# USDA-ARS-GBRU/itsxpress

Measured on AMD Instinct MI355X. Metric: reads/sec trimmed (ITS2, stand-in taxon Tracheophyta for Fungi), higher is better.
Workload: dtype u8+f32

## Files before the change

### itsxpress_amd/csrc/engine.h

```cpp
#pragma once
#include <cstddef>
#include <hip/hip_runtime.h>
#include <stdint.h>
#include <string>
#include <vector>
#include "../../include/itsx_hip.h"
#include "switches.h"

namespace itsx {

constexpr int KP = 18;
constexpr int NCODE = 16;
constexpr int QMAX = 12;
constexpr int MMAX = 46;
constexpr int MSV_REGS = 23;
constexpr int MSV_TW = 24;
constexpr int MAXDOM = 8;
constexpr int BOUND_PAIRS = 23;
constexpr int BOUND_RTAB = BOUND_PAIRS * 12 + 4;
constexpr int BOUND_TAB = (BOUND_PAIRS + 1) * 16 + 2 * BOUND_PAIRS + 2;

struct HostProfile {
  std::string name;
  int M = 0, Q = 0;
  float compo[4];
  float evparam[6];
  std::vector<float> t, mat, tsc, msc;
  float scale_b; int base_b, bias_b, tbm_b, tec_b;
  std::vector<uint8_t> rbv;
  std::vector<float> rfv;
  std::vector<float> tfv;
  float ft10, ft11, fpi0, fpi1;
  float feo[KP][2];
  std::vector<int16_t> rww;
  std::vector<int16_t> tww;
};
std::string parse_hmm_text(const char *text, int64_t len, std::vector<HostProfile> &out);
uint8_t host_tjb_b(int L);

struct alignas(16) DevProfile {
  float tf[QMAX * 8 * 4];
  float tb[QMAX * 6 * 4];
  float rf[NCODE * QMAX * 4];
  float feo[NCODE * 2];
  float ft10, ft11, fpi0, fpi1;
  float ev[6];
  int   M, Q;
  int   pad[4];
  float tfn[(QMAX * 4 + 1) * 8];
};

static_assert(offsetof(DevProfile, tb) == sizeof(float) * QMAX * 8 * 4, "k_float.hip reaches tb as tf + 384 floats");
static_assert(offsetof(DevProfile, tfn) % 16 == 0 && sizeof(DevProfile) % 16 == 0, "tfn is read with 16-byte loads");

constexpr int VIT_TAB = 8 * (MMAX + 1) + NCODE * (MMAX + 1);
struct LenTables {
  float   nullsc;
  float   bias_a;
  float   bias_b;
  float   p1;
  double  lognn3;
  int     tjb;
  int     vmove;
  float   lazy_c;
  int     pad;
};

struct PairRec {
  int32_t  useq;
  int32_t  prof;
  int32_t  xj;
  int32_t  L;
};
struct PairOut {
  float filtersc, fwdsc, bcksc, nullsc, msv_sc;
  int32_t pass_bias, pass_fwd, nregions, ndom, flags;
  int32_t nregions_raw;
};
struct RegionRec {
  int32_t pair;
  int32_t ienv, jenv;
  int32_t multi;
};
struct RegionOut {
  float envsc;
  float domcorrection;
  float n2log[NCODE];
  int32_t ok;
  int32_t own;
  float bN0;
};

#define HIPCHK(expr)                                                                            \
  do {                                                                                          \
    hipError_t e__ = (expr);                                                                    \
    if (e__ != hipSuccess) {                                                                    \
      set_error(std::string(#expr) + ": " + hipGetErrorString(e__));                            \
      return ITSX_E_DEVICE;                                                                     \
    }                                                                                           \
  } while (0)

}
```

### itsxpress_amd/csrc/engine.hip

```cpp
#include <algorithm>
#include <chrono>
#include <cmath>
#include <cstdio>
#include <cstring>
#include <functional>
#include <map>
#include <memory>
#include <numeric>
#include <atomic>
#include <condition_variable>
#include <mutex>
#include <string_view>
#include <thread>
#include <unordered_map>
#include "detmath.h"
#include "engine.h"
#include "k_api.h"
#include "deflate_codes.h"
#include "inflate_codes.h"
#include "fastq_rec.h"
#include "twriter_dev.h"
#include "cluster_multi.h"
#include "fastq_io.h"
#include "iupac.h"
// ... 373 lines not shown
  DBuf<uint32_t> w_slot_of; DBuf<unsigned int> w_ncoll;
  DBuf<uint16_t> w_thr, w_res; DBuf<int32_t> w_tjb, w_cnt, w_total, w_rows, w_rcnt, w_rpref, w_scan2, w_b, w_rrows;
  DBuf<int64_t> w_seg_start, w_idx, w_rseg, w_dz, w_counters, w_useg;
  DBuf<int32_t> w_rrep, w_ruq, w_rurank;
  DBuf<WaveDesc> w_waves, w_rw; DBuf<RegionRec> w_raw; DBuf<float> w_slab, w_eslab;
  DBuf<int32_t> w_mrcnt, w_mroff, w_mrlen, w_mrloff, w_mrrows, w_mrulist, w_mrulist2, w_mru; DBuf<int64_t> w_mrrowoff; DBuf<MrRec> w_mr; DBuf<MrOut> w_mrout; DBuf<int64_t> w_n2off; DBuf<float> w_n2sc, w_mrslab;
  DBuf<uint8_t> w_mrscratch; DBuf<WaveDesc> w_mrwaves;
  DBuf<RegionRec> w_pool, w_pool_sorted; DBuf<int32_t> w_pool_k; DBuf<unsigned long long> w_pool_n, w_pool_key; int64_t pool_cap = 0;
  DBuf<int32_t> w_mrsel; DBuf<int64_t> w_mrselrow; DBuf<MrBig> w_mrbig; DBuf<uint8_t> w_mrarena; DBuf<int32_t> w_mrenv; DBuf<WaveDesc> w_mrbigwaves;
  DBuf<int32_t> w_cl, w_cr;
  DBuf<int8_t> w_side; DBuf<unsigned long long> w_bl, w_br; DBuf<int32_t> w_uind, w_us, w_ue, w_ut, w_rs, w_re, w_rt, w_ri, w_uflag;

  struct ShareBatch { int32_t k0, k1; int64_t node0, nnodes; int32_t nsplit; int64_t gnode0, gnnodes; };
  bool share_on = false; int share_B = 32, share_logB = 5, share_maxd = 0;
  DBuf<unsigned long long> sh_tab, sh_mask_s, sh_mask, sh_counters, msv_xb; DBuf<uint8_t> sh_depth_s, sh_depth;
  DBuf<int32_t> sh_src, sh_parent_s, sh_parent, sh_nn_s, sh_nn, sh_node0_s, sh_node0, sh_order, sh_ulen, sh_uorder, sh_inv, sh_flag, sh_pos, sh_bstart, sh_cursor, sh_segk, sh_scan, sh_cuts;
  std::vector<ShareBatch> sh_batches; std::vector<int32_t> sh_segk_h;
  DBuf<uint4> sh_mgslots; size_t sh_mgslots_half = 0;
  DBuf<uint4> sh_mslots; size_t sh_mslots_half = 0, sh_fslots_half = 0; DBuf<uint32_t> sh_pass, sh_need; DBuf<int32_t> sh_real, sh_segflat, sh_segdepth, sh_wc, sh_woff; DBuf<int64_t> sh_bnd;
  DBuf<uint16_t> sh_res_chk; DBuf<float> sh_fb_chk;
  ShareDev sh_dev{};
  std::string switches_at_search;
  struct TopUp { bool valid = false, list_live = false ; int64_t NP = 0; std::vector<int64_t> seg_start; std::vector<int32_t> total; int32_t u0 = 0, Uc = 0; } topup;
  DBuf<unsigned long long> l_zneed, l_zsplit, l_tcnt; DBuf<int32_t> l_slot, l_pslot; DBuf<uint32_t> l_cut;
  DBuf<int32_t> l_src; DBuf<unsigned long long> l_dmask, l_defn, l_tcnt2;
  int64_t n_topup_deferred = 0, n_topup_ensemble = 0, topup_deferred_live = 0 ;
  std::vector<int64_t> topup_defp;
  std::vector<int32_t> topup_profs, topup_partial;
  std::vector<unsigned long long> h_zneed;
  bool prev_lazy = false; int prev_P = 0; int64_t prev_U = 0, prev_Uc = 0;
  std::vector<int32_t> h_merge_index;
  bool merge_join = false;
  std::vector<int8_t> h_merge_join;
  int64_t pack_exc_hint = 0;
  bool keep_records = false;
  struct Records {
    bool have = false;
    DBuf<uint8_t> seq, qual, titles;
    const uint8_t *seq_p = nullptr;
    DBuf<int64_t> off, toff;
    NameList h_titles;
    void drop() { have = false; seq_p = nullptr; seq.release(); qual.release(); titles.release(); off.release(); toff.release(); h_titles.clear(); }
  } rec;
  bool keep_pair_records = false;
  struct PairRecords {
    bool have = false; int64_t n = 0;
    DBuf<uint8_t> s1, q1, t1, s2, q2, t2;
    DBuf<int64_t> o1, to1, o2, to2;
    DBuf<int32_t> pair_read;
    std::vector<int64_t> pstart;
    void drop()
    {
      have = false; n = 0; pstart.clear(); pair_read.release();
      s1.release(); q1.release(); t1.release(); s2.release(); q2.release(); t2.release(); o1.release(); to1.release(); o2.release(); to2.release();
    }
  } prec;
  DBuf<TrimRec> w_trec2; DBuf<int32_t> w_ttlen;
  DBuf<TrimRec> w_trec; DBuf<int64_t> w_tcnt, w_ttot, w_tblk, w_tfirst, w_tbounds; DBuf<int32_t> w_tstart, w_tstop; DBuf<uint32_t> w_tout;
  DBuf<DeflateBlock> w_dblk; DBuf<uint32_t> w_dtok, w_dtext; DBuf<uint8_t> w_dslots, w_dpacked; DBuf<int32_t> w_dsizes; DBuf<int64_t> w_ddst;
  DBuf<uint8_t> tw_raw; DBuf<int32_t> tw_ls, tw_le; DBuf<int64_t> tw_lblk, tw_qsrc, tw_info;
  DBuf<int8_t> tw_strand; DBuf<uint8_t> tw_comp; bool tw_comp_set = false;
  std::mutex tw_mu; bool tw_failed = false; float tw_ms_deflate = 0;
  DBuf<uint8_t> inf_gz, inf_text; DBuf<int64_t> inf_counts, inf_base, inf_list, inf_where; DBuf<InflateMember> inf_mem; DBuf<int32_t> inf_status;
  int64_t inf_len = -1, n_inf_device = 0, n_inf_declined = 0; bool device_inflate = false; std::mutex inf_mu;
  DBuf<uint8_t> ps_text, ps_seq, ps_qual, ps_titles; DBuf<int64_t> ps_lblk, ps_nl, ps_blk, ps_off, ps_toff, ps_info;
  int64_t ps_n = -1, ps_nb = 0, ps_nt = 0, n_parse_device = 0, n_parse_declined = 0; bool ps_qual_kept = false, device_parse = false; std::mutex ps_mu;
  struct PairSide { DBuf<uint8_t> seq, qual, titles; DBuf<int64_t> off, toff; int64_t nb = 0, nt = 0; } pp[2];
  int64_t pp_n = -1; DBuf<unsigned long long> pp_info;
  bool two_on = false; int share_maxrd = 0; int32_t Ub = 0; size_t sh_gslots_off = 0;
  DBuf<uint8_t> sh_rdepth_s, sh_rdepth; DBuf<unsigned long long> sh_rmask_s, sh_rmask, sh_keys, sh_keys2;
  DBuf<int32_t> sh_rparent_s, sh_rparent, sh_jlev_s, sh_jown_s, sh_endrow_s, sh_rsteps_s, sh_rnn_s, sh_rnode0_s, sh_endrow, sh_jlev, sh_jsrc, sh_jownb;
  DBuf<int32_t> sh_border_s, sh_invb, sh_bsegk, sh_rnn, sh_rnode0, sh_border, sh_bulen, sh_rsrc, sh_bsteps, sh_vals;
  DBuf<uint8_t> sh_sorttmp;
  std::vector<int32_t> sh_bsegk_h;
  BShareDev sh_bdev{};
  DBuf<uint32_t> sh_needb; DBuf<uint16_t> sh_resb; DBuf<int32_t> sh_cntb, sh_totalb, sh_realb, sh_bsegflat, sh_bsegdepth, sh_bwc, sh_bwoff; DBuf<int64_t> sh_bbnd, sh_bseg_start;
  DBuf<PairRec> sh_bpairs; DBuf<WaveDesc> sh_bwaves;
};

#define CTXCHK(c)                                   \
  if (!(c)) return ITSX_E_ARG;
#define SET_ERR(ctx, code, msg) do { (ctx)->set_error(msg); return (code); } while (0)
#undef HIPCHK
#define HIPCHK(expr)                                                                      \
  do {                                                                                    \
    hipError_t e__ = (expr);                                                              \
    if (e__ != hipSuccess) { ctx->set_error(std::string(#expr) + ": " + hipGetErrorString(e__)); return ITSX_E_DEVICE; } \
  } while (0)

template <class T> static hipError_t upload(DBuf<T> &d, const std::vector<T> &h, hipStream_t st, size_t min_elems = 1)
{
  hipError_t e = d.alloc(std::max(h.size(), min_elems));
  if (e != hipSuccess) return e;
  if (h.empty()) return hipSuccess;
  return hipMemcpyAsync(d.p, h.data(), h.size() * sizeof(T), hipMemcpyHostToDevice, st);
}

struct LazyTimers {
  struct Rec { hipEvent_t a, b; float *acc; };
  std::vector<Rec> recs; hipStream_t st;
  explicit LazyTimers(hipStream_t s) : st(s) {}
  size_t begin(float *acc) { Rec r; (void)hipEventCreate(&r.a); (void)hipEventCreate(&r.b); r.acc = acc; (void)hipEventRecord(r.a, st); recs.push_back(r); return recs.size() - 1; }
  void end(size_t i) { (void)hipEventRecord(recs[i].b, st); }
  void collect()
  {
    for (auto &r : recs) { (void)hipEventSynchronize(r.b); float ms = 0; (void)hipEventElapsedTime(&ms, r.a, r.b); *r.acc += ms; (void)hipEventDestroy(r.a); (void)hipEventDestroy(r.b); }
    recs.clear();
  }
  ~LazyTimers() { collect(); }
};

struct StageTimer {
  hipEvent_t a = nullptr, b = nullptr; hipStream_t st;
  explicit StageTimer(hipStream_t s) : st(s) { (void)hipEventCreate(&a); (void)hipEventCreate(&b); (void)hipEventRecord(a, st); }
  float stop() { (void)hipEventRecord(b, st); (void)hipEventSynchronize(b); float ms = 0; (void)hipEventElapsedTime(&ms, a, b); return ms; }
  ~StageTimer() { if (a) (void)hipEventDestroy(a); if (b) (void)hipEventDestroy(b); }
};

using itsx_io::on_threads;

extern "C" {

int itsx_abi_version(void) { return ITSX_ABI_VERSION; }

const char *itsx_last_error(const itsx_ctx *ctx) { return ctx ? ctx->err.c_str() : g_create_error.c_str(); }

struct LoadPriority {
  itsx_ctx *c; bool on;
  explicit LoadPriority(itsx_ctx *ctx) : c(ctx), on(ctx && ctx->st_hi != nullptr) { if (on) std::swap(c->st, c->st_hi); }
  ~LoadPriority() { if (on) { (void)hipStreamSynchronize(c->st); std::swap(c->st, c->st_hi); } }
  LoadPriority(const LoadPriority &) = delete;
  LoadPriority &operator=(const LoadPriority &) = delete;
};

itsx_ctx *itsx_create(int device_id, int flags)
{
  (void)flags;
  int ndev = 0;
  hipError_t e = hipGetDeviceCount(&ndev);
  if (e != hipSuccess || ndev <= 0) { g_create_error = "no HIP device is visible (the engine has no CPU fallback)"; return nullptr; }
  if (device_id < 0 || device_id >= ndev) { g_create_error = "device ordinal out of range"; return nullptr; }
  e = hipSetDevice(device_id);
  if (e != hipSuccess) { g_create_error = std::string("hipSetDevice: ") + hipGetErrorString(e); return nullptr; }
  hipDeviceProp_t prop;
  if (hipGetDeviceProperties(&prop, device_id) != hipSuccess) { g_create_error = "hipGetDeviceProperties failed"; return nullptr; }
  if (std::string(prop.gcnArchName).compare(0, 6, "gfx950") != 0) {
    g_create_error = std::string("device is ") + prop.gcnArchName + "; this engine ships gfx950 code only";
    return nullptr;
  }
  itsx_ctx *ctx = new itsx_ctx();
  ctx->device = device_id;
  ctx->w_slab.pool_device = device_id;
  { std::lock_guard<std::mutex> g(g_pool_mu); g_live_contexts++; }
  if (hipStreamCreate(&ctx->st) != hipSuccess) { g_create_error = "hipStreamCreate failed"; delete ctx; return nullptr; }
  if (!(sw_get("ITSX_LOAD_PRIORITY") && atoi(sw_get("ITSX_LOAD_PRIORITY")) == 0)) {
    int least = 0, greatest = 0;
    if (hipDeviceGetStreamPriorityRange(&least, &greatest) != hipSuccess || greatest == least ||
        hipStreamCreateWithPriority(&ctx->st_hi, hipStreamDefault, greatest) != hipSuccess) { (void)hipGetLastError(); ctx->st_hi = nullptr; }
  }
  std::vector<float> tbl(16000);
  for (int i = 0; i < 16000; i++) tbl[i] = (float)log(1. + exp((double)-i / 1000.f));
  if (upload(ctx->d_flogsum, tbl, ctx->st) != hipSuccess) { g_create_error = "device allocation failed"; delete ctx; return nullptr; }
  std::vector<LogTab> lt(LOGTAB_N);
  build_logtab(lt.data());
  if (upload(ctx->d_logtab, lt, ctx->st) != hipSuccess) { g_create_error = "device allocation failed"; delete ctx; return nullptr; }
  (void)hipStreamSynchronize(ctx->st);
  return ctx;
}

void itsx_destroy(itsx_ctx *ctx)
{
  if (!ctx) return;
  (void)hipSetDevice(ctx->device);
  (void)hipStreamSynchronize(ctx->st);
  if (ctx->st3) { (void)hipStreamSynchronize(ctx->st3); (void)hipStreamDestroy(ctx->st3); (void)hipEventDestroy(ctx->ev_s3a); (void)hipEventDestroy(ctx->ev_s3b); }
  if (ctx->st2) { (void)hipStreamSynchronize(ctx->st2); (void)hipStreamDestroy(ctx->st2); (void)hipEventDestroy(ctx->ev_a); (void)hipEventDestroy(ctx->ev_b);
                  if (ctx->ev_msv0) { (void)hipEventDestroy(ctx->ev_msv0); (void)hipEventDestroy(ctx->ev_msv1); (void)hipEventDestroy(ctx->ev_c); } }
  (void)hipStreamDestroy(ctx->st);
  if (ctx->st_hi) { (void)hipStreamSynchronize(ctx->st_hi); (void)hipStreamDestroy(ctx->st_hi); }
  for (int k = 0; k < itsx_ctx::NSTAGE; k++) { if (ctx->stage_pin[k]) (void)hipHostFree(ctx->stage_pin[k]); if (ctx->stage_ev[k]) (void)hipEventDestroy(ctx->stage_ev[k]); }
  delete ctx;
  grave_flush();
  bool last = false;
  { std::lock_guard<std::mutex> g(g_pool_mu); last = --g_live_contexts <= 0; }
  if (last) pool_flush();
}

int itsx_release_scratch(itsx_ctx *ctx)
{
  CTXCHK(ctx);
  HIPCHK(hipSetDevice(ctx->device));
  HIPCHK(hipStreamSynchronize(ctx->st));
  if (ctx->st2) HIPCHK(hipStreamSynchronize(ctx->st2));
  if (ctx->st3) HIPCHK(hipStreamSynchronize(ctx->st3));
  if (ctx->w_slab.p) { pool_put(ctx->w_slab.p, ctx->w_slab.cap * sizeof(float), ctx->device); ctx->w_slab.p = nullptr; ctx->w_slab.n = ctx->w_slab.cap = 0; }
  return ITSX_OK;
}

static int install_profiles(itsx_ctx *ctx, std::vector<HostProfile> &pv, int *n_profiles)
{
  for (auto &p : pv) {
    if (p.M > MMAX || p.Q > QMAX) SET_ERR(ctx, ITSX_E_UNSUPPORTED, "model '" + p.name + "' has more than 46 nodes; the device kernels hold at most 46");
    if (p.base_b + p.bias_b >= 255) SET_ERR(ctx, ITSX_E_UNSUPPORTED, "model '" + p.name + "': MSV bias too large");
  }
  ctx->thr_memo.clear(); ctx->thr_memo_have.clear(); ctx->thr_memo_F1 = -1.0;
  HIPCHK(hipSetDevice(ctx->device));
  LoadPriority load_priority(ctx);
  ctx->profs = std::move(pv);
  const int P = (int)ctx->profs.size();
  ctx->P = P; ctx->G = (P + 63) / 64;
  const int Ppad = ctx->G * 64;
  std::vector<DevProfile> dp(std::max(P, 1));
  ctx->generic_q.assign(P, 0);
  std::vector<uint32_t> etab((size_t)std::max(P, 1) * 16 * MSV_TW, 0);
  std::vector<int32_t> pb(std::max(Ppad, 64), 0), pt(std::max(Ppad, 64), 0), pm(std::max(Ppad, 64), 0);
  for (size_t i = 0; i < etab.size(); i++) etab[i] = 0xFF01FF01u;
  for (int i = 0; i < P; i++) {
    const HostProfile &h = ctx->profs[i];
    DevProfile &d = dp[i];
    memset(&d, 0, sizeof(d));
    for (int q = 0; q < h.Q; q++) {
      for (int t = 0; t < 7; t++) for (int z = 0; z < 4; z++) d.tf[(q * 8 + t) * 4 + z] = h.tfv[((size_t)q * 7 + t) * 4 + z];
      for (int z = 0; z < 4; z++) d.tf[(q * 8 + 7) * 4 + z] = h.tfv[((size_t)7 * h.Q + q) * 4 + z];
    }
    for (int k = 1; k <= 4 * h.Q; k++)
      for (int t = 0; t < 8; t++) d.tfn[k * 8 + t] = d.tf[(((k - 1) % h.Q) * 8 + t) * 4 + (k - 1) / h.Q];
    for (int q = 0; q < h.Q; q++) {
      const int order[3] = {6, 5, 0};
      for (int k = 0; k < 3; k++) for (int z = 0; z < 4; z++) d.tb[(q * 6 + k) * 4 + z] = d.tf[(q * 8 + order[k]) * 4 + z];
      for (int k = 0; k < 3; k++)
        for (int z = 0; z < 4; z++) {
          float v;
          if (q + 1 < h.Q) v = d.tf[((q + 1) * 8 + 1 + k) * 4 + z];
          else v = (z < 3) ? d.tf[(0 * 8 + 1 + k) * 4 + z + 1] : 0.0f;
          d.tb[(q * 6 + 3 + k) * 4 + z] = v;
        }
    }
    for (int x = 0; x < NCODE; x++)
      for (int q = 0; q < h.Q; q++) for (int z = 0; z < 4; z++) d.rf[(x * QMAX + q) * 4 + z] = h.rfv[((size_t)x * h.Q + q) * 4 + z];
    for (int x = 0; x < NCODE; x++) { d.feo[x * 2] = h.feo[x][0]; d.feo[x * 2 + 1] = h.feo[x][1]; }
    d.ft10 = h.ft10; d.ft11 = h.ft11; d.fpi0 = h.fpi0; d.fpi1 = h.fpi1;
    for (int k = 0; k < 6; k++) d.ev[k] = h.evparam[k];
    d.M = h.M; d.Q = h.Q;
    ctx->generic_q[i] = (h.Q != QMAX);
    for (int x = 0; x < NCODE; x++)
      for (int r = 0; r < MSV_REGS; r++) {
        uint32_t packed = 0;
        for (int half = 0; half < 2; half++) {
          const int k = half * MSV_REGS + r + 1;
          const int cost = (k <= h.M) ? h.rbv[(size_t)x * (h.M + 1) + k] : 255;
          const int16_t e = (int16_t)(h.bias_b - cost);
          packed |= (uint32_t)(uint16_t)e << (16 * half);
        }
        etab[((size_t)i * 16 + x) * MSV_TW + r] = packed;
      }
    pb[i] = h.bias_b; pt[i] = h.tec_b; pm[i] = h.tbm_b;
  }
  {
    std::vector<int16_t> vt((size_t)std::max(P, 1) * VIT_TAB, (int16_t)-32768);
    for (int i = 0; i < P; i++) {
      const HostProfile &h = ctx->profs[i];
      int16_t *t = vt.data() + (size_t)i * VIT_TAB;
      for (int k8 = 0; k8 < 8; k8++) for (int k = 0; k <= h.M; k++) t[k8 * (MMAX + 1) + k] = h.tww[(size_t)k8 * (h.M + 1) + k];
      for (int x = 0; x < NCODE; x++) for (int k = 0; k <= h.M; k++) t[(8 + x) * (MMAX + 1) + k] = h.rww[(size_t)x * (h.M + 1) + k];
    }
    HIPCHK(upload(ctx->d_vtab, vt, ctx->st));
  }
  {
    const int KK = 2 * BOUND_PAIRS;
    std::vector<std::vector<double>> G((size_t)P), SC((size_t)P), AA((size_t)P), RI((size_t)P);
    bool fold = !(sw_get("ITSX_BOUND_FOLD") && atoi(sw_get("ITSX_BOUND_FOLD")) == 0);
    for (int i = 0; i < P && fold; i++) {
      const DevProfile &d = dp[i];
      const int K = 4 * ctx->profs[i].Q;
      auto tn = [&](int k, int t) { return (k >= 1 && k <= K) ? (double)d.tfn[k * 8 + t] : 0.0; };
      std::vector<double> H((size_t)KK + 3, 1.0), &g = G[(size_t)i], &sc = SC[(size_t)i], &aa = AA[(size_t)i], &ri = RI[(size_t)i];
      g.assign((size_t)KK + 2, 1.0); sc.assign((size_t)KK + 3, 1.0); aa.assign((size_t)KK + 2, 0.0); ri.assign((size_t)KK + 2, 1.0);
      for (int k = KK; k >= 1; k--) H[(size_t)k] = 1.0 + tn(k, 7) * H[(size_t)k + 1];
      for (int k = 1; k <= KK; k++) g[(size_t)k] = 1.0 + tn(k, 4) * H[(size_t)k + 1];
      for (int k = 1; k <= KK; k++) {
        const double md = tn(k, 4), dd = tn(k, 7);
        if (md > 0.0) { sc[(size_t)k + 1] = md / g[(size_t)k]; aa[(size_t)k] = sc[(size_t)k] * dd / sc[(size_t)k + 1]; }
        else if (dd > 0.0 && k > 1) fold = false;
        else { sc[(size_t)k + 1] = 1.0; aa[(size_t)k] = 0.0; }
        if (!(sc[(size_t)k + 1] > 1e-6 && sc[(size_t)k + 1] < 1e6 && aa[(size_t)k] < 1e6)) fold = false;
        const double mi = tn(k, 5);
        if (mi > 0.0) ri[(size_t)k] = mi / g[(size_t)k];
        else if (tn(k, 6) > 0.0 || tn(k + 1, 2) > 0.0) fold = false;
        else ri[(size_t)k] = 1.0;
        if (!(ri[(size_t)k] > 1e-6)) fold = false;
      }
    }
    ctx->bound_fold = fold;
    std::vector<float> bt((size_t)std::max(P, 1) * BOUND_TAB, 0.0f);
    for (int i = 0; i < P; i++) {
      const DevProfile &d = dp[i];
      const int K = 4 * ctx->profs[i].Q;
      auto tn = [&](int k, int t) { return (k >= 1 && k <= K) ? d.tfn[k * 8 + t] : 0.0f; };
      auto gk = [&](int k) { return fold && k >= 1 && k <= KK ? G[(size_t)i][(size_t)k] : 1.0; };
      auto sk = [&](int k) { return fold && k >= 1 && k <= KK + 1 ? SC[(size_t)i][(size_t)k] : 1.0; };
      auto rk = [&](int k) { return fold && k >= 1 && k <= KK ? RI[(size_t)i][(size_t)k] : 1.0; };
      for (int j = 0; j <= BOUND_PAIRS; j++) {
        float *o = bt.data() + (size_t)i * BOUND_TAB + (size_t)j * 16;
        if (j < BOUND_PAIRS) {
          const int k1 = 2 * j + 1, k2 = 2 * j + 2;
          o[0] = (float)(tn(k1 + 1, 1) / gk(k1)); o[1] = (float)(tn(k2 + 1, 1) / gk(k2));
          o[2] = (float)(tn(k1 + 1, 2) * rk(k1)); o[3] = (float)(tn(k2 + 1, 2) * rk(k2));
          o[4] = (float)(tn(k1 + 1, 3) * sk(k1)); o[5] = (float)(tn(k2 + 1, 3) * sk(k2));
          o[6] = tn(k1, 6); o[7] = tn(k2, 6);
          o[12] = (float)(tn(k1, 5) / gk(k1)); o[13] = (float)(tn(k2, 5) / gk(k2));
        }
        if (j > 0) {
          const int k1 = 2 * (j - 1) + 1, k2 = 2 * (j - 1) + 2;
          o[8] = tn(k1, 0); o[9] = tn(k2, 0);
          if (fold) { o[10] = k1 > 1 ? (float)AA[(size_t)i][(size_t)k1 - 1] : 0.0f; o[11] = (float)AA[(size_t)i][(size_t)k1]; }
          else { o[10] = tn(k1 - 1, 7); o[11] = tn(k1, 7); }
          o[14] = tn(k1, 4); o[15] = tn(k2, 4);
        }
      }
      float *gq = bt.data() + (size_t)i * BOUND_TAB + (size_t)(BOUND_PAIRS + 1) * 16;
      for (int k0 = 0; k0 < KK; k0++) gq[k0] = (float)gk(k0 + 1);
    }
    HIPCHK(upload(ctx->d_btab, bt, ctx->st));
    std::vector<float> rt((size_t)std::max(P, 1) * BOUND_RTAB, 0.0f);
    for (int i = 0; i < P && fold; i++) {
      const float *b = bt.data() + (size_t)i * BOUND_TAB;
      for (int j = 0; j <= BOUND_PAIRS; j++) {
        float *o = rt.data() + (size_t)i * BOUND_RTAB + (size_t)j * 12;
        if (j < BOUND_PAIRS) {
          for (int q = 0; q < 6; q++) o[q] = b[(size_t)j * 16 + q];
          o[6] = b[(size_t)(j + 1) * 16 + 8]; o[7] = b[(size_t)(j + 1) * 16 + 9];
        }
        if (j >= 1) {
          const int jj = j - 1;
          float *q = j < BOUND_PAIRS ? o + 8 : o;
          q[0] = b[(size_t)jj * 16 + 6]; q[1] = b[(size_t)jj * 16 + 7];
          q[2] = b[(size_t)(jj + 1) * 16 + 11];
          q[3] = (jj + 2 <= BOUND_PAIRS) ? b[(size_t)(jj + 2) * 16 + 10] : 0.0f;
        }
      }
    }
    HIPCHK(upload(ctx->d_rtab, rt, ctx->st));
    std::vector<float> et((size_t)std::max(P, 1) * NCODE * KK, 0.0f);
    for (int i = 0; i < P && fold; i++) {
      const DevProfile &d = dp[i];
      const int Q = ctx->profs[i].Q;
      const float *gq = bt.data() + (size_t)i * BOUND_TAB + (size_t)(BOUND_PAIRS + 1) * 16;
      for (int x = 0; x < NCODE; x++)
        for (int k0 = 0; k0 < KK; k0++) {
          const float e = (k0 < 4 * Q) ? d.rf[(x * QMAX + (k0 % Q)) * 4 + k0 / Q] : 0.0f;
          et[((size_t)i * NCODE + x) * KK + k0] = e * gq[k0];
        }
    }
    HIPCHK(upload(ctx->d_entab, et, ctx->st));
  }
  HIPCHK(upload(ctx->d_prof, dp, ctx->st));
  HIPCHK(upload(ctx->d_etab, etab, ctx->st));
  HIPCHK(upload(ctx->d_pbias, pb, ctx->st));
  HIPCHK(upload(ctx->d_ptec, pt, ctx->st));
  HIPCHK(upload(ctx->d_ptbm, pm, ctx->st));
  HIPCHK(hipStreamSynchronize(ctx->st));
  ctx->stats.n_profiles = P;
  ctx->have_search = ctx->have_final = false;
  if (n_profiles) *n_profiles = P;
  return ITSX_OK;
}

int itsx_load_profiles_mem(itsx_ctx *ctx, const char *text, int64_t len, int *n_profiles)
{
  CTXCHK(ctx && text && len >= 0);
  std::vector<HostProfile> pv;
  const std::string e = parse_hmm_text(text, len, pv);
  if (!e.empty()) SET_ERR(ctx, ITSX_E_FORMAT, e);
  return install_profiles(ctx, pv, n_profiles);
}

static bool inflate_for_loader(itsx_ctx *ctx, const itsx_io::Text &raw, itsx_io::Text &out);
static bool device_inflate_on(const itsx_ctx *ctx);
constexpr int PARSE_FALLBACK = 1;
static bool device_parse_on(const itsx_ctx *ctx);
static int load_parsed_device(itsx_ctx *ctx, const char *const *paths, int32_t n_paths, const char *text, int64_t nbytes, int64_t *n_reads_per_file, bool batch);
static int merge_pairs_load_device(itsx_ctx *ctx, const char *const *r1_paths, const char *const *r2_paths, const char *const *seq_out_paths, int32_t S,
                                   const char *text1, int64_t nb1, const char *text2, int64_t nb2, int maxdiffs, double maxee, int allow_stagger,
                                   int64_t *n_pairs_per_sample, int64_t *n_merged_per_sample, bool batch);
static std::shared_ptr<const itsx_io::Text> slurp(const char *path, bool cacheable, std::string &err, itsx_ctx *ctx = nullptr)
{
  if (ctx && device_inflate_on(ctx)) {
    const itsx_io::InflateFirst first = [ctx](const itsx_io::Text &raw, itsx_io::Text &out) { return inflate_for_loader(ctx, raw, out); };
    return itsx_io::read_text(path, err, cacheable, &first);
  }
  return itsx_io::read_text(path, err, cacheable);
}

int itsx_load_profiles_file(itsx_ctx *ctx, const char *hmm_path, int *n_profiles)
{
  CTXCHK(ctx && hmm_path);
  std::string err;
  const auto tp = slurp(hmm_path, false, err);
  if (!tp) SET_ERR(ctx, ITSX_E_IO, err);
  return itsx_load_profiles_mem(ctx, tp->data(), (int64_t)tp->size(), n_profiles);
}

int itsx_profile_name(const itsx_ctx *ctx, int i, char *buf, int buflen)
{
  CTXCHK(ctx && buf && buflen > 0 && i >= 0 && i < ctx->P);
  snprintf(buf, (size_t)buflen, "%s", ctx->profs[i].name.c_str());
  return ITSX_OK;
}

int itsx_profile_tables(const itsx_ctx *ctx, int i, uint8_t *rbv, float *rfv, float *tfv, int32_t *params6)
{
  CTXCHK(ctx && i >= 0 && i < ctx->P);
  const HostProfile &h = ctx->profs[i];
  if (rbv) memcpy(rbv, h.rbv.data(), h.rbv.size());
  if (rfv) memcpy(rfv, h.rfv.data(), h.rfv.size() * sizeof(float));
  if (tfv) memcpy(tfv, h.tfv.data(), h.tfv.size() * sizeof(float));
  if (params6) { params6[0] = h.M; params6[1] = h.Q; params6[2] = h.base_b; params6[3] = h.bias_b; params6[4] = h.tbm_b; params6[5] = h.tec_b; }
  return ITSX_OK;
}

static int8_t g_code[256];
static bool g_code_init = false;
static void init_codes()
{
  if (g_code_init) return;
  memset(g_code, -1, sizeof(g_code));
  const char *sym = "ACGT-RYMKSWHBVDN";
  for (int i = 0; i < 16; i++) { g_code[(unsigned char)sym[i]] = (int8_t)i; g_code[(unsigned char)(sym[i] | 0x20)] = (int8_t)i; }
  g_code[(unsigned char)'-'] = -1;
  g_code[(unsigned char)'U'] = g_code[(unsigned char)'u'] = 3;
  g_code[(unsigned char)'X'] = g_code[(unsigned char)'x'] = 15;
  g_code_init = true;
}

static int stage_reserve(itsx_ctx *ctx, int64_t bytes)
{
  if ((int64_t)ctx->stage_cap >= bytes) return ITSX_OK;
  for (int k = 0; k < itsx_ctx::NSTAGE; k++) {
    if (ctx->stage_pin[k]) { (void)hipHostFree(ctx->stage_pin[k]); ctx->stage_pin[k] = nullptr; }
    HIPCHK(hipHostMalloc(&ctx->stage_pin[k], (size_t)bytes, hipHostMallocDefault));
    HIPCHK(ctx->stage_dev[k].alloc((size_t)bytes + 16, true));
    if (!ctx->stage_ev[k]) HIPCHK(hipEventCreateWithFlags(&ctx->stage_ev[k], hipEventDisableTiming));
  }
  ctx->stage_cap = (size_t)bytes;
  return ITSX_OK;
}

static int pack_and_upload(itsx_ctx *ctx, const char *view = nullptr, const uint8_t *dev_raw = nullptr)
{
  init_codes();
  ctx->rec.drop(); ctx->prec.drop();
  const auto tp0 = std::chrono::steady_clock::now();
  const int64_t n = ctx->N;
  ctx->dev_bases = dev_raw;
  if (ctx->d_merged_text.p && dev_raw != ctx->d_merged_text.p) ctx->d_merged_text.release();
  ctx->bases_view = dev_raw ? nullptr : (view ? view : ctx->h_bases.data());
  const char *bases = ctx->bases_view;
  ctx->h_len.resize((size_t)n); ctx->h_woff.resize((size_t)n + 1);
  ctx->h_woff[0] = 0;
  int Lmax = 0;
  {
    const int T = n >= (1 << 20) ? std::max(1, std::min(8, itsx_io::io_threads())) : 1;
    std::vector<int64_t> wsum((size_t)T + 1, 0); std::vector<int> lmx((size_t)T, 0), bad((size_t)T, 0);
    on_threads(T, [&](int t) {
      const int64_t lo = n * t / T, hi = n * (t + 1) / T;
      int64_t w = 0; int mx = 0, b = 0;
      for (int64_t r = lo; r < hi; r++) {
        const int64_t L = ctx->h_off[r + 1] - ctx->h_off[r];
        if (L < 0) b |= 1;
        if (L > 65535) b |= 2;
        ctx->h_len[r] = (int32_t)L;
        mx = std::max(mx, (int)std::min<int64_t>(L, 1 << 30));
        w += std::max<int64_t>(1, (L + 15) / 16);
        ctx->h_woff[r + 1] = w;
      }
      wsum[(size_t)t + 1] = w; lmx[(size_t)t] = mx; bad[(size_t)t] = b;
    });
    int b = 0;
    for (int t = 0; t < T; t++) { wsum[(size_t)t + 1] += wsum[(size_t)t]; Lmax = std::max(Lmax, lmx[(size_t)t]); b |= bad[(size_t)t]; }
    if (b & 1) SET_ERR(ctx, ITSX_E_ARG, "read offsets must be non-decreasing");
    if (b & 2) SET_ERR(ctx, ITSX_E_UNSUPPORTED, "reads longer than 65535 bases are not supported");
    if (T > 1)
      on_threads(T, [&](int t) {
        if (t == 0) return;
        const int64_t lo = n * t / T, hi = n * (t + 1) / T, add = wsum[(size_t)t];
        for (int64_t r = lo; r < hi; r++) ctx->h_woff[r + 1] += add;
      });
  }
  ctx->Lmax = Lmax;
  HIPCHK(hipSetDevice(ctx->device));
  hipStream_t st = ctx->st;
  const int64_t nb = n > 0 ? ctx->h_off[n] : 0;
  int64_t CH = 64ll << 20;
  if (const char *e = sw_get("ITSX_PACK_CHUNK")) CH = std::max<int64_t>(70000, atoll(e));
  CH = std::min<int64_t>(CH, std::max<int64_t>(nb, 70000));
  constexpr int K = itsx_ctx::NSTAGE;
  if (!dev_raw) { const int src = stage_reserve(ctx, CH); if (src != ITSX_OK) return src; }
  DBuf<int64_t> &d_off = ctx->w_pk_off; DBuf<int8_t> &d_lut = ctx->w_pk_lut; DBuf<int32_t> &d_excnt = ctx->w_pk_excnt, &d_exstart = ctx->w_pk_exstart, &d_tmp = ctx->w_pk_tmp;
  DBuf<long long> &d_bad = ctx->w_pk_bad;
  HIPCHK(d_off.alloc((size_t)n + 1)); HIPCHK(d_lut.alloc(256)); HIPCHK(d_excnt.alloc((size_t)n + 2)); HIPCHK(d_exstart.alloc((size_t)n + 2));
  HIPCHK(d_tmp.alloc((size_t)scan_tmp_elems(n + 2))); HIPCHK(d_bad.alloc(4));
  HIPCHK(ctx->d_words.alloc((size_t)ctx->h_woff[n] + 1)); HIPCHK(ctx->d_woff.alloc((size_t)n + 1)); HIPCHK(ctx->d_excoff.alloc((size_t)n + 1)); HIPCHK(ctx->d_len.alloc((size_t)n + 1));
  HIPCHK(hipMemcpyAsync(d_off.p, ctx->h_off.data(), ((size_t)n + 1) * 8, hipMemcpyHostToDevice, st));
  HIPCHK(hipMemcpyAsync(ctx->d_woff.p, ctx->h_woff.data(), ((size_t)n + 1) * 8, hipMemcpyHostToDevice, st));
  if (n) HIPCHK(hipMemcpyAsync(ctx->d_len.p, ctx->h_len.data(), (size_t)n * 4, hipMemcpyHostToDevice, st));
  HIPCHK(hipMemcpyAsync(d_lut.p, g_code, 256, hipMemcpyHostToDevice, st));
  HIPCHK(hipMemsetAsync(d_excnt.p, 0, ((size_t)n + 2) * 4, st));
  int64_t ecap = std::max<int64_t>((int64_t)ctx->d_exc.cap, nb / 256 + 4096 + ctx->pack_exc_hint);
  ctx->pack_exc_hint = 0;
  if (const char *e = sw_get("ITSX_PACK_ECAP")) ecap = std::max<int64_t>(1, atoll(e));
  HIPCHK(ctx->d_exc.alloc((size_t)ecap));
  int copy_threads = std::max(1, std::min(8, itsx_io::io_threads()));
  long long hb[4] = {0, 0, 0, 0};
  for (int pass = 0; pass < 2; pass++) {
    const long long init[4] = {0, 0, 0x7f7f7f7f7f7f7f7fll, 0};
    HIPCHK(hipMemcpyAsync(d_bad.p, init, sizeof(init), hipMemcpyHostToDevice, st));
    int64_t r0 = 0; int c = 0;
    if (dev_raw && n > 0) {
      if (pass == 0) launch_pack(dev_raw, 0, d_off.p, ctx->d_woff.p, 0, n, d_lut.p, ctx->d_words.p, d_excnt.p, d_bad.p + 2, st);
      launch_exclusive_scan(d_excnt.p, d_exstart.p, n + 1, d_tmp.p, st);
      launch_pack_exc(dev_raw, 0, d_off.p, 0, n, d_lut.p, d_excnt.p, d_exstart.p, d_bad.p, ecap, ctx->d_excoff.p, ctx->d_exc.p, st);
      r0 = n;
    }
    while (r0 < n) {
      const int64_t b0 = ctx->h_off[r0];
      int64_t r1 = (int64_t)(std::upper_bound(ctx->h_off.begin() + r0, ctx->h_off.begin() + n + 1, b0 + CH) - ctx->h_off.begin()) - 1;
      r1 = std::min<int64_t>(n, std::max<int64_t>(r1, r0 + 1));
      const int64_t bytes = ctx->h_off[r1] - b0;
      const int k = c % K;
      if (c >= K) HIPCHK(hipEventSynchronize(ctx->stage_ev[k]));
      if (bytes > 0) {
        char *dst = (char *)ctx->stage_pin[k];
        const int T = bytes >= (4 << 20) ? copy_threads : 1;
        on_threads(T, [&](int t) { const int64_t lo = bytes * t / T, hi = bytes * (t + 1) / T; memcpy(dst + lo, bases + b0 + lo, (size_t)(hi - lo)); });
        HIPCHK(hipMemcpyAsync(ctx->stage_dev[k].p, dst, (size_t)bytes, hipMemcpyHostToDevice, st));
      }
      if (pass == 0) launch_pack(ctx->stage_dev[k].p, b0, d_off.p, ctx->d_woff.p, r0, r1, d_lut.p, ctx->d_words.p, d_excnt.p, d_bad.p + 2, st);
      launch_exclusive_scan(d_excnt.p + r0, d_exstart.p + r0, r1 - r0 + 1, d_tmp.p, st);
      launch_pack_exc(ctx->stage_dev[k].p, b0, d_off.p, r0, r1, d_lut.p, d_excnt.p, d_exstart.p, d_bad.p, ecap, ctx->d_excoff.p, ctx->d_exc.p, st);
      HIPCHK(hipEventRecord(ctx->stage_ev[k], st));
      r0 = r1; c++;
    }
    if (n == 0) HIPCHK(hipMemsetAsync(ctx->d_excoff.p, 0, 8, st));
    HIPCHK(hipMemcpyAsync(hb, d_bad.p, sizeof(hb), hipMemcpyDeviceToHost, st));
    HIPCHK(hipStreamSynchronize(st));
    HIPCHK(hipGetLastError());
    if (hb[2] >= 0 && hb[2] < n) SET_ERR(ctx, ITSX_E_FORMAT, "read " + std::to_string(hb[2]) + " contains a symbol outside the IUPAC DNA alphabet");
    if (!hb[1]) break;
    if (pass == 1) SET_ERR(ctx, ITSX_E_DEVICE, "exception list overflow after resizing");
    ecap = hb[0] + 1;
    HIPCHK(ctx->d_exc.alloc((size_t)ecap));
  }
  ctx->rd.words = ctx->d_words.p; ctx->rd.woff = ctx->d_woff.p; ctx->rd.len = ctx->d_len.p;
  ctx->rd.excoff = ctx->d_excoff.p; ctx->rd.exc = ctx->d_exc.p; ctx->rd.n = n;
  ctx->have_derep = ctx->have_search = ctx->have_final = false; ctx->drop_cigars();
  ctx->stats.n_reads = n;
  ctx->order_cache_ok = false;
  ctx->S = 1; ctx->sel_sample = -1; ctx->h_sample.clear(); ctx->h_usample.clear();
  ctx->stats.ms_pack = (float)std::chrono::duration<double, std::milli>(std::chrono::steady_clock::now() - tp0).count();
  return ITSX_OK;
}

static int64_t take_offsets(itsx_ctx *ctx, const int64_t *offsets, int64_t n)
{
  const int64_t base0 = offsets[0];
  ctx->h_off.resize((size_t)n + 1);
  int64_t *dst = ctx->h_off.data();
  const int T = n >= (1 << 20) ? std::max(1, std::min(8, itsx_io::io_threads())) : 1;
  on_threads(T, [&](int t) { for (int64_t r = (n + 1) * t / T, hi = (n + 1) * (t + 1) / T; r < hi; r++) dst[r] = offsets[r] - base0; });
  return base0;
}
static int set_reads_impl(itsx_ctx *ctx, const char *bases, const int64_t *offsets, int64_t n, const char *names, const int64_t *name_offsets, bool borrow)
{
  CTXCHK(ctx && offsets && n >= 0 && (bases || offsets[n] == offsets[0]));
  if (n >= (1ll << 31) - 64) SET_ERR(ctx, ITSX_E_UNSUPPORTED, "more than 2^31 reads in one context");
  ctx->N = n;
  const int64_t base0 = take_offsets(ctx, offsets, n);
  const char *view = nullptr;
  if (borrow) { itsx_io::Text().swap(ctx->h_bases); view = bases ? bases + base0 : ""; }
  else if (bases) ctx->h_bases.assign(bases + base0, (size_t)(offsets[n] - base0));
  else ctx->h_bases.clear();
  ctx->h_names.clear();
  if (names && name_offsets) {
    ctx->h_names.assign(names, name_offsets, n);
  }
  return pack_and_upload(ctx, view);
}
int itsx_set_reads(itsx_ctx *ctx, const char *bases, const int64_t *offsets, int64_t n, const char *names, const int64_t *name_offsets)
{ return set_reads_impl(ctx, bases, offsets, n, names, name_offsets, false); }
int itsx_set_reads_view(itsx_ctx *ctx, const char *bases, const int64_t *offsets, int64_t n, const char *names, const int64_t *name_offsets)
{ return set_reads_impl(ctx, bases, offsets, n, names, name_offsets, true); }
int itsx_set_reads_device(itsx_ctx *ctx, const void *d_bases, const int64_t *offsets, int64_t n, const char *names, const int64_t *name_offsets)
{
  CTXCHK(ctx && offsets && n >= 0 && (d_bases || offsets[n] == offsets[0]));
  if (n >= (1ll << 31) - 64) SET_ERR(ctx, ITSX_E_UNSUPPORTED, "more than 2^31 reads in one context");
  ctx->N = n;
  const int64_t base0 = take_offsets(ctx, offsets, n);
  itsx_io::Text().swap(ctx->h_bases);
  ctx->h_names.clear();
  if (names && name_offsets) {
    ctx->h_names.assign(names, name_offsets, n);
  }
  static const uint8_t none = 0;
  return pack_and_upload(ctx, nullptr, d_bases ? (const uint8_t *)d_bases + base0 : &none);
}

struct FastxPart {
  itsx_io::Text seq, qual; std::vector<int64_t> off{0}; NameList ids;
  NameList titles;
  bool lower = false;
  int rc = ITSX_OK; std::string err;
};

static void parse_fastx_range(const char *s, const char *end, bool want_qual, bool upper, FastxPart &out)
{
  auto next_line = [&](const char *&b, const char *&e) -> bool {
    if (s >= end) return false;
    b = s; const char *nl = (const char *)memchr(s, '\n', (size_t)(end - s));
    e = nl ? nl : end; s = nl ? nl + 1 : end;
    if (e > b && e[-1] == '\r') e--;
    return true;
  };
  auto put_seq = [&](const char *b, const char *e) {
    const size_t o = out.seq.size();
    out.seq.append(b, e);
    if (upper) { char *q = out.seq.data(); for (size_t i = o; i < out.seq.size(); i++) { const char u = (char)toupper((unsigned char)q[i]); if (u != q[i]) { q[i] = u; out.lower = true; } } }
  };
  if (end > s && (size_t)(end - s) > ((size_t)1 << 20)) { out.seq.reserve(out.seq.size() + (size_t)(end - s) / 2 + 4096); if (want_qual) out.qual.reserve(out.qual.size() + (size_t)(end - s) / 2 + 4096); out.ids.blob.reserve(out.ids.blob.size() + (size_t)(end - s) / 8); }
  const char *b, *e;
  bool pending = false;
  while (pending || next_line(b, e)) {
    pending = false;
    if (b == e) continue;
    if (*b == '@') {
      const char *ne = b + 1; while (ne < e && *ne != ' ' && *ne != '\t') ne++;
      out.ids.emplace_back(b + 1, ne);
      const char *sb, *se, *pb, *pe, *qb, *qe;
      if (!next_line(sb, se) || !next_line(pb, pe) || !next_line(qb, qe) || pb == pe || *pb != '+' || (qe - qb) != (se - sb)) {
        out.rc = ITSX_E_FORMAT; out.err = "malformed FASTQ record"; return;
      }
      put_seq(sb, se);
// ... 693 lines not shown
  }
  if (n_helpers == 0) return itsx_cluster(ctx, id, strand_both, n_unique);
  if (!(id > 0.0 && id <= 1.0)) SET_ERR(ctx, ITSX_E_ARG, "cluster id must be in (0, 1]");
  if (id == 1.0) return itsx_derep(ctx, strand_both, 32, n_unique);
  if (ctx->S > 1) SET_ERR(ctx, ITSX_E_UNSUPPORTED, "greedy clustering (id < 1) is sequential per sample: run it one sample per call, not on a sample batch");
  ClusterShards shards(ctx->device, ctx->st, hs);
  return cluster_run(ctx, id, strand_both, n_unique, false, &shards);
}
int itsx_cluster_samples(itsx_ctx *ctx, double id, int strand_both, int64_t *n_unique)
{
  CTXCHK(ctx);
  if (!(id > 0.0 && id <= 1.0)) SET_ERR(ctx, ITSX_E_ARG, "cluster id must be in (0, 1]");
  if (id == 1.0) return itsx_derep(ctx, strand_both, 32, n_unique);
  if (ctx->S <= 1) return itsx_cluster(ctx, id, strand_both, n_unique);
  return cluster_run(ctx, id, strand_both, n_unique, true);
}

int itsx_get_cluster(const itsx_ctx *ctx, double *pct_id, int64_t *order, int64_t *n_order)
{
  CTXCHK(ctx && ctx->have_derep && ctx->clustered);
  if (pct_id) for (int64_t r = 0; r < ctx->N; r++) pct_id[r] = ctx->h_pct[r];
  if (order) for (size_t i = 0; i < ctx->h_order.size(); i++) order[i] = ctx->h_order[i];
  if (n_order) *n_order = (int64_t)ctx->h_order.size();
  return ITSX_OK;
}

int itsx_align_clusters(itsx_ctx *ctx, int64_t *n_aligned, float *ms_kernels)
{
  CTXCHK(ctx);
  if (!ctx->have_derep || !ctx->clustered) SET_ERR(ctx, ITSX_E_ARG, "itsx_align_clusters comes after a clustering at id < 1 (itsx_cluster, itsx_cluster_multi, itsx_cluster_samples); exact dereplication has nothing to align");
  HIPCHK(hipSetDevice(ctx->device));
  ctx->drop_cigars();
  const int64_t n = ctx->N;
  hipStream_t st = ctx->st;
  std::vector<int32_t> hq, ht; std::vector<int8_t> hs;
  int Lmax = 1;
  for (int64_t r = 0; r < n; r++) {
    const int32_t rep = ctx->h_rep_of[(size_t)r];
    if (rep < 0 || rep == r) continue;
    hq.push_back((int32_t)r); ht.push_back(rep); hs.push_back(ctx->h_strand[(size_t)r]);
    Lmax = std::max(Lmax, std::max((int)ctx->h_len[(size_t)r], (int)ctx->h_len[(size_t)rep]));
  }
  const size_t M = hq.size();
  float ms = 0.0f;
  std::vector<std::string> text(M);
  if (M > 0) {
    int rows_per_lane = (Lmax + 1 <= 320) ? 5 : (Lmax + 1 <= 512) ? 8 : 10;
    if (const char *e = sw_get("ITSX_CL_ROWS")) rows_per_lane = atoi(e) <= 5 ? 5 : atoi(e) <= 8 ? 8 : 10;
    double budget_mb = 2048.0;
    if (const char *e = sw_get("ITSX_CIGAR_MB")) budget_mb = std::max(0.0, atof(e));
    const size_t budget = (size_t)(budget_mb * 1048576.0);
    DBuf<int32_t> d_q, d_t, d_eq, d_tlen; DBuf<int8_t> d_s; DBuf<int64_t> d_doff, d_soff, d_toff;
    DBuf<uint8_t> d_dir, d_text; DBuf<long long> d_scr, d_res; DBuf<double> d_pid;
    HIPCHK(upload(d_q, hq, st)); HIPCHK(upload(d_t, ht, st)); HIPCHK(upload(d_s, hs, st));
    HIPCHK(d_eq.alloc(M)); HIPCHK(d_res.alloc(M)); HIPCHK(d_pid.alloc(M));
    CigarArgs a{};
    a.rd = ctx->rd; a.q_read = d_q.p; a.t_read = d_t.p; a.strand = d_s.p; a.res = d_res.p; a.pid = d_pid.p;
    std::vector<int32_t> eq(M);
    launch_cg_equal(a, (int32_t)M, d_eq.p, st);
    HIPCHK(hipMemcpyAsync(eq.data(), d_eq.p, M * sizeof(int32_t), hipMemcpyDeviceToHost, st));
    HIPCHK(hipStreamSynchronize(st));
    std::vector<int32_t> pq, pt, pm; std::vector<int8_t> ps; std::vector<int64_t> doff, soff;
    struct Batch { size_t p0, np, dir_bytes, scr_elems; };
    std::vector<Batch> batches;
    for (size_t m = 0; m < M; m++) {
      if (eq[m]) { text[m] = "="; continue; }
      size_t db = 0, sb = 0;
      cg_pair_bytes(ctx->h_len[(size_t)hq[m]], ctx->h_len[(size_t)ht[m]], rows_per_lane, &db, &sb);
      db = (db + 255) & ~(size_t)255;
      if (batches.empty() || (batches.back().np > 0 && batches.back().dir_bytes + batches.back().scr_elems * 8 + db + sb > budget)) batches.push_back(Batch{pq.size(), 0, 0, 0});
      Batch &b = batches.back();
      doff.push_back((int64_t)b.dir_bytes); soff.push_back((int64_t)b.scr_elems);
      b.np++; b.dir_bytes += db; b.scr_elems += sb / 8;
      pq.push_back(hq[m]); pt.push_back(ht[m]); ps.push_back(hs[m]); pm.push_back((int32_t)m);
    }
    const size_t NP = pq.size();
    if (NP > 0) {
      size_t max_dir = 0, max_scr = 0, max_np = 0;
      for (const Batch &b : batches) { max_dir = std::max(max_dir, b.dir_bytes); max_scr = std::max(max_scr, b.scr_elems); max_np = std::max(max_np, b.np); }
      HIPCHK(upload(d_q, pq, st)); HIPCHK(upload(d_t, pt, st)); HIPCHK(upload(d_s, ps, st)); HIPCHK(upload(d_doff, doff, st)); HIPCHK(upload(d_soff, soff, st));
      if (d_dir.alloc(max_dir + 256, true) != hipSuccess || d_scr.alloc(max_scr + 2, true) != hipSuccess) {
        (void)hipGetLastError();
        SET_ERR(ctx, ITSX_E_NOMEM, "itsx_align_clusters: no device memory for " + std::to_string((max_dir + max_scr * 8) >> 20) + " MB of direction bits (lower ITSX_CIGAR_MB; a pair larger than the budget needs its own size)");
      }
      HIPCHK(d_tlen.alloc(max_np)); HIPCHK(d_toff.alloc(max_np + 1));
      a.q_read = d_q.p; a.t_read = d_t.p; a.strand = d_s.p; a.dir_off = d_doff.p; a.scr_off = d_soff.p;
      a.dir = d_dir.p; a.scratch = d_scr.p; a.tlen = d_tlen.p; a.toff = d_toff.p;
      std::vector<int32_t> tlen; std::vector<int64_t> toff; std::vector<char> plane;
      for (const Batch &b : batches) {
        StageTimer t1(st);
        launch_cg_forward(a, (int32_t)b.p0, (int32_t)b.np, rows_per_lane, Lmax, st);
        launch_cg_traceback(a, (int32_t)b.p0, (int32_t)b.np, rows_per_lane, 0, st);
        ms += t1.stop();
        HIPCHK(hipGetLastError());
        tlen.resize(b.np); toff.assign(b.np + 1, 0);
        HIPCHK(hipMemcpy(tlen.data(), d_tlen.p, b.np * sizeof(int32_t), hipMemcpyDeviceToHost));
        for (size_t k = 0; k < b.np; k++) {
          if (tlen[k] <= 0) SET_ERR(ctx, ITSX_E_DEVICE, "itsx_align_clusters: the direction bits of read " + std::to_string(pq[b.p0 + k]) + " do not lead back to the first cell");
          toff[k + 1] = toff[k] + tlen[k];
        }
        HIPCHK(d_text.alloc((size_t)toff[b.np] + 1));
        a.text = reinterpret_cast<char *>(d_text.p);
        HIPCHK(hipMemcpyAsync(d_toff.p, toff.data(), (b.np + 1) * sizeof(int64_t), hipMemcpyHostToDevice, st));
        StageTimer t2(st);
        launch_cg_traceback(a, (int32_t)b.p0, (int32_t)b.np, rows_per_lane, 1, st);
        ms += t2.stop();
        HIPCHK(hipGetLastError());
        plane.resize((size_t)toff[b.np]);
        HIPCHK(hipMemcpy(plane.data(), d_text.p, plane.size(), hipMemcpyDeviceToHost));
        for (size_t k = 0; k < b.np; k++) text[(size_t)pm[b.p0 + k]].assign(plane.data() + toff[k], (size_t)tlen[k]);
      }
      std::vector<double> pid(NP);
      HIPCHK(hipMemcpy(pid.data(), d_pid.p, NP * sizeof(double), hipMemcpyDeviceToHost));
      for (size_t k = 0; k < NP; k++)
        if (memcmp(&pid[k], &ctx->h_pct[(size_t)pq[k]], sizeof(double)) != 0)
          SET_ERR(ctx, ITSX_E_DEVICE, "itsx_align_clusters: read " + std::to_string(pq[k]) + " aligns at identity " + std::to_string(pid[k]) + ", the clustering accepted it at " + std::to_string(ctx->h_pct[(size_t)pq[k]]));
    }
  }
  ctx->h_cg_off.assign((size_t)n + 1, 0);
  { size_t m = 0, tot = 0; for (int64_t r = 0; r < n; r++) { ctx->h_cg_off[(size_t)r] = (int64_t)tot; if (m < M && hq[m] == r) tot += text[m++].size(); } ctx->h_cg_off[(size_t)n] = (int64_t)tot; ctx->h_cg_text.reserve(tot); }
  for (size_t m = 0; m < M; m++) ctx->h_cg_text += text[m];
  ctx->have_cigar = true;
  if (n_aligned) *n_aligned = (int64_t)M;
  if (ms_kernels) *ms_kernels = ms;
  return ITSX_OK;
}
int itsx_get_cluster_cigars(const itsx_ctx *ctx, int64_t *offs, char *text)
{
  CTXCHK(ctx && offs);
  if (!ctx->cigars_live()) SET_ERR(ctx, ITSX_E_ARG, "itsx_get_cluster_cigars: no alignments for the current clustering (itsx_align_clusters comes after itsx_cluster* at id < 1)");
  memcpy(offs, ctx->h_cg_off.data(), ((size_t)ctx->N + 1) * sizeof(int64_t));
  if (text && !ctx->h_cg_text.empty()) memcpy(text, ctx->h_cg_text.data(), ctx->h_cg_text.size());
  return ITSX_OK;
}

int itsx_get_derep(const itsx_ctx *ctx, int64_t *rep_of, int8_t *strand, int64_t *uniq_of)
{
  CTXCHK(ctx && ctx->have_derep);
  for (int64_t r = 0; r < ctx->N; r++) {
    if (rep_of) rep_of[r] = ctx->h_rep_of[r];
    if (strand) strand[r] = ctx->h_strand[r];
    if (uniq_of) uniq_of[r] = ctx->h_uniq_of[r];
  }
  return ITSX_OK;
}
int itsx_get_uniques(const itsx_ctx *ctx, int64_t *seed_read, int64_t *abundance)
{
  CTXCHK(ctx && ctx->have_derep);
  for (int32_t u = 0; u < ctx->U; u++) { if (seed_read) seed_read[u] = ctx->h_seed_read[u]; if (abundance) abundance[u] = ctx->h_abund[u]; }
  return ITSX_OK;
}


int itsx_unique_keys(itsx_ctx *ctx, uint64_t seed, uint64_t *fwd, uint64_t *rc)
{
  CTXCHK(ctx && ctx->have_derep && fwd && rc);
  if (ctx->S > 1) SET_ERR(ctx, ITSX_E_UNSUPPORTED, "cross-rank dereplication of a sample batch is not supported: shard whole samples across ranks");
  HIPCHK(hipSetDevice(ctx->device));
  const int64_t n = ctx->N;
  if (n == 0 || ctx->U == 0) return ITSX_OK;
  HIPCHK(ctx->w_hf.alloc((size_t)n + 1)); HIPCHK(ctx->w_hr.alloc((size_t)n + 1));
  launch_hash_reads(ctx->rd, seed, 1, ctx->w_hf.p, ctx->w_hr.p, ctx->st);
  std::vector<uint64_t> hf((size_t)n), hr((size_t)n);
  HIPCHK(hipMemcpyAsync(hf.data(), ctx->w_hf.p, (size_t)n * 8, hipMemcpyDeviceToHost, ctx->st));
  HIPCHK(hipMemcpyAsync(hr.data(), ctx->w_hr.p, (size_t)n * 8, hipMemcpyDeviceToHost, ctx->st));
  HIPCHK(hipStreamSynchronize(ctx->st));
  for (int32_t u = 0; u < ctx->U; u++) {
    const size_t r = (size_t)ctx->h_seed_read[u];
    const uint64_t lm = (uint64_t)ctx->h_len[r] * 0x9E3779B97F4A7C15ULL;
    fwd[u] = hf[r] ^ lm; rc[u] = hr[r] ^ lm;
  }
  return ITSX_OK;
}

static int set_walked_uniques(itsx_ctx *ctx, const std::vector<int32_t> *keep)
{
  const std::vector<int32_t> &lst = keep ? *keep : ctx->h_sorted_uniq;
  ctx->U_active = (int32_t)lst.size();
  ctx->h_sorted_active = lst;
  if (!lst.empty()) {
    HIPCHK(hipMemcpyAsync(ctx->d_sorted_uniq.p, lst.data(), lst.size() * 4, hipMemcpyHostToDevice, ctx->st));
    launch_fill_ulen(ctx->U_active, ctx->d_sorted_uniq.p, ctx->d_seed_read.p, ctx->rd.len, ctx->d_ulen.p, ctx->st);
    HIPCHK(hipStreamSynchronize(ctx->st));
  }
  return ITSX_OK;
}

int itsx_set_active_uniques(itsx_ctx *ctx, const uint8_t *active)
{
  CTXCHK(ctx && ctx->have_derep && (active || ctx->U == 0));
  HIPCHK(hipSetDevice(ctx->device));
  std::vector<int32_t> keep; keep.reserve((size_t)ctx->U);
  for (int32_t s = 0; s < ctx->U; s++) { const int32_t u = ctx->h_sorted_uniq[(size_t)s]; if (active[u]) keep.push_back(u); }
  { const int rc = set_walked_uniques(ctx, &keep); if (rc != ITSX_OK) return rc; }
  ctx->active_narrowed = true;
  ctx->have_search = ctx->have_final = false;
  return ITSX_OK;
}

static float msv_score_from_byte(int xj, int tjb)
{
  float sc = ((float)(xj - tjb) - 190.0f);
  sc /= (float)(3.0 / 0.69314718055994529);
  sc -= 3.0f;
  return sc;
}

static int search_chunk(itsx_ctx *ctx, int ci, int32_t u0, int32_t U, int Lcap, double T, double F1, double F3);
static int append_traces(itsx_ctx *ctx);

static int build_share(itsx_ctx *ctx)
{
  hipStream_t st = ctx->st;
  itsx_stats &S = ctx->stats;
  ctx->share_on = false; ctx->sh_batches.clear(); ctx->sh_segk_h.clear();
  S.share_B = 0; S.share_batches = 0; S.share_nodes = S.share_chains = 0; S.ms_share_build = 0; S.share_frac = 0;
  ctx->two_on = false; ctx->Ub = 0; ctx->share_maxrd = 0; ctx->sh_bsegk_h.clear();
  S.two_sided = 0; S.n_joined = 0; S.bwd_chains = 0; S.gamma_nodes = 0; S.bwd_rows = 0; S.join_maxdiff = 0; S.ms_bwd_bound = 0; S.n_bwd_launches = 0; S.two_fwd_rows = S.two_bwd_rows = S.two_rows_full = 0;
  const int32_t U = ctx->U_active, Uc = (int32_t)std::min<int64_t>(ctx->s_Uc, 0x7fffffff), P = ctx->P;
  if (const char *e = sw_get("ITSX_SHARE")) if (atoi(e) == 0) return ITSX_OK;
  if (sw_get("ITSX_LAZY_EXACT_BOUND")) return ITSX_OK;
  if (U < 2 || U >= (1 << 26) || P <= 0) return ITSX_OK;
  int B = 32;
  if (const char *e = sw_get("ITSX_SHARE_B")) B = atoi(e);
  int logB = 0; while ((1 << logB) < B) logB++;
  if (B < 16 || B > 1024 || (1 << logB) != B) SET_ERR(ctx, ITSX_E_ARG, "ITSX_SHARE_B must be a power of two between 16 and 1024");
  StageTimer tm(st);
  TrieArgs a{};
  a.rd = ctx->rd; a.sorted_uniq = ctx->d_sorted_uniq.p; a.seed_read = ctx->d_seed_read.p; a.U = U; a.Uc = std::max(1, Uc); a.B = B;
  HIPCHK(ctx->sh_counters.alloc(16));
  HIPCHK(hipMemsetAsync(ctx->sh_counters.p, 0, 16 * sizeof(unsigned long long), st));
  a.counters = ctx->sh_counters.p;
  launch_trie_keycount(a, st);
  if (ctx->lazy && ctx->bound_fold) { TrieArgs r0 = a; r0.rev = 1; launch_trie_keycount(r0, st); }
  unsigned long long hc0[8] = {0, 0, 0, 0, 0, 0, 0, 0};
  HIPCHK(hipMemcpyAsync(hc0, ctx->sh_counters.p, sizeof(hc0), hipMemcpyDeviceToHost, st));
  HIPCHK(hipStreamSynchronize(st));
  const unsigned long long nkeys = std::max(hc0[4], hc0[6]);
  if (nkeys == 0) return ITSX_OK;
  uint64_t slots = 1024; while (slots < 2 * nkeys) slots <<= 1;
  HIPCHK(ctx->sh_tab.alloc((size_t)slots, true));
  HIPCHK(hipMemsetAsync(ctx->sh_tab.p, 0xFF, (size_t)slots * sizeof(unsigned long long), st));
  HIPCHK(ctx->sh_depth_s.alloc((size_t)U + 1)); HIPCHK(ctx->sh_parent_s.alloc((size_t)U + 1)); HIPCHK(ctx->sh_mask_s.alloc((size_t)U + 1));
  HIPCHK(ctx->sh_nn_s.alloc((size_t)U + 2)); HIPCHK(ctx->sh_node0_s.alloc((size_t)U + 2)); HIPCHK(ctx->sh_scan.alloc((size_t)scan_tmp_elems((int64_t)U + 2)));
  HIPCHK(hipMemsetAsync(ctx->sh_mask_s.p, 0, ((size_t)U + 1) * sizeof(unsigned long long), st));
  a.tab = ctx->sh_tab.p; a.tmask = slots - 1; a.depth = ctx->sh_depth_s.p; a.parent = ctx->sh_parent_s.p; a.mask = ctx->sh_mask_s.p; a.nn = ctx->sh_nn_s.p;
  launch_trie_insert(a, st); launch_trie_resolve(a, st); launch_trie_link(a, st); launch_trie_count(a, st);
  launch_exclusive_scan(ctx->sh_nn_s.p, ctx->sh_node0_s.p, (int64_t)U + 1, ctx->sh_scan.p, st);
  bool two = ctx->lazy && ctx->bound_fold && !(sw_get("ITSX_SHARE_TWO") && atoi(sw_get("ITSX_SHARE_TWO")) == 0);
  TrieArgs ar = a;
  JoinArgs ja{};
  if (two) {
    HIPCHK(ctx->sh_rdepth_s.alloc((size_t)U + 1)); HIPCHK(ctx->sh_rparent_s.alloc((size_t)U + 1)); HIPCHK(ctx->sh_rmask_s.alloc((size_t)U + 1));
    HIPCHK(ctx->sh_jlev_s.alloc((size_t)U + 1)); HIPCHK(ctx->sh_jown_s.alloc((size_t)U + 1)); HIPCHK(ctx->sh_endrow_s.alloc((size_t)U + 1));
    HIPCHK(ctx->sh_rsteps_s.alloc((size_t)U + 1)); HIPCHK(ctx->sh_rnn_s.alloc((size_t)U + 2)); HIPCHK(ctx->sh_rnode0_s.alloc((size_t)U + 2));
    HIPCHK(hipMemsetAsync(ctx->sh_tab.p, 0xFF, (size_t)slots * sizeof(unsigned long long), st));
    HIPCHK(hipMemsetAsync(ctx->sh_rmask_s.p, 0, ((size_t)U + 1) * sizeof(unsigned long long), st));
    ar.rev = 1; ar.depth = ctx->sh_rdepth_s.p; ar.parent = ctx->sh_rparent_s.p; ar.mask = ctx->sh_rmask_s.p; ar.nn = ctx->sh_rnn_s.p;
    launch_trie_insert(ar, st); launch_trie_resolve(ar, st); launch_trie_link(ar, st);
    ja.t = ar; ja.fdepth = ctx->sh_depth_s.p; ja.fmask = ctx->sh_mask_s.p; ja.rmask = ctx->sh_rmask_s.p; ja.jlev = ctx->sh_jlev_s.p; ja.jown = ctx->sh_jown_s.p;
    ja.endrow = ctx->sh_endrow_s.p; ja.rsteps = ctx->sh_rsteps_s.p; ja.counters = ctx->sh_counters.p;
    launch_join_resolve(ja, st);
    for (int r = 63; r >= 1; r--) launch_join_up(ja, r, st);
    launch_join_ends(ja, st);
    launch_popc64(ctx->sh_rmask_s.p, ctx->sh_rnn_s.p, (int64_t)U + 1, U, st);
    launch_exclusive_scan(ctx->sh_rnn_s.p, ctx->sh_rnode0_s.p, (int64_t)U + 1, ctx->sh_scan.p, st);
  }
  const int32_t ncap = 65536 + U / std::max(1, Uc) + 8;
  HIPCHK(ctx->sh_cuts.alloc((size_t)ncap * 3));
  launch_share_cuts(ctx->d_ulen.p, ctx->sh_node0_s.p, two ? ctx->sh_rnode0_s.p : nullptr, U, a.Uc, ncap, ctx->sh_cuts.p, ctx->sh_counters.p + 5, st);
  int32_t NN = 0, NG = 0;
  unsigned long long hc[16];
  HIPCHK(hipMemcpyAsync(hc, ctx->sh_counters.p, sizeof(hc), hipMemcpyDeviceToHost, st));
  HIPCHK(hipMemcpyAsync(&NN, ctx->sh_node0_s.p + U, sizeof(NN), hipMemcpyDeviceToHost, st));
  if (two) HIPCHK(hipMemcpyAsync(&NG, ctx->sh_rnode0_s.p + U, sizeof(NG), hipMemcpyDeviceToHost, st));
  HIPCHK(hipStreamSynchronize(st));
  const int maxd = (int)hc[0];
  const double frac = hc[2] ? (double)hc[1] / (double)hc[2] : 0.0;
  S.share_frac = (float)frac;
  double min_frac = 0.10;
  if (const char *e = sw_get("ITSX_SHARE_MIN")) min_frac = atof(e);
  const int64_t ncuts = (int64_t)hc[5];
  if (frac < min_frac || maxd <= 0 || NN <= 0 || ncuts > ncap) { S.ms_share_build = tm.stop(); return ITSX_OK; }
  if (two && (hc[10] == 0 || NG <= 0)) two = false;
  const int maxrd = two ? (int)hc[13] : 0;
  std::vector<int32_t> cuts((size_t)ncuts * 3);
  HIPCHK(hipMemcpyAsync(cuts.data(), ctx->sh_cuts.p, cuts.size() * 4, hipMemcpyDeviceToHost, st));
  HIPCHK(hipStreamSynchronize(st));
  struct Cut { int32_t s, n, g; };
  std::vector<Cut> cv((size_t)ncuts);
  for (int64_t i = 0; i < ncuts; i++) cv[(size_t)i] = {cuts[(size_t)3 * i], cuts[(size_t)3 * i + 1], two ? cuts[(size_t)3 * i + 2] : 0};
  std::sort(cv.begin(), cv.end(), [](const Cut &x, const Cut &y) { return x.s < y.s; });
  cv.push_back({U, NN, two ? NG : 0});
  const bool fwd_too = ctx->lazy;
  double gb = fwd_too ? (two ? 76.0 : 48.0) : 8.0;
  {
    size_t fr = 0, tot = 0;
    const double held = (double)ctx->w_slab.cap * sizeof(float) + (double)ctx->sh_mslots.cap * sizeof(uint4);
    if (hipMemGetInfo(&fr, &tot) == hipSuccess) gb = std::min(gb, std::max(0.25, ((double)fr + held) / (double)(1ull << 30) / (fwd_too ? 3.0 : 8.0)));
  }
  if (const char *e = sw_get("ITSX_SHARE_GB")) gb = std::max(0.0001, atof(e));
  const bool two_fwd = sw_get("ITSX_SHARE_FWD_STREAMS") ? atoi(sw_get("ITSX_SHARE_FWD_STREAMS")) >= 2 : (U < 2000000 && !sw_get("ITSX_SHARE_GB"));
  const double state_b = fwd_too ? (two_fwd ? 2.0 : 1.0) * (double)FWD_STATE_Q * sizeof(float4) : 2.0 * (double)MSV_STATE_Q * sizeof(uint4);
  if (!sw_get("ITSX_SHARE_GB")) gb = std::min(gb, std::max(1.0, (double)((int64_t)NN + NG) * state_b * (double)P / (double)(1ull << 30) / 3.8));
  if (gb > 1.0) gb = floor(gb * 2.0) / 2.0;
  const int64_t nodes_max = std::max<int64_t>(1, (int64_t)(gb * (double)(1ull << 30) / (state_b * (double)P)));
  std::vector<int32_t> bstart; std::vector<itsx_ctx::ShareBatch> &bt = ctx->sh_batches;
  {
    size_t i = 0;
    while (i + 1 < cv.size()) {
      size_t j = i + 1;
      while (j + 1 < cv.size() && cv[j].s % a.Uc != 0 && ((int64_t)cv[j + 1].n - cv[i].n) + ((int64_t)cv[j + 1].g - cv[i].g) <= nodes_max) j++;
      itsx_ctx::ShareBatch b{};
      b.k0 = cv[i].s; b.k1 = cv[j].s; b.node0 = cv[i].n; b.nnodes = (int64_t)cv[j].n - cv[i].n; b.gnode0 = cv[i].g; b.gnnodes = (int64_t)cv[j].g - cv[i].g;
      b.nsplit = (int32_t)std::min<int64_t>(P, (b.nnodes + b.gnnodes + nodes_max - 1) / nodes_max); if (b.nsplit < 1) b.nsplit = 1;
      bstart.push_back(b.k0); bt.push_back(b);
      i = j;
    }
    bstart.push_back(U);
  }
  const int nb = (int)bt.size();
  if (nb >= (1 << 24)) { bt.clear(); S.ms_share_build = tm.stop(); return ITSX_OK; }
  for (auto &b : bt) if ((double)(b.nnodes + b.gnnodes) * state_b * (double)((P + b.nsplit - 1) / b.nsplit) > 1.5 * gb * (double)(1ull << 30)) { bt.clear(); S.ms_share_build = tm.stop(); return ITSX_OK; }
  HIPCHK(upload(ctx->sh_bstart, bstart, st)); HIPCHK(ctx->sh_segk.alloc((size_t)nb * SHARE_SEGS));
  HIPCHK(ctx->sh_uorder.alloc((size_t)U + 1)); HIPCHK(ctx->sh_inv.alloc((size_t)U + 1));
  HIPCHK(ctx->sh_keys.alloc((size_t)U + 1)); HIPCHK(ctx->sh_keys2.alloc((size_t)U + 1)); HIPCHK(ctx->sh_vals.alloc((size_t)U + 1));
  const size_t sort_bytes = order_sort_bytes(U);
  HIPCHK(ctx->sh_sorttmp.alloc(sort_bytes));
  launch_order_keys(ctx->sh_depth_s.p, two ? ctx->sh_endrow_s.p : ctx->d_ulen.p, nullptr, U, ctx->sh_bstart.p, nb, ctx->sh_keys.p, ctx->sh_vals.p, st);
  if (order_sort(ctx->sh_sorttmp.p, sort_bytes, ctx->sh_keys.p, ctx->sh_keys2.p, ctx->sh_vals.p, ctx->sh_uorder.p, U, st) != 0) SET_ERR(ctx, ITSX_E_DEVICE, "prefix sharing: the order's radix sort failed");
  HIPCHK(hipMemsetAsync(ctx->sh_counters.p + 15, 0, sizeof(unsigned long long), st));
  launch_order_segk(ctx->sh_keys2.p, U, nb, ctx->sh_segk.p, ctx->sh_inv.p, ctx->sh_uorder.p, U, ctx->sh_counters.p + 15, st);
  ctx->sh_segk_h.assign((size_t)nb * SHARE_SEGS, 0);
  HIPCHK(hipMemcpyAsync(ctx->sh_segk_h.data(), ctx->sh_segk.p, (size_t)nb * SHARE_SEGS * 4, hipMemcpyDeviceToHost, st));
  HIPCHK(ctx->sh_depth.alloc((size_t)U + 1)); HIPCHK(ctx->sh_parent.alloc((size_t)U + 1)); HIPCHK(ctx->sh_mask.alloc((size_t)U + 1));
  HIPCHK(ctx->sh_nn.alloc((size_t)U + 2)); HIPCHK(ctx->sh_node0.alloc((size_t)U + 2)); HIPCHK(ctx->sh_order.alloc((size_t)U + 1)); HIPCHK(ctx->sh_ulen.alloc((size_t)U + 1));
  HIPCHK(ctx->sh_endrow.alloc((size_t)U + 1)); HIPCHK(ctx->sh_jlev.alloc((size_t)U + 1)); HIPCHK(ctx->sh_jsrc.alloc((size_t)U + 1)); HIPCHK(ctx->sh_jownb.alloc((size_t)U + 1));
  ShareDev &o = ctx->sh_dev;
  HIPCHK(ctx->sh_src.alloc((size_t)U + 1));
  o.src = ctx->sh_src.p;
  o.depth = ctx->sh_depth.p; o.parent = ctx->sh_parent.p; o.mask = ctx->sh_mask.p; o.nn = ctx->sh_nn.p; o.node0 = ctx->sh_node0.p; o.order = ctx->sh_order.p; o.ulen = ctx->sh_ulen.p;
  o.endrow = ctx->sh_endrow.p; o.jlev = ctx->sh_jlev.p; o.jsrc = ctx->sh_jsrc.p;
  launch_share_permute(a, ctx->d_ulen.p, ctx->sh_uorder.p, ctx->sh_inv.p, two ? ctx->sh_endrow_s.p : nullptr, two ? ctx->sh_jlev_s.p : nullptr, o, st);
  launch_exclusive_scan(ctx->sh_nn.p, ctx->sh_node0.p, (int64_t)U + 1, ctx->sh_scan.p, st);
  launch_share_src(o, U, a.Uc, st);
  int32_t Ub = 0;
  if (two) {
    HIPCHK(ctx->sh_border_s.alloc((size_t)U + 1)); HIPCHK(ctx->sh_invb.alloc((size_t)U + 1)); HIPCHK(ctx->sh_bsegk.alloc((size_t)nb * SHARE_SEGS));
    launch_order_keys(ctx->sh_rdepth_s.p, ctx->sh_rsteps_s.p, ctx->sh_rsteps_s.p, U, ctx->sh_bstart.p, nb, ctx->sh_keys.p, ctx->sh_vals.p, st);
    if (order_sort(ctx->sh_sorttmp.p, sort_bytes, ctx->sh_keys.p, ctx->sh_keys2.p, ctx->sh_vals.p, ctx->sh_border_s.p, U, st) != 0) SET_ERR(ctx, ITSX_E_DEVICE, "two-sided sharing: the order's radix sort failed");
    HIPCHK(hipMemsetAsync(ctx->sh_counters.p + 15, 0, sizeof(unsigned long long), st));
    launch_order_segk(ctx->sh_keys2.p, U, nb, ctx->sh_bsegk.p, ctx->sh_invb.p, ctx->sh_border_s.p, U, ctx->sh_counters.p + 15, st);
    unsigned long long nv = 0;
    ctx->sh_bsegk_h.assign((size_t)nb * SHARE_SEGS, 0);
    HIPCHK(hipMemcpyAsync(ctx->sh_bsegk_h.data(), ctx->sh_bsegk.p, (size_t)nb * SHARE_SEGS * 4, hipMemcpyDeviceToHost, st));
    HIPCHK(hipMemcpyAsync(&nv, ctx->sh_counters.p + 15, sizeof(nv), hipMemcpyDeviceToHost, st));
    HIPCHK(hipStreamSynchronize(st));
    Ub = (int32_t)nv;
    HIPCHK(ctx->sh_rdepth.alloc((size_t)Ub + 1)); HIPCHK(ctx->sh_rparent.alloc((size_t)Ub + 1)); HIPCHK(ctx->sh_rmask.alloc((size_t)Ub + 1));
    HIPCHK(ctx->sh_rnn.alloc((size_t)Ub + 2)); HIPCHK(ctx->sh_rnode0.alloc((size_t)Ub + 2)); HIPCHK(ctx->sh_border.alloc((size_t)Ub + 1)); HIPCHK(ctx->sh_bulen.alloc((size_t)Ub + 1));
    HIPCHK(ctx->sh_rsrc.alloc((size_t)Ub + 1)); HIPCHK(ctx->sh_bsteps.alloc((size_t)Ub + 1));
    BShareDev &ob = ctx->sh_bdev;
    ob.depth = ctx->sh_rdepth.p; ob.parent = ctx->sh_rparent.p; ob.mask = ctx->sh_rmask.p; ob.nn = ctx->sh_rnn.p; ob.node0 = ctx->sh_rnode0.p; ob.order = ctx->sh_border.p;
    ob.ulen = ctx->sh_bulen.p; ob.src = ctx->sh_rsrc.p; ob.steps = ctx->sh_bsteps.p;
    launch_bshare_permute(ar, Ub, ctx->d_ulen.p, ctx->sh_border_s.p, ctx->sh_invb.p, ctx->sh_rmask_s.p, ctx->sh_rsteps_s.p, ob, st);
    launch_exclusive_scan(ctx->sh_rnn.p, ctx->sh_rnode0.p, (int64_t)Ub + 1, ctx->sh_scan.p, st);
    launch_bshare_src(ob, Ub, st);
    launch_join_src(U, B, ctx->sh_uorder.p, ctx->sh_jown_s.p, ctx->sh_invb.p, ob, o, ctx->sh_jownb.p, st);
    HIPCHK(ctx->sh_chain.alloc((size_t)U + 1)); HIPCHK(ctx->sh_bchain.alloc((size_t)Ub + 1));
    launch_chain_recs(U, ctx->rd, o.order, ctx->d_seed_read.p, o.src, o.node0, o.mask, o.endrow, o.jlev, o.jsrc, ctx->sh_chain.p, st);
    launch_chain_recs(Ub, ctx->rd, ob.order, ctx->d_seed_read.p, ob.src, ob.node0, ob.mask, ob.steps, nullptr, nullptr, ctx->sh_bchain.p, st);
  }
  HIPCHK(hipStreamSynchronize(st));
  int64_t need_slots = 0, need_gslots = 0;
  for (auto &b : bt) {
    const int64_t pr = (int64_t)((P + b.nsplit - 1) / b.nsplit);
    need_slots = std::max<int64_t>(need_slots, b.nnodes * pr); need_gslots = std::max<int64_t>(need_gslots, b.gnnodes * pr);
  }
  ctx->sh_mslots_half = (size_t)need_slots * MSV_STATE_Q;
  const size_t half = ((size_t)need_slots + (size_t)(two ? need_gslots : 0)) * FWD_STATE_Q;
  ctx->sh_gslots_off = (size_t)need_slots * FWD_STATE_Q;
  ctx->sh_fslots_half = (fwd_too && two_fwd && nb > 1) ? half : 0;
  ctx->sh_mgslots_half = (size_t)need_gslots * MSV_STATE_Q;
  if (ctx->sh_mslots.alloc(2 * (size_t)need_slots * MSV_STATE_Q + 1) != hipSuccess || (two && ctx->sh_mgslots.alloc(2 * (size_t)need_gslots * MSV_STATE_Q + 1) != hipSuccess) ||
      (fwd_too && ctx->w_slab.alloc(((4 * (half * (ctx->sh_fslots_half ? 2 : 1) + 1) + ((size_t)64 << 20) - 1) >> 26) << 26, true) != hipSuccess)) {
    (void)hipGetLastError();
    ctx->sh_mslots.release(); bt.clear();
    S.ms_share_build = tm.stop();
    return ITSX_OK;
  }
  ctx->share_on = true; ctx->share_B = B; ctx->share_logB = logB; ctx->share_maxd = maxd;
  ctx->two_on = two; ctx->Ub = Ub; ctx->share_maxrd = maxrd;
  S.share_B = B; S.share_batches = nb; S.share_nodes = NN; S.share_chains = (int64_t)hc[3];
  S.msv_rows_full = (int64_t)hc[2] * P; S.msv_rows = (int64_t)(hc[2] - hc[1]) * P;
  if (two && !(sw_get("ITSX_MSV_TWO") && atoi(sw_get("ITSX_MSV_TWO")) == 0)) S.msv_rows = (int64_t)(hc[11] + hc[12]) * P;
  if (two) { S.two_sided = 1; S.n_joined = (int64_t)hc[10]; S.bwd_chains = (int64_t)hc[14]; S.gamma_nodes = NG; S.two_fwd_rows = (int64_t)hc[11]; S.two_bwd_rows = (int64_t)hc[12]; S.two_rows_full = (int64_t)hc[2]; }
  S.ms_share_build = tm.stop();
  return ITSX_OK;
}

static int run_chunks(itsx_ctx *ctx, double T, double F1, double F3)
{
  const int64_t U = ctx->U_active, Uc = std::max<int64_t>(1, ctx->s_Uc);
  int ci = 0;
  if (ctx->st2) HIPCHK(hipStreamSynchronize(ctx->st2));
  ctx->msv_pre_u0 = -1;
  msv_diag_begin();
  const bool count_xb = sw_get("ITSX_PASSA_DBG") && (atoi(sw_get("ITSX_PASSA_DBG")) & 64);
  if (count_xb) { HIPCHK(ctx->msv_xb.alloc(8)); HIPCHK(hipMemsetAsync(ctx->msv_xb.p, 0, 8 * sizeof(unsigned long long), ctx->st)); HIPCHK(hipStreamSynchronize(ctx->st)); }
  else ctx->msv_xb.release();
  for (int64_t u0 = 0; u0 < U; u0 += Uc, ci++) {
    ctx->next_u0 = (u0 + Uc < U) ? u0 + Uc : -1;
    ctx->next_U = (int32_t)std::min<int64_t>(Uc, U - (u0 + Uc));
    const int rc = search_chunk(ctx, ci, (int32_t)u0, (int32_t)std::min<int64_t>(Uc, U - u0), ctx->s_Lcap, T, F1, F3);
    if (rc != ITSX_OK) return rc;
  }
  if (count_xb) {
    unsigned long long n[5] = {0, 0, 0, 0, 0};
    HIPCHK(hipDeviceSynchronize());
    HIPCHK(hipMemcpy(n, ctx->msv_xb.p, sizeof(n), hipMemcpyDeviceToHost));
    fprintf(stderr, "[itsx] msv floored wave-rows %llu, with the xB branch %llu (%.4f)\n", n[0], n[1], n[0] ? (double)n[1] / (double)n[0] : 0.0);
    int nsplit = 0;
    for (const auto &b : ctx->sh_batches) nsplit = std::max(nsplit, (int)b.nsplit);
    fprintf(stderr, "[itsx] msv shared waves: whole read %llu, window %llu, 16 words at a time %llu; profile ranges of a batch: at most %d\n", n[2], n[3], n[4], nsplit);
  }
  ctx->n_chunks = ci;
  return ITSX_OK;
}

static int compact_setup(itsx_ctx *ctx)
{
  hipStream_t st = ctx->st;
  const int P = ctx->P;
  ctx->compact_zmax = 1e9; ctx->compact_dome_min = 1e-2;
  if (const char *e = sw_get("ITSX_COMPACT_ZMAX")) ctx->compact_zmax = std::max(1.0, atof(e));
  if (const char *e = sw_get("ITSX_COMPACT_DOME_MIN")) ctx->compact_dome_min = std::max(1e-300, atof(e));
  ctx->compact_lnp = log(ctx->compact_dome_min / ctx->compact_zmax) - 1e-6;
  std::vector<int8_t> cls((size_t)P, 0); std::vector<std::string> seen;
  for (int p = 0; p < P; p++) {
    const std::string pre = ctx->profs[p].name.substr(0, 2);
    size_t k = 0; while (k < seen.size() && seen[k] != pre) k++;
    if (k == seen.size()) seen.push_back(pre);
    if (k > 126) SET_ERR(ctx, ITSX_E_UNSUPPORTED, "ITSX_COMPACT_ROWS: more than 127 distinct 2-character profile name prefixes");
    cls[p] = (int8_t)k;
  }
  ctx->compact_ncls = (int)seen.size();
  HIPCHK(upload(ctx->w_cls, cls, st));
  HIPCHK(ctx->w_bestc.alloc((size_t)ctx->U * ctx->compact_ncls + 1));
  HIPCHK(hipMemsetAsync(ctx->w_bestc.p, 0, ((size_t)ctx->U * ctx->compact_ncls + 1) * sizeof(unsigned long long), st));
  return ITSX_OK;
}

static int compact_segment(itsx_ctx *ctx, const itsx_domain *d_rows, int64_t NR, size_t di)
{
  hipStream_t st = ctx->st;
  launch_compact_best(d_rows, NR, ctx->w_cls.p, ctx->compact_ncls, ctx->compact_lnp, ctx->w_bestc.p, st);
  HIPCHK(ctx->w_keep.alloc((size_t)NR + 1)); HIPCHK(ctx->w_keeppos.alloc((size_t)NR + 1)); HIPCHK(ctx->w_keeptmp.alloc((size_t)scan_tmp_elems(NR + 1)));
  launch_compact_mark(d_rows, NR, ctx->w_cls.p, ctx->compact_ncls, ctx->compact_lnp, ctx->w_bestc.p, ctx->w_keep.p, st);
  launch_exclusive_scan(ctx->w_keep.p, ctx->w_keeppos.p, NR + 1, ctx->w_keeptmp.p, st);
  int32_t kept = 0;
  HIPCHK(hipMemcpyAsync(&kept, ctx->w_keeppos.p + NR, sizeof(kept), hipMemcpyDeviceToHost, st));
  HIPCHK(hipStreamSynchronize(st));
  DBuf<itsx_domain> &small = *ctx->dom_bufs[di];
  HIPCHK(small.alloc((size_t)std::max<int32_t>(kept, 1), true));
  launch_compact_scatter(d_rows, NR, ctx->w_keep.p, ctx->w_keeppos.p, small.p, st);
  ctx->rows_before_compaction += NR;
  ctx->dom_n[di] = kept;
  return ITSX_OK;
}

static int search_rows_mode(const itsx_ctx *ctx)
{
  int mode = ctx->rows_mode;
  if (mode < 0) {
    mode = ITSX_ROWS_FULL;
    if (sw_get("ITSX_COMPACT_ROWS") && atoi(sw_get("ITSX_COMPACT_ROWS")) != 0) mode = ITSX_ROWS_COMPACT;
    if (const char *e = sw_get("ITSX_ROWS")) mode = !strcmp(e, "lazy") ? ITSX_ROWS_LAZY : !strcmp(e, "compact") ? ITSX_ROWS_COMPACT : ITSX_ROWS_FULL;
  }
  if (mode == ITSX_ROWS_LAZY && sw_get("ITSX_KEEP_TRACE")) mode = ITSX_ROWS_COMPACT;
  return mode;
}

static int filter_tables(itsx_ctx *ctx, double F1, int64_t *cells_active_out)
{
  hipStream_t st = ctx->st;
  const int P = ctx->P, Ppad = ctx->G * 64;
  const int Lcap = ctx->Lmax + 1;
  std::vector<LenTables> lt((size_t)Lcap);
  std::vector<int32_t> tjb((size_t)Lcap, 0);
  std::vector<char> present((size_t)Lcap, 0);
  int64_t cells_active = 0;
  {
    const int32_t Ua = ctx->U, Uact = ctx->U_active;
    const int Th = Ua >= (1 << 19) ? std::max(1, std::min(8, itsx_io::io_threads())) : 1;
    std::vector<std::vector<char>> pres((size_t)Th); std::vector<int64_t> csum((size_t)Th, 0);
    on_threads(Th, [&](int t) {
      std::vector<char> &pr = pres[(size_t)t]; pr.assign((size_t)Lcap, 0);
      int64_t c = 0;
      for (int64_t u = (int64_t)Ua * t / Th, hi = (int64_t)Ua * (t + 1) / Th; u < hi; u++) {
        const int32_t L = ctx->h_len[ctx->h_seed_read[(size_t)u]];
        pr[(size_t)L] = 1;
        if (Uact == Ua) c += L;
      }
      csum[(size_t)t] = c;
    });
    for (int t = 0; t < Th; t++) { cells_active += csum[(size_t)t]; for (int L = 0; L < Lcap; L++) present[(size_t)L] |= pres[(size_t)t][(size_t)L]; }
    if (Uact != Ua) for (int32_t u : ctx->h_sorted_active) cells_active += ctx->h_len[ctx->h_seed_read[(size_t)u]];
  }
  for (int L = 0; L < Lcap; L++) {
    LenTables &t = lt[L]; memset(&t, 0, sizeof(t));
    if (L == 0) continue;
    const float p1 = (float)L / (float)(L + 1);
    t.p1 = p1;
    t.nullsc = (float)((double)(float)L * log((double)p1) + log(1. - (double)p1));
    t.bias_a = (float)L * logf(p1);
    t.bias_b = logf((float)(1. - (double)p1));
    t.lognn3 = log((double)((float)L / (float)(L + 3)));
    t.tjb = host_tjb_b(L);
    tjb[L] = t.tjb;
    {
      const double n = (double)L;
      const double c = 1.0 + (2.0 * log(2.0 * (n + 3.0) / (3.0 * (n + 2.0))) + n * log((n + 3.0) / (n + 2.0))) / 0.69314718055994529;
      const double margin = std::max(0.02, 6.0 * (n + (double)MMAX) * 5.9604644775390625e-8 / 0.69314718055994529);
      t.lazy_c = nextafterf((float)(c + margin), 1e30f);
    }
    { const float w = roundf((float)(500.0 / 0.69314718055994529) * logf((2.0f + 1.0f) / ((float)L + 2.0f + 1.0f)));
      t.vmove = (w >= 32767.0f) ? 32767 : (w <= -32768.0f) ? -32768 : (int)w; }
  }
  if (ctx->thr_memo_F1 != F1 || ctx->thr_memo_Ppad != Ppad) { ctx->thr_memo.clear(); ctx->thr_memo_have.clear(); ctx->thr_memo_F1 = F1; ctx->thr_memo_Ppad = Ppad; }
  if (ctx->thr_memo_have.size() < (size_t)Lcap) { ctx->thr_memo_have.resize((size_t)Lcap, 0); ctx->thr_memo.resize((size_t)Lcap * Ppad, 257); }
  std::vector<uint16_t> thr((size_t)Lcap * Ppad, 257);
  for (int L = 1; L < Lcap; L++) {
    if (!present[L]) continue;
    if (ctx->thr_memo_have[(size_t)L]) { memcpy(&thr[(size_t)L * Ppad], &ctx->thr_memo[(size_t)L * Ppad], (size_t)Ppad * sizeof(uint16_t)); continue; }
    ctx->thr_memo_have[(size_t)L] = 2;
    for (int p = 0; p < P; p++) {
      const HostProfile &h = ctx->profs[p];
      auto passes = [&](int xj) {
        const float usc = msv_score_from_byte(xj, lt[L].tjb);
        const double Pv = gumbel_surv((double)(usc - lt[L].nullsc) / 0.69314718055994529, (double)h.evparam[0], (double)h.evparam[1]);
        return !(Pv > F1);
      };
      int lo = 0, hi = 255;
      if (!passes(254)) { thr[(size_t)L * Ppad + p] = 256; continue; }
      while (lo < hi) { const int mid = (lo + hi) / 2; if (passes(mid)) hi = mid; else lo = mid + 1; }
      thr[(size_t)L * Ppad + p] = (uint16_t)lo;
    }
  }
  for (int L = 1; L < Lcap; L++)
    if (ctx->thr_memo_have[(size_t)L] == 2) { memcpy(&ctx->thr_memo[(size_t)L * Ppad], &thr[(size_t)L * Ppad], (size_t)Ppad * sizeof(uint16_t)); ctx->thr_memo_have[(size_t)L] = 1; }
  DBuf<uint16_t> &d_thr = ctx->w_thr; DBuf<int32_t> &d_tjb = ctx->w_tjb;
  HIPCHK(upload(ctx->d_lt, lt, st)); HIPCHK(upload(d_thr, thr, st)); HIPCHK(upload(d_tjb, tjb, st));

  HIPCHK(hipStreamSynchronize(st));
  if (cells_active_out) *cells_active_out = cells_active;
  return ITSX_OK;
}

static int search_active(itsx_ctx *ctx, double T, double F1, double F2, double F3)
{
  CTXCHK(ctx);
  if (!ctx->have_derep) SET_ERR(ctx, ITSX_E_ARG, "itsx_search called before itsx_derep / itsx_cluster");
  if (ctx->P <= 0) SET_ERR(ctx, ITSX_E_ARG, "no profiles loaded");
  ctx->F2 = F2; ctx->have_vit = F2 < F1;
  ctx->switches_at_search = sw_report();
  HIPCHK(hipSetDevice(ctx->device));
  hipStream_t st = ctx->st;
  const int P = ctx->P, G = ctx->G, Ppad = G * 64, U = ctx->U_active;
  ctx->T = T;
  ctx->h_dom.clear(); ctx->drop_alignments(); ctx->h_trace.clear(); ctx->trace_sorted = false;
  ctx->domz.assign((size_t)P * ctx->S, 0);
  itsx_stats &S = ctx->stats;
  S.n_pairs = (int64_t)U * P; S.n_past_msv = S.n_past_bias = S.n_past_fwd = S.n_regions = S.n_multidomain = S.n_domains = S.n_domain_overflow = 0;
  S.ms_msv = S.ms_filters = S.ms_domains = S.ms_msv_kernel = S.ms_fwd_kernel = S.ms_bwd_kernel = S.ms_env_kernel = S.ms_bias_kernel = S.ms_decode_kernel = 0; S.n_batches = 0; S.ms_ensemble = 0; S.n_mr_clustered = S.n_mr_distinct = S.n_mr_failed = S.n_mr_envelopes = 0; S.n_slab_shrinks = 0; S.n_mr_overflow = 0; S.ms_vit_kernel = 0; for (int k = 0; k < 8; k++) S.n_mr_fail_kind[k] = 0; S.n_rows_resident = 0; S.msv_cells = 0; S.msv_launches = 0; S.fwd_rows = 0; S.env_rows = 0; S.n_env_unique = 0;
  ctx->npairs_padded = 0; ctx->dom_n.clear(); ctx->trace_u0 = 0; ctx->n_chunks = 0;
  ctx->have_search = true; ctx->have_final = false; ctx->domz_on_device = false; ctx->topup.valid = false; ctx->topup.list_live = false; ctx->injected = false;
  const int mode = search_rows_mode(ctx);
  ctx->compact_rows = mode != ITSX_ROWS_FULL;
  ctx->lazy = mode == ITSX_ROWS_LAZY;
  ctx->lazy_pending = 0; ctx->domz_exchanged = false; ctx->sF1 = F1; ctx->sF3 = F3;
  ctx->domz_ub.assign((size_t)P * ctx->S, 0);
  if (ctx->compact_rows)
    for (auto &b : ctx->dom_bufs) if (b && b->cap * sizeof(itsx_domain) > ((size_t)256 << 20)) b->release();
  S.lazy = ctx->lazy; S.n_lazy_evaluated = S.n_lazy_round1 = S.n_lazy_pending = S.n_lazy_reruns = 0; S.n_lazy_completed = S.n_lazy_completed_profiles = S.n_lazy_pending_profiles = 0; S.ms_lazy_complete = 0; S.lazy_bound_maxdiff = 0; S.ms_bound_kernel = S.ms_lazy_select = 0; S.bound_rows = 0; S.n_bound_launches = 0; S.n_lazy_topup = 0; S.ms_lazy_topup = 0; S.ms_lazy_topup_stages = 0; ctx->n_topup_deferred = ctx->n_topup_ensemble = 0;
  if (ctx->compact_rows && U > 0) { const int rc = compact_setup(ctx); if (rc != ITSX_OK) return rc; }
  if (U == 0) return ITSX_OK;

  const int Lcap = ctx->Lmax + 1;
  int64_t cells_active = 0;
  { const int rc = filter_tables(ctx, F1, &cells_active); if (rc != ITSX_OK) return rc; }
  HIPCHK(ctx->d_domz32.alloc((size_t)P * ctx->S));
  HIPCHK(hipMemsetAsync(ctx->d_domz32.p, 0, (size_t)P * ctx->S * 4, st));
  {
    const int64_t cells = cells_active;
    int64_t msum = 0; for (auto &h : ctx->profs) msum += h.M;
    S.msv_cells = cells * msum;
    S.msv_rows = S.msv_rows_full = cells * P; S.bound_rows_full = 0; S.n_share_helpers = 0; S.share_mismatch = 0;
  }
  if (ctx->pair_budget <= 0) {
    size_t fr = 0, tot = 0;
    double gb = 32.0;
    if (hipMemGetInfo(&fr, &tot) == hipSuccess) gb = std::max(1.0, (double)fr / (double)(1ull << 30) / 4.0);
    ctx->pair_budget = (int64_t)(gb * (double)(1ull << 30) / 400.0);
  }
  int64_t lazy_budget = ctx->pair_budget * 5;
  if (ctx->lazy) {
    size_t fr = 0, tot = 0;
// ... 4582 lines not shown
```

### itsxpress_amd/csrc/k_api.h

```cpp
#pragma once
#include "engine.h"

#include "detmath.h"
namespace itsx {

struct ReadsDev {
  const uint32_t *words;
  const int64_t  *woff;
  const int32_t  *len;
  const int64_t  *excoff;
  const uint32_t *exc;
  int64_t         n;
};

void launch_hash_reads(const ReadsDev &rd, uint64_t seed, int strand_both, uint64_t *hf, uint64_t *hr, hipStream_t st, const int32_t *sample = nullptr);
void launch_table_insert(int64_t n, const int32_t *len, int minlen, const uint64_t *hf, const uint64_t *hr,
                         unsigned long long *keys, int32_t *vals, uint64_t mask, uint32_t *slot_of, hipStream_t st);
void launch_table_resolve(const ReadsDev &rd, const uint64_t *hf, const int32_t *vals, const uint32_t *slot_of,
                          int32_t *rep_of, int8_t *strand, int32_t *is_seed, unsigned int *n_collisions, hipStream_t st,
                          const int32_t *sample = nullptr);
void launch_uniques(int64_t n, const int32_t *rep_of, const int32_t *seed_rank, int32_t *uniq_of, int32_t *seed_read,
                    int32_t *abundance, hipStream_t st);
void launch_len_hist(int32_t U, const int32_t *seed_read, const int32_t *len, int32_t *hist, int32_t lcap, hipStream_t st, int32_t nb = 0 );
void launch_len_scatter(int32_t U, const int32_t *seed_read, const int32_t *len, int32_t *cursor, int32_t lcap,
// ... 53 lines not shown
  int32_t *newq, *rm;
  int32_t *xlist, *xn, *hard; unsigned long long *xkey; double *xpid;
  int32_t *work, *xwork, *work_n;
  int32_t *spairs;
  int32_t *awork;
  const uint32_t *dmask;
  const uint64_t *rhash;
  unsigned long long *ctab_key; int32_t *ctab_val; int32_t *canon;
  int32_t *replay;
  int32_t *skipm;
  int32_t *wout;
  int32_t *dbg;
  unsigned long long *scratch; int32_t scratch_pitch;
  double thr;
  unsigned long long *n_align;
  int32_t *need; int32_t need_pitch;
  unsigned long long *n_skipped;
  unsigned long long *pre_stats;
  int32_t pre_k;
  int32_t use_score;
};
constexpr int CL_QS_MAX = 8192;
constexpr int CL_HEAVY = 128;
void launch_cl_segs(const ClusterArgs &a, hipStream_t st);
void launch_cl_kmers(const ClusterArgs &a, hipStream_t st);
void launch_cl_qindex(const ClusterArgs &a, int32_t *scan_tmp, hipStream_t st);
void launch_cl_stream(const ClusterArgs &a, int c0, int c1, int mode, hipStream_t st);
void launch_cl_topk(const ClusterArgs &a, int final, hipStream_t st);
void launch_cl_init(const ClusterArgs &a, hipStream_t st);
void launch_cl_walk(const ClusterArgs &a, int rows_per_lane, hipStream_t st);
void launch_cl_outcome(const ClusterArgs &a, hipStream_t st);
void launch_cl_wsum(const ClusterArgs &a, hipStream_t st);
void launch_cl_columns(const ClusterArgs &a, int clear, hipStream_t st);
void launch_cl_validate(const ClusterArgs &a, int rows_per_lane, hipStream_t st);
void launch_cl_finalize(int32_t nk, const int32_t *order, const int32_t *res_col, const int8_t *res_strand, const double *res_id,
                        const int32_t *cent_read, int32_t *rep_of, int8_t *strand, double *pct, int32_t *is_seed, hipStream_t st);

struct CigarArgs {
  ReadsDev rd;
  const int32_t *q_read, *t_read;
  const int8_t *strand;
  const int64_t *dir_off;
  const int64_t *scr_off;
  uint8_t *dir; long long *scratch;
  long long *res; double *pid;
  int32_t *tlen;
  const int64_t *toff; char *text;
};
void launch_cg_equal(const CigarArgs &a, int32_t n, int32_t *eq, hipStream_t st);
void launch_cg_forward(const CigarArgs &a, int32_t p0, int32_t np, int rows_per_lane, int lmax, hipStream_t st);
void launch_cg_traceback(const CigarArgs &a, int32_t p0, int32_t np, int rows_per_lane, int fill, hipStream_t st);
void cg_pair_bytes(int Lq, int Lt, int rows_per_lane, size_t *dir_bytes, size_t *scr_bytes);

void launch_orient(const ReadsDev &rd, const uint32_t *dbbits , const uint32_t *dmask , int8_t *strand, int32_t *cfwd, int32_t *crev, hipStream_t st);
void launch_dust(const ReadsDev &rd, uint32_t *dmask, hipStream_t st);
int64_t orient_long_table_words(int64_t n_long);
void launch_orient_long(const ReadsDev &rd, const int32_t *list, int64_t n_long, const uint32_t *dbbits, const uint32_t *dmask, uint32_t *tabs,
                        int8_t *strand, int32_t *cfwd, int32_t *crev, hipStream_t st);
struct OrientApplyArgs {
  ReadsDev rd;
  const int8_t *strand;
  const int32_t *sample;
  int64_t *blk;
  int64_t *total;
  int32_t *src;
  int64_t *woff, *excoff;
  int32_t *len, *osample;
  int64_t *sample_count;
  uint32_t *words, *exc;
};
int64_t orient_apply_blocks(int64_t n);
int orient_apply_tile();
void launch_orient_apply_plan(const OrientApplyArgs &a, hipStream_t st);
void launch_orient_apply_scatter(const OrientApplyArgs &a, int64_t m, hipStream_t st);
void launch_op_iota(int32_t *v, int32_t n, hipStream_t st);
void launch_op_verdict(const uint16_t *res_f, const uint16_t *res_r, int32_t cU, int32_t P, const int32_t *sorted, int32_t *ucf, int32_t *ucr,
                       int8_t *ustrand, hipStream_t st);
void launch_op_compose(int64_t n, const int32_t *uniq_of, const int8_t *rstrand, const int32_t *ucf, const int32_t *ucr, const int8_t *ustrand,
                       int8_t *strand, int32_t *cf, int32_t *cr, int8_t *keep, hipStream_t st);

struct MergeArgs {
  const uint8_t *fseq, *fqual, *rseq, *rqual;
  const int64_t *foff, *roff;
  int64_t n;
  int32_t max_total;
  int32_t maxdiffs, allow_stagger; double maxee;
  const double *q2p, *match, *mism;
  const uint8_t *qsame, *qdiff;
  uint8_t *out_seq, *out_qual;
  int32_t *out_len, *reason, *shift; double *score;
  int32_t join; int8_t *joined;
};
void launch_merge(const MergeArgs &a, hipStream_t st);
struct MergeCompactArgs {
  const int32_t *reason, *out_len;
  const int64_t *foff, *roff;
  int64_t n;
  int32_t n_samples;
  const int64_t *pair_start;
  int64_t *blk_cnt, *blk_len;
  int32_t *pair_index;
  int64_t *srcoff, *dstoff;
  int32_t *sample;
  int64_t *sample_count;
  int32_t join;
};
int64_t merge_compact_blocks(int64_t n);
void launch_merge_compact(const MergeCompactArgs &a, int64_t *total, hipStream_t st);

struct alignas(16) TrimRec {
  int64_t out;
  int64_t src;
  int64_t toff;
  int32_t tl, slen;
};
static_assert(sizeof(TrimRec) == 32, "k_trim_copy reads a record as two 16-byte loads");
struct TrimPlanArgs {
  const int32_t *start, *stop; int32_t stride;
  const int64_t *off, *toff;
  int64_t n; int32_t ccs;
  int64_t *blk;
  TrimRec *rec; int64_t *cnt, *tot;
};
int64_t trim_plan_blocks(int64_t n);
void launch_trim_plan(const TrimPlanArgs &a, const int64_t *first, int32_t S, int64_t *bounds, hipStream_t st);
struct TrimCopyArgs {
  const TrimRec *rec; int64_t n;
  const uint8_t *seq, *qual, *titles;
  int64_t total, ntiles; int32_t ccs;
  uint32_t *out;
  const int64_t *qsrc = nullptr;
  const uint8_t *comp = nullptr;
};
int64_t trim_copy_bytes(int64_t total);
void launch_trim_copy(TrimCopyArgs a, hipStream_t st);
struct TrimPairPlanArgs {
  const int32_t *start, *stop, *tlen; int32_t stride;
  const int32_t *pair_read; int64_t n_reads;
  const int64_t *off1, *toff1, *off2, *toff2;
  int64_t n; int32_t ccs;
  int64_t *blk;
  TrimRec *rec1, *rec2; int64_t *cnt;
};
void launch_trim_pair_plan(const TrimPairPlanArgs &a, const int64_t *first, int32_t S, int64_t *bounds, hipStream_t st);
constexpr int TRIM_UNIT_INFO = 8;
struct TrimUnitArgs {
  const uint8_t *text; int64_t nbytes;
  int64_t count;
  int32_t *ls, *le;
  const int32_t *start, *stop;
  const int8_t *strand;
  int32_t mode, ccs;
  int64_t *lblk;
  int64_t *blk;
  TrimRec *rec; int64_t *qsrc;
  int64_t *info;
};
int64_t trim_index_blocks(int64_t nbytes);
void launch_trim_unit(const TrimUnitArgs &a, hipStream_t st);
void launch_trim_orient(const uint8_t *seq, const uint8_t *qual, const int64_t *off, const int32_t *from, const int8_t *strand, const uint8_t *comp,
                        const int64_t *noff, int64_t m, uint8_t *nseq, uint8_t *nqual, hipStream_t st);

constexpr int DEFLATE_BLOCK_BYTES = 65535;
constexpr int DEFLATE_SLOT_BYTES = 65600;
constexpr int DEFLATE_TOKEN_SLOT = 65536;
struct DeflateBlock { int64_t src; int32_t len, pad; };
struct DeflateArgs {
  const uint8_t *text;
  const DeflateBlock *blk; int32_t nblk;
  uint32_t *tokens;
  uint8_t *slots;
  int32_t *sizes;
};
void launch_deflate(const DeflateArgs &a, int grid, hipStream_t st);
void launch_deflate_pack(const uint8_t *slots, const int32_t *sizes, const int64_t *dst, int32_t nblk, uint8_t *out, hipStream_t st);

constexpr int INFLATE_FIND_TILE = 4096;
struct InflateMember { int64_t c, c_end, o; uint32_t isize; int32_t id; };
struct InflateArgs {
  const uint8_t *gz;
  const InflateMember *mem; int32_t nmem;
  uint8_t *text;
  int32_t *status;
  int64_t *where;
};
void launch_inflate_find(const uint8_t *gz, int64_t n, int64_t *counts, const int64_t *base, int64_t *list, hipStream_t st);
void launch_inflate_scan(const int64_t *counts, int64_t ntiles, int64_t *base, int64_t *total, hipStream_t st);
void launch_inflate(const InflateArgs &a, int grid, hipStream_t st);

constexpr int FASTQ_INFO = 8;
struct FastqArgs {
  const uint8_t *text; int64_t nbytes;
  int64_t *lblk;
  int64_t *nl; int64_t nlines, nnl;
  int64_t n;
  int64_t *blk;
  int64_t *off, *toff;
  int64_t *info;
};
int64_t fastq_index_blocks(int64_t nbytes);
int64_t fastq_plan_blocks(int64_t n);
void launch_fastq_count(const FastqArgs &a, hipStream_t st);
void launch_fastq_index(const FastqArgs &a, hipStream_t st);
void launch_fastq_plan(const FastqArgs &a, hipStream_t st);
void launch_fastq_gather(const uint8_t *text, const int64_t *nl, const int64_t *doff, int64_t n, int which, uint8_t *dst, int64_t gbase, int64_t total, hipStream_t st);
struct FastqPairArgs { uint8_t *seq[2]; const uint8_t *qual[2]; int64_t total[2]; const int64_t *off[2]; int64_t n; unsigned long long *info; };
void launch_fastq_pairs(const FastqPairArgs &a, hipStream_t st);

int64_t scan_tmp_elems(int64_t n);
void    launch_exclusive_scan(const int32_t *in, int32_t *out, int64_t n, int32_t *tmp, hipStream_t st);
void    launch_pack(const uint8_t *raw, int64_t raw_base, const int64_t *off, const int64_t *woff, int64_t r0, int64_t r1, const int8_t *lut,
                    uint32_t *words, int32_t *excnt, long long *first_bad, hipStream_t st);
void    launch_pack_exc(const uint8_t *raw, int64_t raw_base, const int64_t *off, int64_t r0, int64_t r1, const int8_t *lut, const int32_t *excnt,
                        const int32_t *exstart, long long *ebase, int64_t ecap, int64_t *excoff, uint32_t *exc, hipStream_t st);
void    launch_calib(int pattern, float *slab, int64_t nwaves, int64_t R, float *out, hipStream_t st);
void    launch_issue(int op, int waves_per_simd, int iters, int blocks, unsigned long long *ticks, float *sink, hipStream_t st);
void    launch_detmath(const double *x, int64_t n, double *ol, double *oe, hipStream_t st);
void    launch_logf_fast(const float *x, int64_t n, const LogTab *tab, float *out, hipStream_t st);

struct TrieArgs {
  ReadsDev rd;
  const int32_t *sorted_uniq, *seed_read;
  int32_t U, Uc, B;
  int32_t rev;
  unsigned long long *tab; uint64_t tmask;
  uint8_t *depth;
  int32_t *parent;
  unsigned long long *mask;
  int32_t *nn;
  unsigned long long *counters;
};
void launch_trie_keycount(const TrieArgs &a, hipStream_t st);
void launch_trie_insert(const TrieArgs &a, hipStream_t st);
void launch_trie_resolve(const TrieArgs &a, hipStream_t st);
void launch_trie_link(const TrieArgs &a, hipStream_t st);
void launch_trie_count(const TrieArgs &a, hipStream_t st);
void launch_share_cuts(const int32_t *ulen, const int32_t *node0_s, const int32_t *rnode0_s , int32_t U, int32_t Uc, int32_t cap,
                       int32_t *cuts , unsigned long long *n, hipStream_t st);
struct PairRec;
void launch_diff_u16(const uint16_t *x, const uint16_t *y, int64_t n, unsigned long long *c, hipStream_t st);
void launch_diff_scores(const float *x, const float *y, const PairRec *pairs, int64_t n, const int32_t *jlev , unsigned long long *c , hipStream_t st);
void launch_popc64(const unsigned long long *m, int32_t *out, int64_t n, int64_t nvalid, hipStream_t st);
constexpr int SHARE_SEGS = 66;
struct ShareDev {
  uint8_t *depth; int32_t *parent ; unsigned long long *mask; int32_t *nn, *node0; int32_t *order , *ulen;
  int32_t *src;
  int32_t *endrow, *jlev, *jsrc;
};
void launch_share_src(const ShareDev &o, int32_t U, int32_t Uc, hipStream_t st);
struct JoinArgs {
  TrieArgs t;
  const uint8_t *fdepth; const unsigned long long *fmask;
  unsigned long long *rmask;
  int32_t *jlev, *jown;
  int32_t *endrow;
  int32_t *rsteps;
  unsigned long long *counters;
};
void launch_join_resolve(const JoinArgs &a, hipStream_t st);
void launch_join_up(const JoinArgs &a, int r, hipStream_t st);
void launch_join_ends(const JoinArgs &a, hipStream_t st);
void launch_order_keys(const uint8_t *depth, const int32_t *minor, const int32_t *runs , int32_t U, const int32_t *bstart, int nb, unsigned long long *keys, int32_t *vals, hipStream_t st);
size_t order_sort_bytes(int64_t n);
int  order_sort(void *tmp, size_t bytes, const unsigned long long *kin, unsigned long long *kout, const int32_t *vin, int32_t *vout, int64_t n, hipStream_t st);
void launch_order_segk(const unsigned long long *sorted_keys, int32_t n, int nb, int32_t *segk , int32_t *inv , const int32_t *vals, int32_t U, unsigned long long *nvalid, hipStream_t st);
void launch_share_permute(const TrieArgs &a, const int32_t *ulen_s, const int32_t *uorder, const int32_t *inv, const int32_t *endrow_s, const int32_t *jlev_s,
                          const ShareDev &o, hipStream_t st);
struct BShareDev {
  uint8_t *depth; int32_t *parent ; unsigned long long *mask; int32_t *nn, *node0; int32_t *order , *ulen;
  int32_t *src;
  int32_t *steps;
};
void launch_bshare_permute(const TrieArgs &a, int32_t Ub, const int32_t *ulen_s, const int32_t *border_s, const int32_t *invb, const unsigned long long *rmask_s,
                           const int32_t *rsteps_s, const BShareDev &o, hipStream_t st);
void launch_bshare_src(const BShareDev &o, int32_t Ub, hipStream_t st);
void launch_join_src(int32_t U, int32_t B, const int32_t *uorder, const int32_t *jown_s, const int32_t *invb, const BShareDev &ob, const ShareDev &o, int32_t *jownb, hipStream_t st);
void launch_join_need(const int32_t *jlev, const int32_t *jownb, int32_t U, int32_t W, int32_t cb0, const uint32_t *pass, uint32_t *need_b, hipStream_t st);
void launch_need_up_b(int r, const uint8_t *rdepth, const int32_t *rparent, int32_t cb0, int32_t Ub, int32_t W, uint32_t *need_b, hipStream_t st);
void launch_need_res(const uint32_t *need_b, int32_t Ub, int32_t P, int32_t W, uint16_t *res, hipStream_t st);
struct ShareLaunch {
  const int32_t *src; const unsigned long long *mask; const int32_t *node0;
  void *slots;
  int64_t node_base; int32_t p0, Pb;
  int32_t depth, logB;
  float rescale;
  const int32_t *endrow, *jlev, *jsrc;
  const void *gslots; int64_t gnode_base;
  const struct ChainRec *chain;
  const float *entab;
  uint32_t *b10; uint8_t *done; unsigned long long *gtop; const int8_t *cls; int32_t ncls;
  int32_t dbg;
};
struct alignas(16) ChainRec {
  int64_t woff, excoff;
  int32_t nexc, L, src, node0;
  unsigned long long mask;
  int32_t endrow;
  int32_t jlev, jsrc, pad;
};
static_assert(sizeof(ChainRec) == 64, "k_fwd_bound / k_bwd_bound read a chain's record as four 16-byte loads");
void launch_chain_recs(int32_t n, const ReadsDev &rd, const int32_t *order , const int32_t *seed_read, const int32_t *src, const int32_t *node0,
                       const unsigned long long *mask, const int32_t *endrow, const int32_t *jlev, const int32_t *jsrc, ChainRec *out, hipStream_t st);
constexpr int MSV_STATE_Q = 8;
constexpr int FWD_STATE_Q = 36;
void launch_need_bits(const uint16_t *res, int32_t U, int32_t P, int32_t W, uint32_t *pass, uint32_t *need, hipStream_t st);
void launch_need_up(int d, const uint8_t *depth, const int32_t *parent, int32_t U, int32_t W, uint32_t *need, hipStream_t st);
void launch_need_mark(uint16_t *res, int32_t U, int32_t P, int32_t W, const uint32_t *pass, const uint32_t *need, unsigned long long *n_helpers, hipStream_t st);
void launch_share_bounds(const PairRec *pairs, const int64_t *seg_start, const int32_t *total, const int32_t *segk, int32_t nseg, int32_t P, int64_t *bnd, hipStream_t st);
void launch_share_wcount(const int64_t *bnd, int32_t nseg, int32_t P, int32_t *wc, hipStream_t st);
struct WaveDesc;
void launch_share_waves(int32_t nw, int32_t nseg, int32_t P, const int32_t *woff, const int64_t *bnd, const int32_t *seg_depth, int32_t B, const PairRec *pairs,
                        const int32_t *endrow , int backward, WaveDesc *w,
                        unsigned long long *lane_rows , hipStream_t st);
void launch_share_wavelist(int32_t nw, int32_t nseg, int32_t P, const int32_t *woff, const int64_t *bnd, WaveDesc *w, hipStream_t st);
void launch_share_rows(int32_t U, int32_t W, const uint32_t *need, const int32_t *ulen, const int32_t *endrow , const int32_t *segk, int32_t nseg,
                       const int32_t *seg_depth, int32_t B, int backward, unsigned long long *lane_rows, hipStream_t st);

struct MsvArgs {
  ReadsDev rd;
  const int32_t *sorted_uniq;
  const int32_t *seed_read;
  int32_t U;
  int32_t G;
  int32_t P;
  int32_t PB;
  const uint32_t *etab;
  const int32_t *pbias, *ptec, *ptbm;
  const uint16_t *thr;
  const int32_t *tjb;
  int32_t Lcap;
  uint16_t *res;
  const int32_t *plist;
  int32_t nlist;
  int32_t k0, k1;
  int32_t pfirst, plast;
  int32_t wtl;
  int32_t wwin;
  unsigned long long *xb_cnt;
  int32_t share;
  ShareLaunch sl;
};
void launch_msv(const MsvArgs &a, hipStream_t st, int lds_pad = 0);
void msv_diag_begin();

constexpr int CHUNK = 2048;
void launch_pair_count(const uint16_t *res, int32_t P, int32_t U, int32_t nchunks, int32_t *cnt , hipStream_t st);
void launch_chunk_scan(int32_t *cnt, int32_t P, int32_t nchunks, int32_t *total , int32_t *real , hipStream_t st);
void launch_pair_fill(const uint16_t *res, int32_t P, int32_t U, int32_t nchunks, const int32_t *cnt,
                      const int64_t *seg_start , const int32_t *total , const int32_t *ulen ,
                      PairRec *pairs, hipStream_t st);
void launch_fill_ulen(int32_t U, const int32_t *sorted_uniq, const int32_t *seed_read, const int32_t *len, int32_t *ulen, hipStream_t st);

struct WaveDesc {
  int32_t prof;
  int32_t count;
  int64_t first;
  int64_t slab;
  int32_t rows;
  int32_t pad;
};
struct VitOut { float vitsc; int32_t ran, pass; };
struct RegionPool { RegionRec *rec; int32_t *k; unsigned long long *n; int64_t cap; };
__device__ __forceinline__ void pool_put(const RegionPool &p, const RegionRec &r, int k)
{
  const unsigned long long i = atomicAdd(p.n, 1ULL);
  if ((int64_t)i < p.cap) { p.rec[i] = r; p.k[i] = k; }
}
struct RegionPoolView { const RegionRec *rec; const unsigned long long *key; int64_t n; };
__device__ __forceinline__ RegionRec raw_region(const RegionRec *raw, const RegionPoolView &pv, int64_t pi, int k)
{
  if (k < MAXDOM) return raw[pi * MAXDOM + k];
  const unsigned long long want = ((unsigned long long)pi << 24) | (unsigned long long)k;
  int64_t lo = 0, hi = pv.n;
  while (lo < hi) { const int64_t mid = (lo + hi) >> 1; if (pv.key[mid] < want) lo = mid + 1; else hi = mid; }
  return pv.rec[lo];
}
struct FloatArgs {
  ReadsDev rd;
  const int32_t *sorted_uniq, *seed_read;
  const DevProfile *prof;
  const LenTables *lt;
  const float *flogsum;
  const LogTab *logtab;
  const PairRec *pairs;
  PairOut *pout;
  const WaveDesc *waves;
  float *slab;
  int64_t slab_plane;
  RegionRec *regions;
  RegionPool pool;
  const VitOut *vit;
  double F1, F3;
};
struct VitArgs {
  ReadsDev rd;
  const int32_t *sorted_uniq, *seed_read;
  const DevProfile *prof;
  const LenTables *lt;
  const PairRec *pairs;
  const PairOut *pout;
  const WaveDesc *waves;
  const int16_t *vtab;
  VitOut *vit;
  int32_t eloop;
  double F2;
};
void launch_vit(const VitArgs &a, int nwaves, int wave0, hipStream_t st);
void launch_bias(const FloatArgs &a, int64_t npairs, hipStream_t st, int lds_pad = 0);
void launch_filters_fwd(const FloatArgs &a, int nwaves, int wave0, int generic_q, hipStream_t st);
void launch_fwd_bound(const FloatArgs &a, float *fb, int nwaves, int wave0, int generic_q, hipStream_t st);
void launch_fwd_bound_seq(const FloatArgs &a, const float *btab, bool fold, float *fb, int nwaves, int wave0, hipStream_t st);
void launch_fwd_bound_share(const FloatArgs &a, const float *btab, bool fold, float *fb, int nwaves, int wave0, const ShareLaunch &sl, hipStream_t st);
void launch_bwd_bound_share(const FloatArgs &a, const float *btab, const float *rtab, int nwaves, int wave0, const ShareLaunch &sl, hipStream_t st);
void launch_bwd_decode(const FloatArgs &a, int nwaves, int wave0, int generic_q, hipStream_t st);
void launch_decode(const FloatArgs &a, int nwaves, int wave0, hipStream_t st);

struct EnvArgs {
  ReadsDev rd;
  const int32_t *sorted_uniq, *seed_read;
  const DevProfile *prof;
  const LenTables *lt;
  const PairRec *pairs;
  const RegionRec *regions;
  RegionOut *rout;
  const WaveDesc *waves;
  float *slab;
};
void launch_envelopes(const EnvArgs &a, int nwaves, int wave0, int generic_q, hipStream_t st);
void launch_align(const EnvArgs &a, itsx_alignment *out, int nwaves, int wave0, int generic_q, hipStream_t st);

constexpr int MRV = 52;
constexpr int MRENV = 4;
#ifndef ITSX_MR_LANES
#define ITSX_MR_LANES 64
#endif
constexpr int MR_LANES = ITSX_MR_LANES;
constexpr int MR_LANES_LONG = 4;
constexpr double MR_LONG_FRAC = 0.02;
constexpr int MR_MAXD = 8;
constexpr int MR_TCAP = 512;
constexpr int MR_SCAP = 200 * MR_MAXD;
constexpr int MR_NSIG = 32;
static_assert(MR_NSIG * 50 >= 200 * MR_MAXD, "MR_NSIG must hold every cluster that can reach 25 % of 200 paths");
constexpr int MR_HASH = 1024;
constexpr int MR_EPC = 256;
constexpr int MR_SCRATCH = 19456;
struct MrRec { int32_t pair, ireg, jreg, slot; };
struct MrOut { int32_t status, nenv; int32_t ei[MRENV], ej[MRENV]; int64_t big; };
struct MrBig { int64_t off, envoff; int32_t capD, capT; uint32_t hmask; int32_t pad; };
struct MrArgs {
  ReadsDev rd;
  const int32_t *sorted_uniq, *seed_read;
  const DevProfile *prof;
  const PairRec *pairs;
  const MrRec *mr;
  const int32_t *ulist;
  int64_t u0;
  const WaveDesc *waves;
  int32_t lds_bytes = 0;
  float4 *slab;
  const int64_t *rowoff;
  int64_t rowoff0;
  const int64_t *n2off;
  float *n2sc;
  MrOut *out;
  uint8_t *scratch;
  const int32_t *sel; const int64_t *sel_rowoff; const MrBig *big; uint8_t *arena;
  int32_t *envpool;
  unsigned long long *dbg;
};
void launch_mr_count(const PairOut *pout, const RegionRec *raw, RegionPoolView pv, int64_t npairs, int32_t *cnt, hipStream_t st);
void launch_mr_fill(const PairOut *pout, const RegionRec *raw, RegionPoolView pv, int64_t npairs, const int32_t *off, MrRec *mr, hipStream_t st);
void launch_mr_ulist(int64_t nmr, const MrRec *mr, const int32_t *rep, const int32_t *is_uniq, const int32_t *urank, int32_t *ulist, int32_t *ulen,
                     int32_t *mr_u, hipStream_t st);
void launch_mr_reorder(int64_t nu, int64_t nmr, const int32_t *newpos, const int32_t *ulist_in, int32_t *ulist_out, int32_t *mr_u, hipStream_t st);
void launch_mr_ensemble(const MrArgs &a, int nwaves, int wave0, hipStream_t st, int64_t one_first = 0, int64_t one_count = 0);
void launch_mr_ensemble_big(const MrArgs &a, int nwaves, hipStream_t st);
void launch_mr_overflowed(const MrOut *out, int64_t nu, int32_t *list, unsigned long long *n, hipStream_t st);
struct RegionListArgs {
  PairOut *pout; const RegionRec *raw; RegionPoolView pv; int64_t npairs;
  const int32_t *mr_off; const int32_t *mr_u; const MrOut *mrout; const int32_t *envpool;
};
void launch_region_list_count(const RegionListArgs &a, int32_t *cnt, unsigned long long *counters, hipStream_t st);
void launch_region_list_fill(const RegionListArgs &a, const int64_t *pair_region0, RegionRec *out, hipStream_t st);

struct ScoreArgs {
  ReadsDev rd;
  const int32_t *sorted_uniq, *seed_read;
  const DevProfile *prof;
  const LenTables *lt;
  const float *flogsum;
  const PairRec *pairs;
  const PairOut *pout;
  const RegionRec *regions;
  const RegionOut *rout;
  const int64_t *pair_region0;
  const int32_t *upos;
  itsx_domain *dom;
  int64_t npairs;
  double T;
  const MrRec *mr; const int32_t *mr_u; const MrOut *mrout; const int64_t *n2off; const float *n2sc; const int32_t *mr_off;
  int32_t *domz;
  const int32_t *usample;
  int32_t P;
};
void launch_score(const ScoreArgs &a, hipStream_t st);
void launch_region_count_fill(const PairOut *pout, const RegionRec *raw, int64_t npairs, const int32_t *pref,
                              const int64_t *seg_pair_start, const int64_t *seg_region_start, const int32_t *seg_of_pair_base,
                              RegionRec *out, hipStream_t st);

__host__ __device__ __forceinline__ unsigned long long rank_key(const itsx_domain &d)
{
  long long tenths = (long long)__builtin_rint((double)d.bitscore * 10.0) + (1ll << 23);
  if (tenths < 0) tenths = 0;
  if (tenths > (1ll << 24) - 1) tenths = (1ll << 24) - 1;
  const unsigned long long di = (unsigned long long)(d.dom_idx < 0 ? 0 : (d.dom_idx > 0xFFFFF ? 0xFFFFF : d.dom_idx));
  return ((unsigned long long)tenths << 40) | ((unsigned long long)(0xFFFFF - (d.prof & 0xFFFFF)) << 20) | (0xFFFFFull - di);
}

constexpr int LAZY_TENTHS_BIAS = 1 << 23;
struct LazyArgs {
  const PairRec *pairs; int64_t NP;
  const float *fb;
  const LenTables *lt;
  const int8_t *cls; int32_t ncls;
  const int32_t *sorted_uniq;
  uint32_t *b10;
  unsigned long long *gtop;
  int64_t ngroups;
  const unsigned long long *bestc;
  int64_t nbest;
  uint32_t *thr; int64_t nthr;
  uint8_t *done;
  unsigned long long *smask;
  int32_t *scnt;
};
void launch_lazy_bound(const LazyArgs &a, hipStream_t st);
void launch_pad_b10(int32_t P, const int64_t *seg_start , const int32_t *total , uint32_t *b10, hipStream_t st);
void launch_lazy_mark(const LazyArgs &a, int round, hipStream_t st);
void launch_lazy_scatter(const PairRec *pairs, int64_t NP, const unsigned long long *smask, const int32_t *spos, const int64_t *seg_old, const int64_t *seg_new,
                         PairRec *out, hipStream_t st, int32_t *src = nullptr );
void launch_finalize_lazy(itsx_domain *dom, int64_t n, const int64_t *zlb, const int64_t *zub, double domE, const int32_t *usample, int P, hipStream_t st);
void launch_lazy_sure(const itsx_domain *dom, int64_t n, const int8_t *cls, int ncls, unsigned long long *sure, int32_t *has, hipStream_t st);
void launch_lazy_pending(const itsx_domain *dom, int64_t n, const int8_t *cls, int ncls, const unsigned long long *sure, const int32_t *has,
                         unsigned long long *count, int32_t *prof_flag, uint8_t *uniq_flag, unsigned long long *zneed , const unsigned long long *zsplit , double domE, hipStream_t st);
void launch_topup_count(const uint8_t *done, const int64_t *seg_start, const int32_t *total, const int32_t *prof_of_slot, int nslots, unsigned long long *cnt, hipStream_t st);
void launch_topup_keys(const PairRec *pairs, int64_t NP, const uint8_t *done, const uint32_t *b10, const int32_t *slot_of_prof, unsigned long long *smask, int32_t *scnt, const int32_t *spos ,
                       unsigned long long *keys, int32_t *vals, hipStream_t st);
void launch_topup_mark(const PairRec *pairs, int64_t NP, uint8_t *done, const uint32_t *b10, const int32_t *slot_of_prof, const uint32_t *cutoff, unsigned long long *smask, int32_t *scnt, hipStream_t st);
void launch_topup_defer(PairOut *pout, const int32_t *mrcnt, const int32_t *src, int64_t npairs, uint8_t *done, unsigned long long *dmask, unsigned long long *n, hipStream_t st);
void launch_topup_count_mask(const unsigned long long *dmask, const int64_t *seg_start, const int32_t *total, const int32_t *prof_of_slot, int nslots, unsigned long long *cnt, hipStream_t st);
void launch_topup_deferred_select(const unsigned long long *dmask, int64_t NP, unsigned long long *smask, int32_t *scnt, uint8_t *done, hipStream_t st);

}
```

### itsxpress_amd/csrc/k_lazy.hip

```cpp
#include "engine.h"
#include "k_api.h"
#include "detmath.h"
#include "k_vec.h"

namespace itsx {

constexpr int BP = BOUND_PAIRS;
typedef const f4 __attribute__((address_space(4))) *cf4q;
struct BT { f2 mm, im, dm, mi, ii, bm, md; float dd1, dd2; };
DEV BT ldbt(const float *tab, int j)
{
  const f4 a = *(cf4q)(uintptr_t)(tab + j * 16), b = *(cf4q)(uintptr_t)(tab + j * 16 + 4), c = *(cf4q)(uintptr_t)(tab + j * 16 + 8),
           d = *(cf4q)(uintptr_t)(tab + j * 16 + 12);
  BT t;
  t.mm = (f2){a.x, a.y}; t.im = (f2){a.z, a.w}; t.dm = (f2){b.x, b.y}; t.ii = (f2){b.z, b.w};
  t.bm = (f2){c.x, c.y}; t.dd1 = c.z; t.dd2 = c.w; t.mi = (f2){d.x, d.y}; t.md = (f2){d.z, d.w};
  return t;
}
DEV f2 pfma(f2 a, f2 b, f2 c) { return __builtin_elementwise_fma(a, b, c); }
DEV uint32_t lazy_tenths(float f, const LenTables &lt)
{
  if (f != f || f == __builtin_inff()) return (1u << 24) - 1;
  if (f == -__builtin_inff()) return 1u;
  const double bits = ((double)f - (double)lt.nullsc) / 0.69314718055994529 + (double)lt.lazy_c;
  double t = __builtin_floor(bits * 10.0 + 0.5) + (double)LAZY_TENTHS_BIAS;
  if (t < 1.0) t = 1.0;
  if (t > (double)((1 << 24) - 1)) t = (double)((1 << 24) - 1);
  return (uint32_t)t;
}
DEV void lazy_bound_put(const ShareLaunch &sl, const LenTables *lt, int64_t pi, const PairRec &pr, float f)
{
  if (pr.xj < 0) { sl.b10[pi] = 0u; sl.done[pi] = 1; return; }
  const uint32_t b = lazy_tenths(f, lt[pr.L]);
  sl.b10[pi] = b;
  atomicMax(&sl.gtop[(size_t)pr.useq * sl.ncls + sl.cls[pr.prof]], ((unsigned long long)b << 32) | (unsigned long long)(0xFFFFFFFFu - (uint32_t)pi));
}
DEV int wave_max(int v)
{
#pragma unroll
  for (int o = 32; o >= 1; o >>= 1) { const int t = __shfl_xor(v, o, 64); v = t > v ? t : v; }
  return uni(v);
}

#ifndef ITSX_FWD_WPB
#define ITSX_FWD_WPB 1
#endif
constexpr int FWD_WPB = ITSX_FWD_WPB;
template <bool SHARE, bool FOLD>
__global__ void __launch_bounds__(64 * FWD_WPB, 2) k_fwd_bound(FloatArgs a, int wave0, int nwaves, const float *__restrict__ btab, float *__restrict__ fb, ShareLaunch sl)
{
  const int wv = threadIdx.x >> 6, widx = blockIdx.x * FWD_WPB + wv;
  WaveDesc wd = a.waves[wave0 + min(widx, nwaves - 1)];
  if (widx >= nwaves) { wd.count = 0; wd.rows = 1; }
  const int lane = threadIdx.x & 63;
  const int prof = uni(wd.prof);
  const DevProfile *pp = a.prof + prof;
  __shared__ __attribute__((aligned(16))) float en_all[FWD_WPB][NCODE * 2 * BP];
  float *en = en_all[wv];
  const float *tab = btab + (size_t)prof * BOUND_TAB;
  const bool active = lane < wd.count;
  const int64_t pi = wd.first + (active ? lane : 0);
  const PairRec pr = a.pairs[pi];
  const int L = pr.L;
  const bool recs = SHARE && sl.chain != nullptr;
  ChainRec cr{};
  if (recs) { const f4 *q = (const f4 *)(sl.chain + pr.useq); const f4 q0 = q[0], q1 = q[1], q2 = q[2], q3 = q[3]; f4 *o = (f4 *)&cr; o[0] = q0; o[1] = q1; o[2] = q2; o[3] = q3; }
  if (FOLD && recs && sl.entab) {
    const f4 *e4 = (const f4 *)(sl.entab + (size_t)prof * (NCODE * 2 * BP));
    for (int i = lane; i < NCODE * 2 * BP / 4; i += 64) ((f4 *)en)[i] = e4[i];
    __builtin_amdgcn_fence(__ATOMIC_RELEASE, "wavefront"); __builtin_amdgcn_wave_barrier(); __builtin_amdgcn_fence(__ATOMIC_ACQUIRE, "wavefront");
  } else {
    const int Q = uni(pp->Q);
    const float *g = tab + (BP + 1) * 16;
    for (int i = lane; i < NCODE * 2 * BP; i += 64) {
      const int x = i / (2 * BP), k0 = i % (2 * BP);
      const float e = (k0 < 4 * Q) ? pp->rf[(x * QMAX + (k0 % Q)) * 4 + k0 / Q] : 0.0f;
      en[i] = FOLD ? e * g[k0] : e;
    }
    __syncthreads();
  }
  Seq sq;
  if (recs) { sq.w = a.rd.words + cr.woff; sq.exc = a.rd.exc + cr.excoff; sq.nexc = cr.nexc; sq.L = cr.L; }
  else sq = open_seq(a.rd, a.seed_read[a.sorted_uniq[pr.useq]]);
  int Lw = wd.rows - 1;
  f2 M[BP], I[BP], D[BP];
#pragma unroll
  for (int j = 0; j < BP; j++) { M[j] = (f2){0.f, 0.f}; I[j] = (f2){0.f, 0.f}; D[j] = (f2){0.f, 0.f}; }
  const float pmove = (2.0f + 1.0f) / ((float)L + 2.0f + 1.0f);
  const float ploop = 1.0f - pmove;
  float xE = 0.f, xN = 1.f, xJ = 0.f, xB = pmove, xC = 0.f;
  double totscale = 0.0;
  const int row0 = SHARE ? (sl.depth << sl.logB) : 0;
  unsigned long long smask = 0ull; int64_t snode = 0;
  int endrow = L, jlev = -1; int64_t jnode = 0;
  if constexpr (SHARE) {
    const int k = pr.useq;
    if (active) {
      if (recs) {
        smask = cr.mask; snode = (int64_t)cr.node0 - sl.node_base;
        endrow = cr.endrow; jlev = pr.xj >= 0 ? cr.jlev : -1; jnode = (int64_t)cr.jsrc - sl.gnode_base;
      } else {
        smask = sl.mask[k]; snode = (int64_t)sl.node0[k] - sl.node_base;
        if (sl.endrow) { endrow = sl.endrow[k]; jlev = pr.xj >= 0 ? sl.jlev[k] : -1; jnode = (int64_t)sl.jsrc[k] - sl.gnode_base; }
      }
    }
    Lw = wave_max(active ? endrow : 0);
    if (sl.dbg & 1) Lw = row0;
    if (sl.dbg & 4) jlev = -1;
    if (sl.depth > 0 && !(sl.dbg & 2)) {
      const int64_t node = (int64_t)(recs ? cr.src : sl.src[k]) - sl.node_base;
      const f4 *src = (const f4 *)sl.slots + (node * sl.Pb + (prof - sl.p0)) * FWD_STATE_Q;
#pragma unroll
      for (int j = 0; j < BP; j++) { const f4 v = src[j]; M[j] = (f2){v.x, v.y}; I[j] = (f2){v.z, v.w}; }
#pragma unroll
      for (int j = 0; j < BP / 2; j++) { const f4 v = src[BP + j]; D[2 * j] = (f2){v.x, v.y}; D[2 * j + 1] = (f2){v.z, v.w}; }
      const f4 u = src[BP + BP / 2], t = src[BP + BP / 2 + 1];
      D[BP - 1] = (f2){u.x, u.y}; xN = u.z; xJ = u.w; xC = t.x; xB = t.y;
      totscale = __builtin_bit_cast(double, (f2){t.z, t.w});
    }
  }
  SeqStream ss; ss.open(sq, row0, +1);
  int xnext = ss.get(row0);
  for (int i = row0 + 1; ; i++) {
    if constexpr (SHARE) {
      if (((i - 1) & ((1 << sl.logB) - 1)) == 0) {
        const int d = (i - 1) >> sl.logB;
        if (d < 64 && ((smask >> d) & 1ull) && i - 1 > row0) {
          const int64_t node = snode + __popcll(smask & ((1ull << d) - 1ull));
          f4 *dst = (f4 *)sl.slots + (node * sl.Pb + (prof - sl.p0)) * FWD_STATE_Q;
#pragma unroll
          for (int j = 0; j < BP; j++) dst[j] = (f4){M[j].x, M[j].y, I[j].x, I[j].y};
#pragma unroll
          for (int j = 0; j < BP / 2; j++) dst[BP + j] = (f4){D[2 * j].x, D[2 * j].y, D[2 * j + 1].x, D[2 * j + 1].y};
          const f2 ts = __builtin_bit_cast(f2, totscale);
          dst[BP + BP / 2] = (f4){D[BP - 1].x, D[BP - 1].y, xN, xJ};
          dst[BP + BP / 2 + 1] = (f4){xC, xB, ts.x, ts.y};
        }
        if (d == jlev) {
          const f4 *g = (const f4 *)sl.gslots + (jnode * sl.Pb + (prof - sl.p0)) * FWD_STATE_Q;
          f2 sa = (f2){0.f, 0.f}, sb = (f2){0.f, 0.f};
#pragma unroll
          for (int j = 0; j < BP; j++) { const f4 v = g[j]; sa = pfma(M[j], (f2){v.x, v.y}, sa); sb = pfma(I[j], (f2){v.z, v.w}, sb); }
#pragma unroll
          for (int j = 0; j < BP / 2; j++) { const f4 v = g[BP + j]; sa = pfma(D[2 * j], (f2){v.x, v.y}, sa); sb = pfma(D[2 * j + 1], (f2){v.z, v.w}, sb); }
          const f4 u = g[BP + BP / 2], t = g[BP + BP / 2 + 1];
          sa = pfma(D[BP - 1], (f2){u.x, u.y}, sa);
          sb = pfma((f2){xN, xJ}, (f2){u.z, u.w}, sb);
          sa = pfma((f2){xC, xB}, (f2){t.x, t.y}, sa);
          const float dot = (sa.x + sa.y) + (sb.x + sb.y);
          const double gscale = __builtin_bit_cast(double, (f2){t.z, t.w});
          const bool jbad = (dot != dot) || (dot <= 0.0f) || (dot == __builtin_inff());
          const float sc = jbad ? __builtin_nanf("") : (float)(totscale + gscale + det_log((double)dot));
          fb[pi] = sc;
          if (sl.b10) lazy_bound_put(sl, a.lt, pi, pr, sc);
        }
      }
    }
    if (i > Lw) break;
    if (i <= endrow) {
      const int x = xnext;
      if (i < L) xnext = ss.get(i);
      const float *ex = en + x * (2 * BP);
      const float *tb = tab + opaque_zero();
      const f2 xBv = (f2){xB, xB};
      f2 acc = (f2){0.f, 0.f};
      float sprev = 0.0f;
      BT cur = ldbt(tb, 0);
      f2 ecur = *(const f2 *)(ex);
      __builtin_amdgcn_s_waitcnt(0xC07F);
      f2 Scur = pfma(M[0], cur.mm, pfma(I[0], cur.im, D[0] * cur.dm));
      if constexpr (FOLD) I[0] = pfma(I[0], cur.ii, M[0]); else I[0] = pfma(M[0], cur.mi, I[0] * cur.ii);
      float dprev = 0.0f, mdprev = 0.0f;
      f2 Sprev = (f2){0.f, 0.f};
      f2 dlast = (f2){0.f, 0.f};
      cur = ldbt(tb, 1);
#define SB __builtin_amdgcn_sched_barrier(0)
#pragma unroll
      for (int j = 0; j < BP; j++) {
        __builtin_amdgcn_s_waitcnt(0xC07F);
        const bool more = j + 1 < BP;
        BT nxt = cur; f2 enxt = ecur;
        if (more) { nxt = ldbt(tb, j + 2); enxt = *(const f2 *)(ex + 2 * (j + 1)); }
        SB;
        const f2 sh = (f2){Sprev.y, Scur.x}; SB;
        f2 t = (f2){0.f, 0.f}, u = t, Sn = Scur;
        if (more) { t = D[j + 1] * cur.dm; SB; }
        f2 dn;
        asm("v_fma_f32 %0, %1, %2, %3" : "=v"(dn.x) : "v"(dprev), "s"(cur.dd1), "v"(mdprev)); SB;
        const f2 w = pfma(xBv, cur.bm, sh); SB;
        if (more) { t = pfma(I[j + 1], cur.im, t); SB; if constexpr (!FOLD) { u = I[j + 1] * cur.ii; SB; } }
        const f2 mn = w * ecur; SB;
        if (more) { Sn = pfma(M[j + 1], cur.mm, t); SB; }
        if constexpr (FOLD) {
          acc = acc + mn; SB;
          if (more) { I[j + 1] = pfma(I[j + 1], cur.ii, M[j + 1]); SB; }
          asm("v_fma_f32 %0, %1, %2, %3" : "=v"(dn.y) : "v"(dn.x), "s"(cur.dd2), "v"(mn.x)); SB;
          mdprev = mn.y;
        } else {
          const f2 md = mn * cur.md; SB;
          acc = acc + mn; SB;
          if (more) { I[j + 1] = pfma(M[j + 1], cur.mi, u); SB; }
          acc = acc + dlast; SB;
          asm("v_fma_f32 %0, %1, %2, %3" : "=v"(dn.y) : "v"(dn.x), "s"(cur.dd2), "v"(md.x)); SB;
          mdprev = md.y; dlast = dn;
        }
        M[j] = mn; D[j] = dn;
        dprev = dn.y;
        Sprev = Scur; Scur = Sn; cur = nxt; ecur = enxt;
      }
#undef SB
      if constexpr (!FOLD) acc = acc + dlast;
      xE = acc.x + acc.y;
      xN = xN * ploop;
      xC = __builtin_fmaf(xC, ploop, xE * 0.5f);
      xJ = __builtin_fmaf(xJ, ploop, xE * 0.5f);
      xB = (xJ + xN) * pmove;
      if (xE > sl.rescale) {
        const float r = 1.0f / xE;
        xN *= r; xC *= r; xJ *= r; xB *= r;
        const f2 rv = (f2){r, r};
#pragma unroll
        for (int j = 0; j < BP; j++) { M[j] = M[j] * rv; I[j] = I[j] * rv; D[j] = D[j] * rv; }
        totscale += det_log((double)xE);
        xE = 1.0f;
      }
    }
  }
  const bool bad = (xC != xC) || (xC == 0.0f) || (xC == __builtin_inff());
  if (active && jlev < 0) {
    const float sc = bad ? __builtin_nanf("") : (float)(totscale + det_log((double)(xC * pmove)));
    fb[pi] = sc;
    if (sl.b10) lazy_bound_put(sl, a.lt, pi, pr, sc);
  }
}

struct RT { f2 mm, im, dm, bm, ii, aa; };
DEV RT ldrt(const float *tab, int j)
{
  const f4 a = *(cf4q)(uintptr_t)(tab + j * 12), b = *(cf4q)(uintptr_t)(tab + j * 12 + 4), c = *(cf4q)(uintptr_t)(tab + j * 12 + 8);
  RT t;
  t.mm = (f2){a.x, a.y}; t.im = (f2){a.z, a.w}; t.dm = (f2){b.x, b.y}; t.bm = (f2){b.z, b.w}; t.ii = (f2){c.x, c.y}; t.aa = (f2){c.z, c.w};
  return t;
}
__global__ void __launch_bounds__(64 * FWD_WPB, 2) k_bwd_bound(FloatArgs a, int wave0, int nwaves, const float *__restrict__ btab, const float *__restrict__ rtab, ShareLaunch sl)
{
  const int wv = threadIdx.x >> 6, widx = blockIdx.x * FWD_WPB + wv;
  WaveDesc wd = a.waves[wave0 + min(widx, nwaves - 1)];
  if (widx >= nwaves) { wd.count = 0; wd.rows = 1; }
  const int lane = threadIdx.x & 63;
  const int prof = uni(wd.prof);
  const DevProfile *pp = a.prof + prof;
  __shared__ __attribute__((aligned(16))) float en_all[FWD_WPB][NCODE * 2 * BP];
  float *en = en_all[wv];
  const float *tab = rtab + (size_t)prof * BOUND_RTAB;
  (void)pp; (void)btab;
  const bool active = lane < wd.count;
  const int64_t pi = wd.first + (active ? lane : 0);
  const PairRec pr = a.pairs[pi];
  const int L = pr.L;
  ChainRec cr;
  { const f4 *q = (const f4 *)(sl.chain + pr.useq); const f4 q0 = q[0], q1 = q[1], q2 = q[2], q3 = q[3]; f4 *o = (f4 *)&cr; o[0] = q0; o[1] = q1; o[2] = q2; o[3] = q3; }
  {
    const f4 *e4 = (const f4 *)(sl.entab + (size_t)prof * (NCODE * 2 * BP));
    for (int i = lane; i < NCODE * 2 * BP / 4; i += 64) ((f4 *)en)[i] = e4[i];
    __builtin_amdgcn_fence(__ATOMIC_RELEASE, "wavefront"); __builtin_amdgcn_wave_barrier(); __builtin_amdgcn_fence(__ATOMIC_ACQUIRE, "wavefront");
  }
  Seq sq; sq.w = a.rd.words + cr.woff; sq.exc = a.rd.exc + cr.excoff; sq.nexc = cr.nexc; sq.L = cr.L;
  const int nsteps = (sl.dbg & 32) ? 0 : wave_max(active ? cr.endrow : 0);
  f2 M[BP], I[BP], D[BP];
#pragma unroll
  for (int j = 0; j < BP; j++) { M[j] = (f2){0.f, 0.f}; I[j] = (f2){0.f, 0.f}; D[j] = (f2){0.f, 0.f}; }
  const float pmove = (2.0f + 1.0f) / ((float)L + 2.0f + 1.0f);
  const float ploop = 1.0f - pmove;
  float xN = 0.f, xJ = 0.f, xB = 0.f, xC = pmove;
  double totscale = 0.0;
  const int kb = pr.useq;
  const int rd = sl.depth;
  unsigned long long smask = 0ull; int64_t snode = 0; int mysteps = 0;
  (void)kb;
  if (active) { smask = cr.mask; snode = (int64_t)cr.node0 - sl.node_base; mysteps = cr.endrow; }
  if (rd > 0 && !(sl.dbg & 16)) {
    const int64_t node = (int64_t)cr.src - sl.node_base;
    const f4 *src = (const f4 *)sl.slots + (node * sl.Pb + (prof - sl.p0)) * FWD_STATE_Q;
#pragma unroll
    for (int j = 0; j < BP; j++) { const f4 v = src[j]; M[j] = (f2){v.x, v.y}; I[j] = (f2){v.z, v.w}; }
#pragma unroll
    for (int j = 0; j < BP / 2; j++) { const f4 v = src[BP + j]; D[2 * j] = (f2){v.x, v.y}; D[2 * j + 1] = (f2){v.z, v.w}; }
    const f4 u = src[BP + BP / 2], t = src[BP + BP / 2 + 1];
    D[BP - 1] = (f2){u.x, u.y}; xN = u.z; xJ = u.w; xC = t.x; xB = t.y;
    totscale = __builtin_bit_cast(double, (f2){t.z, t.w});
  }
  const int A = (L + (1 << sl.logB) - 1) >> sl.logB;
  const int top = (A - rd) << sl.logB;
  const int first = top < L ? top : L;
  SeqStream ss; ss.open(sq, first > 0 ? first - 1 : 0, -1);
  int xnext = first > 0 ? ss.get(first - 1) : 0;
  for (int step = 0; ; step++) {
    if ((step & ((1 << sl.logB) - 1)) == 0 && step > 0) {
      const int rdl = rd + (step >> sl.logB);
      if (active && rdl < 64 && ((smask >> rdl) & 1ull) && !(sl.dbg & 8)) {
        const int64_t node = snode + __popcll(smask & ((1ull << rdl) - 1ull));
        f4 *dst = (f4 *)sl.slots + (node * sl.Pb + (prof - sl.p0)) * FWD_STATE_Q;
#pragma unroll
        for (int j = 0; j < BP; j++) dst[j] = (f4){M[j].x, M[j].y, I[j].x, I[j].y};
#pragma unroll
        for (int j = 0; j < BP / 2; j++) dst[BP + j] = (f4){D[2 * j].x, D[2 * j].y, D[2 * j + 1].x, D[2 * j + 1].y};
        const f2 ts = __builtin_bit_cast(f2, totscale);
        dst[BP + BP / 2] = (f4){D[BP - 1].x, D[BP - 1].y, xN, xJ};
        dst[BP + BP / 2 + 1] = (f4){xC, xB, ts.x, ts.y};
      }
    }
    if (step >= nsteps) break;
    const int row = top - step;
    if (row <= L && step < mysteps) {
      const int x = xnext;
      if (row > 1) xnext = ss.get(row - 2);
      const float *ex = en + x * (2 * BP);
      const float *tb = tab + opaque_zero();
      const float gb0 = xB * pmove;
      const float nJ = xJ + gb0, nN = xN + gb0;
      const float aE = 0.5f * (nJ + xC);
      const f2 aEv = (f2){aE, aE};
      float aDn = 0.0f, wn = 0.0f;
      f2 accB = (f2){0.f, 0.f};
#define SB __builtin_amdgcn_sched_barrier(0)
      const f4 tl = *(cf4q)(uintptr_t)(tb + BP * 12);
      RT cur = ldrt(tb, BP - 1);
      f2 ecur = *(const f2 *)(ex + 2 * (BP - 1));
      __builtin_amdgcn_s_waitcnt(0xC07F);
      float aD2 = __builtin_fmaf(tl.w, aDn, D[BP - 1].y);
      f2 pre = M[BP - 1] + aEv;
      float aD1 = __builtin_fmaf(tl.z, aD2, D[BP - 1].x);
      f2 iig = (f2){tl.x, tl.y} * I[BP - 1];
      f2 aM = pre + (f2){aD2, aDn};
      aDn = aD1;
#pragma unroll
      for (int j = BP - 1; j >= 0; j--) {
        __builtin_amdgcn_s_waitcnt(0xC07F);
        const RT t = cur;
        const f2 e = ecur;
        const bool more = j > 0;
        if (more) { cur = ldrt(tb, j - 1); ecur = *(const f2 *)(ex + 2 * (j - 1)); }
        SB;
        const f2 w = aM * e; SB;
        float aD2n = 0.f, aD1n = 0.f; f2 pren = (f2){0.f, 0.f}, iign = pren, aMn = pren;
        if (more) { aD2n = __builtin_fmaf(t.aa.y, aDn, D[j - 1].y); SB; }
        accB = pfma(t.bm, w, accB); SB;
        if (more) { pren = M[j - 1] + aEv; SB; }
        const f2 wsh = (f2){w.y, wn}; SB;
        if (more) { aD1n = __builtin_fmaf(t.aa.x, aD2n, D[j - 1].x); SB; }
        const f2 gi = I[j];
        M[j] = pfma(t.mm, wsh, gi); SB;
        if (more) { iign = t.ii * I[j - 1]; SB; }
        I[j] = pfma(t.im, wsh, iig); SB;
        if (more) { aMn = pren + (f2){aD2n, aDn}; SB; }
        D[j] = t.dm * wsh; SB;
        wn = w.x; aDn = aD1n; aM = aMn; iig = iign;
      }
#undef SB
      xB = accB.x + accB.y;
      xN = ploop * nN; xJ = ploop * nJ; xC = ploop * xC;
    }
    if ((step & 15) == 15) {
      f2 sm = (f2){0.f, 0.f};
#pragma unroll
      for (int j = 0; j < BP; j++) sm = sm + ((M[j] + I[j]) + D[j]);
      const float tot = (sm.x + sm.y) + ((xN + xJ) + (xC + xB));
      if (tot > 1e6f || (tot < 1e-6f && tot > 0.0f)) {
        const float r = 1.0f / tot;
        const f2 rv = (f2){r, r};
#pragma unroll
        for (int j = 0; j < BP; j++) { M[j] = M[j] * rv; I[j] = I[j] * rv; D[j] = D[j] * rv; }
        xN *= r; xJ *= r; xC *= r; xB *= r;
        totscale += det_log((double)tot);
      }
    }
  }
}
void launch_bwd_bound_share(const FloatArgs &a, const float *btab, const float *rtab, int nwaves, int wave0, const ShareLaunch &sl, hipStream_t st)
{
  if (nwaves <= 0) return;
  const dim3 g((nwaves + FWD_WPB - 1) / FWD_WPB), b(64 * FWD_WPB);
  hipLaunchKernelGGL(k_bwd_bound, g, b, 0, st, a, wave0, nwaves, btab, rtab, sl);
}

static float bound_rescale()
{
  static const float v = [] { const char *e = sw_get("ITSX_BOUND_RESCALE_EXP"); const double x = e ? atof(e) : 20.0; return (float)pow(10.0, x < 4.0 ? 4.0 : x > 28.0 ? 28.0 : x); }();
  return v;
}
void launch_fwd_bound_seq(const FloatArgs &a, const float *btab, bool fold, float *fb, int nwaves, int wave0, hipStream_t st)
{
  if (nwaves <= 0) return;
  ShareLaunch none{}; none.rescale = bound_rescale();
  const dim3 g((nwaves + FWD_WPB - 1) / FWD_WPB), b(64 * FWD_WPB);
  if (fold) hipLaunchKernelGGL((k_fwd_bound<false, true>), g, b, 0, st, a, wave0, nwaves, btab, fb, none);
  else hipLaunchKernelGGL((k_fwd_bound<false, false>), g, b, 0, st, a, wave0, nwaves, btab, fb, none);
}
void launch_fwd_bound_share(const FloatArgs &a, const float *btab, bool fold, float *fb, int nwaves, int wave0, const ShareLaunch &sl0, hipStream_t st)
{
  if (nwaves <= 0) return;
  ShareLaunch sl = sl0; sl.rescale = bound_rescale();
  const dim3 g((nwaves + FWD_WPB - 1) / FWD_WPB), b(64 * FWD_WPB);
  if (fold) hipLaunchKernelGGL((k_fwd_bound<true, true>), g, b, 0, st, a, wave0, nwaves, btab, fb, sl);
  else hipLaunchKernelGGL((k_fwd_bound<true, false>), g, b, 0, st, a, wave0, nwaves, btab, fb, sl);
}

__global__ void __launch_bounds__(256) k_lazy_bound(LazyArgs a)
{
  const int64_t i = (int64_t)blockIdx.x * blockDim.x + threadIdx.x;
  if (i >= a.NP) return;
  const PairRec pr = a.pairs[i];
  if (pr.prof < 0) { a.b10[i] = 0u; return; }
  if (pr.xj < 0) { a.b10[i] = 0u; a.done[i] = 1; return; }
  const uint32_t b = lazy_tenths(a.fb[i], a.lt[pr.L]);
  a.b10[i] = b;
  const size_t g = (size_t)pr.useq * a.ncls + a.cls[pr.prof];
  atomicMax(&a.gtop[g], ((unsigned long long)b << 32) | (unsigned long long)(0xFFFFFFFFu - (uint32_t)i));
}

__device__ __forceinline__ void select_store(int64_t i, int64_t nch, int f, unsigned long long *__restrict__ smask, int32_t *__restrict__ scnt)
{
  const unsigned long long m = __ballot(f);
  if ((threadIdx.x & 63) == 0) {
    const int64_t c = i >> 6;
    if (c < nch) smask[c] = m;
    scnt[c] = (int32_t)__popcll(m);
  }
}

__global__ void __launch_bounds__(256) k_lazy_first(LazyArgs a)
{
  const int64_t g = (int64_t)blockIdx.x * blockDim.x + threadIdx.x;
  if (g >= a.ngroups) return;
  const unsigned long long top = a.gtop[g];
  const int64_t i = (int64_t)(0xFFFFFFFFu - (uint32_t)(top & 0xFFFFFFFFull));
  if (i >= a.NP) return;
  const PairRec pr = a.pairs[i];
  if (pr.prof < 0 || a.done[i] || (int64_t)pr.useq * a.ncls + a.cls[pr.prof] != g) return;
  a.done[i] = 1;
  atomicOr(&a.smask[i >> 6], 1ull << (i & 63));
}
__global__ void __launch_bounds__(256) k_select_count(const unsigned long long *__restrict__ smask, int64_t nch, int32_t *__restrict__ scnt)
{
  const int64_t c = (int64_t)blockIdx.x * blockDim.x + threadIdx.x;
  if (c <= nch) scnt[c] = c < nch ? (int32_t)__popcll(smask[c]) : 0;
}
__global__ void __launch_bounds__(256) k_lazy_thr(LazyArgs a)
{
  const int64_t g = (int64_t)blockIdx.x * blockDim.x + threadIdx.x;
  if (g >= a.nthr) return;
  const int64_t su = a.sorted_uniq[g / a.ncls], idx = su * a.ncls + g % a.ncls;
  const unsigned long long bc = (su >= 0 && idx < a.nbest) ? a.bestc[idx] : 0ull;
  a.thr[g] = (uint32_t)(bc >> 40);
}
constexpr int MARK_K = 4;
static inline unsigned select_grid(int64_t NP) { const int64_t nw = (((NP + 63) >> 6) + 1 + MARK_K - 1) / MARK_K; return (unsigned)((nw + 3) / 4); }
__global__ void __launch_bounds__(256) k_lazy_mark(LazyArgs a)
{
  const int lane = threadIdx.x & 63;
  const int64_t nch = (a.NP + 63) >> 6;
  const int64_t c0 = ((int64_t)blockIdx.x * 4 + (threadIdx.x >> 6)) * MARK_K;
  if (c0 > nch) return;
  PairRec pr[MARK_K]; uint8_t dn[MARK_K]; uint32_t b[MARK_K], t[MARK_K]; int cl[MARK_K]; bool live[MARK_K];
#pragma unroll
  for (int k = 0; k < MARK_K; k++) {
    const int64_t i = (c0 + k) * 64 + lane;
    pr[k].useq = 0; pr[k].prof = -1; pr[k].xj = -1; pr[k].L = 0; dn[k] = 1; b[k] = 0;
    if (i < a.NP) { pr[k] = a.pairs[i]; dn[k] = a.done[i]; b[k] = a.b10[i]; }
  }
#pragma unroll
  for (int k = 0; k < MARK_K; k++) {
    live[k] = pr[k].prof >= 0 && !dn[k];
    cl[k] = 0;
    if (live[k]) cl[k] = a.cls[pr[k].prof];
  }
#pragma unroll
  for (int k = 0; k < MARK_K; k++) { t[k] = 0u; if (live[k]) t[k] = a.thr[(size_t)pr[k].useq * a.ncls + cl[k]]; }
#pragma unroll
  for (int k = 0; k < MARK_K; k++) {
    const int64_t c = c0 + k;
    if (c > nch) break;
    const int f = live[k] && b[k] >= t[k];
    if (f) a.done[c * 64 + lane] = 1;
    select_store(c * 64 + lane, nch, f, a.smask, a.scnt);
  }
}

constexpr int SCATTER_CHUNKS = 16;
__global__ void __launch_bounds__(256) k_lazy_scatter(const PairRec *__restrict__ pairs, int64_t NP, const unsigned long long *__restrict__ smask,
                                                      const int32_t *__restrict__ spos, const int64_t *__restrict__ seg_old,
                                                      const int64_t *__restrict__ seg_new, PairRec *__restrict__ out, int32_t *__restrict__ src)
{
  const int lane = threadIdx.x & 63;
  const int64_t nch = (NP + 63) >> 6;
  const int64_t c0 = ((int64_t)blockIdx.x * 4 + (threadIdx.x >> 6)) * SCATTER_CHUNKS;
  for (int k = 0; k < SCATTER_CHUNKS; k++) {
    const int64_t c = c0 + k;
    if (c >= nch) return;
    const unsigned long long m = smask[c];
    if (!((m >> lane) & 1ull)) continue;
    const int64_t i = c * 64 + lane;
    const PairRec pr = pairs[i];
    const int32_t rank = spos[c] + (int32_t)__popcll(m & ((1ull << lane) - 1ull)) - spos[seg_old[pr.prof] >> 6];
    out[seg_new[pr.prof] + (int64_t)rank] = pr;
    if (src) src[seg_new[pr.prof] + (int64_t)rank] = (int32_t)i;
  }
}

__global__ void __launch_bounds__(256) k_finalize_lazy(itsx_domain *__restrict__ dom, int64_t n, const int64_t *__restrict__ zlb,
                                                       const int64_t *__restrict__ zub, double domE, const int32_t *__restrict__ usample, int P)
{
  const int64_t i = (int64_t)blockIdx.x * blockDim.x + threadIdx.x;
  if (i >= n) return;
  const itsx_domain d = dom[i];
  if (d.dom_idx < 0) return;
  int rep = 0;
  if (d.seq_reported) {
    const size_t z = (size_t)(usample ? usample[d.rep] * P : 0) + d.prof;
    const double p = det_exp(d.lnP);
    const double lo = (double)(zlb[z] > 1 ? zlb[z] : 1), hi = (double)(zub[z] > 1 ? zub[z] : 1);
    rep = (p * hi <= domE) ? 1 : (p * lo <= domE) ? 2 : 0;
  }
  dom[i].dom_reported = rep;
}

__global__ void __launch_bounds__(256) k_lazy_sure(const itsx_domain *__restrict__ dom, int64_t n, const int8_t *__restrict__ cls, int ncls,
                                                   unsigned long long *__restrict__ sure, int32_t *__restrict__ has)
{
  const int64_t i = (int64_t)blockIdx.x * blockDim.x + threadIdx.x;
  if (i >= n) return;
  const itsx_domain d = dom[i];
  if (d.dom_idx < 0 || d.dom_reported != 1) return;
  has[d.rep] = 1;
  atomicMax(&sure[(size_t)d.rep * ncls + cls[d.prof]], rank_key(d));
}
__global__ void __launch_bounds__(256) k_lazy_pending(const itsx_domain *__restrict__ dom, int64_t n, const int8_t *__restrict__ cls, int ncls,
                                                      const unsigned long long *__restrict__ sure, const int32_t *__restrict__ has,
                                                      unsigned long long *__restrict__ count, int32_t *__restrict__ prof_flag,
                                                      uint8_t *__restrict__ uniq_flag, unsigned long long *__restrict__ zneed, const unsigned long long *__restrict__ zsplit,
                                                      double domE)
{
  const int64_t i = (int64_t)blockIdx.x * blockDim.x + threadIdx.x;
  int c = 0;
  if (i < n) {
    const itsx_domain d = dom[i];
    if (d.dom_idx >= 0 && d.dom_reported == 2) c = !has[d.rep] || rank_key(d) > sure[(size_t)d.rep * ncls + cls[d.prof]];
    if (c) {
      prof_flag[d.prof] = 1; uniq_flag[d.rep] = 1;
      if (zneed) {
        const double z = domE / det_exp(d.lnP);
        if (z < 9.0e18) {
          const unsigned long long zf = (unsigned long long)z;
          if (zf + 2ull <= zsplit[d.prof]) atomicMax(&zneed[2 * d.prof], zf + 2ull);
          else atomicMin(&zneed[2 * d.prof + 1], zf > 2ull ? zf - 2ull : 0ull);
        } else atomicMin(&zneed[2 * d.prof + 1], (unsigned long long)9.0e18);
      }
    }
  }
  const unsigned long long m = __ballot(c);
  if (m && (threadIdx.x & 63) == (unsigned)__builtin_ctzll(m)) atomicAdd(count, (unsigned long long)__builtin_popcountll(m));
}

__global__ void __launch_bounds__(64) k_pad_b10(const int64_t *__restrict__ seg_start, const int32_t *__restrict__ total, uint32_t *__restrict__ b10)
{
  const int64_t e = seg_start[blockIdx.x] + total[blockIdx.x] + threadIdx.x;
  if (e < seg_start[blockIdx.x + 1]) b10[e] = 0u;
}
void launch_pad_b10(int32_t P, const int64_t *seg_start, const int32_t *total, uint32_t *b10, hipStream_t st)
{
  if (P > 0) hipLaunchKernelGGL(k_pad_b10, dim3((unsigned)P), dim3(64), 0, st, seg_start, total, b10);
}
void launch_lazy_bound(const LazyArgs &a, hipStream_t st)
{
  if (a.NP > 0) hipLaunchKernelGGL(k_lazy_bound, dim3((unsigned)((a.NP + 255) / 256)), dim3(256), 0, st, a);
}
void launch_lazy_mark(const LazyArgs &a, int round, hipStream_t st)
{
  const int64_t nch = (a.NP + 63) >> 6;
  if (round == 0) {
    (void)hipMemsetAsync(a.smask, 0, (size_t)nch * sizeof(unsigned long long), st);
    if (a.ngroups > 0) hipLaunchKernelGGL(k_lazy_first, dim3((unsigned)((a.ngroups + 255) / 256)), dim3(256), 0, st, a);
    hipLaunchKernelGGL(k_select_count, dim3((unsigned)((nch + 1 + 255) / 256)), dim3(256), 0, st, a.smask, nch, a.scnt);
  } else {
    if (a.nthr > 0) hipLaunchKernelGGL(k_lazy_thr, dim3((unsigned)((a.nthr + 255) / 256)), dim3(256), 0, st, a);
    hipLaunchKernelGGL(k_lazy_mark, dim3(select_grid(a.NP)), dim3(256), 0, st, a);
  }
}
void launch_lazy_scatter(const PairRec *pairs, int64_t NP, const unsigned long long *smask, const int32_t *spos, const int64_t *seg_old, const int64_t *seg_new,
                         PairRec *out, hipStream_t st, int32_t *src)
{
  const int64_t nch = (NP + 63) >> 6, per_block = 4 * SCATTER_CHUNKS;
  if (NP > 0) hipLaunchKernelGGL(k_lazy_scatter, dim3((unsigned)((nch + per_block - 1) / per_block)), dim3(256), 0, st, pairs, NP, smask, spos, seg_old, seg_new, out, src);
}
void launch_finalize_lazy(itsx_domain *dom, int64_t n, const int64_t *zlb, const int64_t *zub, double domE, const int32_t *usample, int P, hipStream_t st)
{
  if (n > 0) hipLaunchKernelGGL(k_finalize_lazy, dim3((unsigned)((n + 255) / 256)), dim3(256), 0, st, dom, n, zlb, zub, domE, usample, P);
}
void launch_lazy_sure(const itsx_domain *dom, int64_t n, const int8_t *cls, int ncls, unsigned long long *sure, int32_t *has, hipStream_t st)
{
  if (n > 0) hipLaunchKernelGGL(k_lazy_sure, dim3((unsigned)((n + 255) / 256)), dim3(256), 0, st, dom, n, cls, ncls, sure, has);
}
void launch_lazy_pending(const itsx_domain *dom, int64_t n, const int8_t *cls, int ncls, const unsigned long long *sure, const int32_t *has,
                         unsigned long long *count, int32_t *prof_flag, uint8_t *uniq_flag, unsigned long long *zneed, const unsigned long long *zsplit, double domE, hipStream_t st)
{
  if (n > 0) hipLaunchKernelGGL(k_lazy_pending, dim3((unsigned)((n + 255) / 256)), dim3(256), 0, st, dom, n, cls, ncls, sure, has, count, prof_flag, uniq_flag, zneed, zsplit, domE);
}
__global__ void __launch_bounds__(256) k_topup_count(const uint8_t *__restrict__ done, const int64_t *__restrict__ seg_start, const int32_t *__restrict__ total,
                                                     const int32_t *__restrict__ prof_of_slot, unsigned long long *__restrict__ cnt)
{
  const int sl = blockIdx.y, p = prof_of_slot[sl];
  const int64_t base = seg_start[p], n = total[p];
  unsigned long long c = 0;
  for (int64_t i = (int64_t)blockIdx.x * 256 + threadIdx.x; i < n; i += (int64_t)gridDim.x * 256) c += done[base + i] != 0;
  for (int o = 32; o >= 1; o >>= 1) c += __shfl_xor(c, o, 64);
  if ((threadIdx.x & 63) == 0 && c) atomicAdd(&cnt[sl], c);
}
void launch_topup_count(const uint8_t *done, const int64_t *seg_start, const int32_t *total, const int32_t *prof_of_slot, int nslots, unsigned long long *cnt, hipStream_t st)
{
  if (nslots > 0) hipLaunchKernelGGL(k_topup_count, dim3(512, (unsigned)nslots), dim3(256), 0, st, done, seg_start, total, prof_of_slot, cnt);
}

__global__ void __launch_bounds__(256) k_topup_keys(const PairRec *__restrict__ pairs, int64_t NP, const uint8_t *__restrict__ done, const uint32_t *__restrict__ b10,
                                                    const int32_t *__restrict__ slot_of_prof, unsigned long long *__restrict__ smask, int32_t *__restrict__ scnt,
                                                    const int32_t *__restrict__ spos, unsigned long long *__restrict__ keys, int32_t *__restrict__ vals)
{
  const int lane = threadIdx.x & 63;
  const int64_t nch = (NP + 63) >> 6;
  const int64_t c0 = ((int64_t)blockIdx.x * 4 + (threadIdx.x >> 6)) * MARK_K;
  if (c0 > nch) return;
  if (!spos) {
    PairRec pr[MARK_K]; uint8_t dn[MARK_K];
#pragma unroll
    for (int k = 0; k < MARK_K; k++) {
      const int64_t i = (c0 + k) * 64 + lane;
      pr[k].useq = 0; pr[k].prof = -1; pr[k].xj = -1; pr[k].L = 0; dn[k] = 1;
      if (i < NP) { pr[k] = pairs[i]; dn[k] = done[i]; }
    }
    int sl[MARK_K];
#pragma unroll
    for (int k = 0; k < MARK_K; k++) { sl[k] = -1; if (pr[k].prof >= 0 && pr[k].xj >= 0 && !dn[k]) sl[k] = slot_of_prof[pr[k].prof]; }
#pragma unroll
    for (int k = 0; k < MARK_K; k++) {
      if (c0 + k > nch) break;
      select_store((c0 + k) * 64 + lane, nch, sl[k] >= 0, smask, scnt);
    }
    return;
  }
  unsigned long long m[MARK_K];
#pragma unroll
  for (int k = 0; k < MARK_K; k++) m[k] = c0 + k < nch ? smask[c0 + k] : 0ull;
#pragma unroll
  for (int k = 0; k < MARK_K; k++) {
    if (!((m[k] >> lane) & 1ull)) continue;
    const int64_t i = (c0 + k) * 64 + lane;
    const int32_t at = spos[c0 + k] + (int32_t)__popcll(m[k] & ((1ull << lane) - 1ull));
    const int sl = slot_of_prof[pairs[i].prof];
    keys[at] = ((unsigned long long)sl << 32) | (unsigned long long)(0xFFFFFFFFu - b10[i]); vals[at] = (int32_t)i;
  }
}
__global__ void __launch_bounds__(256) k_topup_mark(const PairRec *__restrict__ pairs, int64_t NP, uint8_t *__restrict__ done, const uint32_t *__restrict__ b10,
                                                    const int32_t *__restrict__ slot_of_prof, const uint32_t *__restrict__ cutoff,
                                                    unsigned long long *__restrict__ smask, int32_t *__restrict__ scnt)
{
  const int lane = threadIdx.x & 63;
  const int64_t nch = (NP + 63) >> 6;
  const int64_t c0 = ((int64_t)blockIdx.x * 4 + (threadIdx.x >> 6)) * MARK_K;
  if (c0 > nch) return;
  PairRec pr[MARK_K]; uint8_t dn[MARK_K]; uint32_t b[MARK_K];
#pragma unroll
  for (int k = 0; k < MARK_K; k++) {
    const int64_t i = (c0 + k) * 64 + lane;
    pr[k].useq = 0; pr[k].prof = -1; pr[k].xj = -1; pr[k].L = 0; dn[k] = 1; b[k] = 0;
    if (i < NP) { pr[k] = pairs[i]; dn[k] = done[i]; b[k] = b10[i]; }
  }
  int sl[MARK_K];
#pragma unroll
  for (int k = 0; k < MARK_K; k++) { sl[k] = -1; if (pr[k].prof >= 0 && pr[k].xj >= 0 && !dn[k]) sl[k] = slot_of_prof[pr[k].prof]; }
  uint32_t hi[MARK_K], lo[MARK_K];
#pragma unroll
  for (int k = 0; k < MARK_K; k++) { hi[k] = 0; lo[k] = 0; if (sl[k] >= 0) { hi[k] = cutoff[2 * sl[k]]; lo[k] = cutoff[2 * sl[k] + 1]; } }
#pragma unroll
  for (int k = 0; k < MARK_K; k++) {
    if (c0 + k > nch) break;
    const int f = (hi[k] > 0 && b[k] >= hi[k]) || (lo[k] > 0 && b[k] <= lo[k]);
    if (f) done[(c0 + k) * 64 + lane] = 1;
    select_store((c0 + k) * 64 + lane, nch, f, smask, scnt);
  }
}
void launch_topup_keys(const PairRec *pairs, int64_t NP, const uint8_t *done, const uint32_t *b10, const int32_t *slot_of_prof, unsigned long long *smask, int32_t *scnt,
                       const int32_t *spos, unsigned long long *keys, int32_t *vals, hipStream_t st)
{
// ... 54 lines not shown
```

### itsxpress_amd/csrc/switches.cpp

```cpp
#include "switches.h"
#include <cstdlib>
#include <cstring>

namespace itsx {

static const Switch g_sw[] = {
  {"ITSX_NO_ENSEMBLE", SW_HOOK, "multidomain regions keep their region as one envelope instead of hmmsearch's stochastic-traceback clustering (changes envelopes)"},
  {"ITSX_LAZY_ZUB_SCALE", SW_HOOK, "multiplies the lazy stage's upper bound on domZ: more undecided rows for the completion tests"},
  {"ITSX_LAZY_FORCE_PENDING", SW_HOOK, "treats rows as undecided so that the completion path runs"},
  {"ITSX_LAZY_NO_RERUN", SW_HOOK, "skips the full re-search safety net (leaves undecided rows undecided)"},
  {"ITSX_LAZY_NO_COMPLETE", SW_HOOK, "skips itsx_lazy_complete inside itsx_search_finalize (leaves undecided rows undecided)"},
  {"ITSX_COMPACT_ZMAX", SW_HOOK, "largest domZ the compact / lazy modes call a row 'certain' for (default 1e9); a value below the data's domZ can drop a winner"},
  {"ITSX_COMPACT_DOME_MIN", SW_HOOK, "smallest --domE the compact / lazy modes call a row 'certain' for (default 1e-2)"},
  {"ITSX_PASSA_DBG", SW_HOOK, "pass A diagnostic bits (no rows / no restore / no join): timings only, scores are garbage; 64: the shared MSV kernel counts its floored wave-rows, those with the xB branch and its waves by word layout (results unchanged; one stderr line per search)"},
  {"ITSX_MSV_PB", SW_HOOK, "profiles one block of the MSV filter takes its sequences through (1 .. 32; default: by the job's size, 1 for a small job): same cells"},
  {"ITSX_TWRITER_HOST_SLICE", SW_HOOK, "=1: a streamed writer with a device (itsx_twriter_set_device) slices every unit on the host, as it does a unit its line index does not fit (same file bytes)"},
  {"ITSX_TOPUP_FORCE_SECOND", SW_HOOK, "=1: the top-up round's second sub-round (the deferred pairs through the ensemble stage) runs as if the count-only sub-round had left rows undecided (same rows)"},
  {"ITSX_ROWS", SW_MODE, "rows mode when the caller did not call itsx_set_rows_mode: full | compact | lazy (coordinates identical in all three)"},
  {"ITSX_COMPACT_ROWS", SW_MODE, "=1: rows mode compact (older spelling of ITSX_ROWS=compact)"},
  {"ITSX_QMASK", SW_MODE, "=none: vsearch's --qmask none for cluster_size / orient seeds (default dust, as vsearch)"},
  {"ITSX_KEEP_TRACE", SW_MODE, "keeps per-pair filter traces for itsx_get_pairtraces (forces the compact path of a lazy search)"},
  {"ITSX_GZIP_LEVEL", SW_MODE, "deflate level of the trimmed-FASTQ writers (default 6; output bytes differ, records do not)"},
  {"ITSX_DEVICE_DEFLATE", SW_MODE, "=1: the batch writers deflate gzip output on the device, and so do the outputs a StreamEngine plans (output bytes differ, records do not)"},
  {"ITSX_SHARE_SAMPLES", SW_MODE, "=1: every context shares the HMM stages across the samples of a batch, as after itsx_set_sample_sharing(ctx, 1) (full rows mode, S > 1; same rows, counters, coordinates and files)"},
  {"ITSX_SHARE_SAMPLES_LAZY", SW_MODE, "=1: every context shares the HMM stages across the samples of a batch in the compact and lazy rows modes, as after itsx_set_sample_sharing_lazy(ctx, 1) (S > 1; same coordinates and files, valid domZ bounds)"},
  {"ITSX_TEST_HOOKS", SW_DIAG, "=1: honour the HOOK switches above"},
  {"ITSX_SHARE_CHECK", SW_DIAG, "runs the unshared kernels beside the shared ones and counts differences (itsx_stats.share_mismatch, join_maxdiff)"},
  {"ITSX_LAZY_CHECK_BOUND", SW_DIAG, "compares pass A's scores with HMMER's own Forward arithmetic (itsx_stats.lazy_bound_maxdiff)"},
  {"ITSX_LAZY_HIST", SW_DIAG, "prints the histogram of round-2 candidates per group"},
  {"ITSX_PASSA_DUMP", SW_DIAG, "prints every pass-A launch's waves and wave-rows (scripts/passa_launches.py)"},
  {"ITSX_TRACE_ALLOC", SW_DIAG, "prints every hipMalloc / free with its time"},
  {"ITSX_CL_DEBUG", SW_DIAG, "clustering: prints per-window counters"},
  {"ITSX_MR_DEBUG", SW_DIAG, "ensemble stage: prints per-batch counters"},
  {"ITSX_SHARE", SW_TUNING, "=0: no prefix sharing (round 4's schedule)"},
  {"ITSX_SHARE_TWO", SW_TUNING, "=0: one-sided (prefix-only) sharing for pass A"},
  {"ITSX_MSV_TWO", SW_TUNING, "=0: the MSV filter keeps the one-sided (prefix-only) schedule when pass A shares two-sidedly"},
  {"ITSX_SHARE_B", SW_TUNING, "rows per block of the prefix / suffix trees (default 32)"},
  {"ITSX_SHARE_GB", SW_TUNING, "budget of the saved row states, GB"},
  {"ITSX_SHARE_MIN", SW_TUNING, "smallest shared-row fraction for which the shared schedule is used (default 0.10)"},
  {"ITSX_SHARE_FWD_STREAMS", SW_TUNING, "1 | 2 streams for pass A's batches"},
  {"ITSX_SHARE_MSV_STREAMS", SW_TUNING, "1 | 2 streams for the MSV filter's batches"},
  {"ITSX_NO_CHAINREC", SW_TUNING, "pass A reads a chain's data through the round-5 arrays instead of its 64-byte record (A/B)"},
  {"ITSX_BOUND_FOLD", SW_TUNING, "=0: pass A's plain recurrences instead of the folded ones (also switches two-sided sharing off)"},
  {"ITSX_BOUND_RESCALE_EXP", SW_TUNING, "power of ten at which pass A rescales a row (default 20)"},
  {"ITSX_LAZY_TOPUP", SW_TUNING, "=0: undecided rows go straight to the full count of their profiles (no top-up round); =2: the round also looks for unreported pairs among a profile's weakest (rows settled from above)"},
  {"ITSX_LAZY_EXACT_BOUND", SW_TUNING, "pass A through the HMMER-order Forward kernel (A/B)"},
  {"ITSX_CHUNK_UNIQUES", SW_TUNING, "representatives per search chunk"},
  {"ITSX_MSV_OVERLAP", SW_TUNING, "=0: the next chunk's MSV filter does not run beside the domain stage"},
  {"ITSX_MSV_PAD", SW_TUNING, "dynamic LDS of the overlapped MSV launch (an occupancy cap)"},
  {"ITSX_MSV_WHOLE", SW_TUNING, "where the MSV filter keeps a lane's packed words: 2 (default) shared chains keep their wave's window of at most 16 words, loaded once per block; 1 the whole read when the launch's longest fits 37 words, as the unshared kernel always does; 0 16 words at a time everywhere (A/B arms: same cells; read at every launch)"},
  {"ITSX_MSV_FLOOR", SW_TUNING, "=0: the MSV filter's plain three-instruction row on every row instead of the floored two-instruction one (A/B arm: same cells; read at every launch)"},
  {"ITSX_BIAS_OVERLAP", SW_TUNING, "=0: the bias filter does not run on the second stream"},
  {"ITSX_ST2_PRIO", SW_TUNING, "priority of the second stream"},
  {"ITSX_LOAD_PRIORITY", SW_TUNING, "=0: loads do not use the high-priority stream"},
  {"ITSX_SLAB_GB", SW_TUNING, "DP slab budget, GB"},
  {"ITSX_SLAB_ADAPT", SW_TUNING, "=0: the slab budget does not adapt to the job"},
  {"ITSX_ALIGN_SLAB_MB", SW_TUNING, "itsx_align_domains: slab budget of one batch of waves, MB (default 4096; a small value forces several batches: same alignments)"},
  {"ITSX_DEFER_FREE_GB", SW_TUNING, "device memory kept on the deferred-free list, GB"},
  {"ITSX_MR_LONG_FRAC", SW_TUNING, "ensemble stage: share of regions taken as 'long'"},
  {"ITSX_MR_LONG_LANES", SW_TUNING, "ensemble stage: lanes per long region"},
  {"ITSX_MSV_BWD_WHOLE", SW_TUNING, "=1: the MSV filter's Backward chains copy their whole read to LDS first (A/B arm: same cells)"},
  {"ITSX_LAZY_TOPUP_ALL", SW_TUNING, "=0: a profile whose undecided rows need most of its pairs is left to the full count (itsx_lazy_complete) instead of taking all its unevaluated pairs in the top-up round; =2 (with the count-only round): such a profile takes what its row needs like any other, and its remaining pairs follow in a count-only sub-round of their own only if the row is still undecided (same coordinates; read at every call)"},
  {"ITSX_TOPUP_COUNT_ONLY", SW_TUNING, "=0: the top-up round sends its pairs through the whole domain pipeline like a third lazy round (rows kept, an ensemble invocation of its own) instead of counting reported targets only and deferring the pairs with a multidomain region (A/B arm and cross-check: same coordinates)"},
  {"ITSX_MR_WAVES", SW_TUNING, "ensemble stage: waves a batch is spread over (lanes per wave = regions / this, 2 .. 64); 0 = waves of 64 lanes"},
  {"ITSX_MR_ONE_MAX", SW_TUNING, "ensemble stage: a batch of at most this many regions (default 2048) is walked one region per wave with the matrix in LDS; 0 = never"},
  {"ITSX_CIGAR_MB", SW_TUNING, "itsx_align_clusters: byte budget of one batch of pairs (direction bits and border rows), MB (default 2048; a small value forces several batches, and a pair larger than it runs alone: same alignments)"},
  {"ITSX_CL_NOSCORE", SW_TUNING, "clustering: skips the score-only pre-pass (A/B arm; the walk then aligns every candidate: same outcomes)"},
  {"ITSX_CL_NOPRECHECK", SW_TUNING, "clustering: skips the certificate pre-check (A/B arm: same outcomes)"},
  {"ITSX_CL_CAPACITY", SW_TUNING, "clustering: candidate-list capacity"},
  {"ITSX_CL_CCAP", SW_TUNING, "clustering: centroid capacity step"},
  {"ITSX_CL_HEAVY", SW_TUNING, "clustering: heavy-word split on / off"},
  {"ITSX_CL_HEAVY_MIN", SW_TUNING, "clustering: centroids a word needs to count as conserved"},
  {"ITSX_CL_ROWS", SW_TUNING, "clustering: alignment rows per lane"},
  {"ITSX_CL_WINDOW", SW_TUNING, "clustering: queries per speculative window"},
  {"ITSX_PACK_CHUNK", SW_TUNING, "reads per packing launch"},
  {"ITSX_PACK_ECAP", SW_TUNING, "initial capacity of the exception list"},
  {"ITSX_HUGEPAGES", SW_TUNING, "=0: host buffers without MADV_HUGEPAGE"},
  {"ITSX_IO_LIBDEFLATE", SW_TUNING, "=0: zlib instead of libdeflate when both are present"},
  {"ITSX_IO_THREADS", SW_TUNING, "host threads of the FASTQ readers / writers"},
  {"ITSX_IO_BLOCK_KB", SW_TUNING, "deflate unit of the block-parallel writer"},
  {"ITSX_DEVICE_INFLATE", SW_TUNING, "=1: the whole-file loaders of every context try a gzip file of independent members on the device first (same text; read at every load)"},
  {"ITSX_INFLATE_MEMBER_KB", SW_TUNING, "longest compressed member the device inflate takes (default 8192: twice the host writer's block); a file with a longer one is the host's"},
  {"ITSX_INFLATE_GRID", SW_TUNING, "most workgroups of the device inflate's launch (default: four per CU, what their LDS allows); fewer: each decodes more members in a row (same text)"},
  {"ITSX_DEVICE_PARSE", SW_TUNING, "=1: the whole-file loaders and the paired merge loaders of every context parse FASTQ text on the device (same reads; a text it declines is the host parser's; read at every load)"},
  {"ITSX_PARALLEL_INFLATE", SW_TUNING, "=0: single-stream inflate"},
  {"ITSX_PINFLATE_CHUNK_KB", SW_TUNING, "chunk of the block-parallel inflater"},
  {"ITSX_PARSE_MIN_MB", SW_TUNING, "smallest text parsed on several threads"},
  {"ITSX_TEXT_CACHE_GB", SW_TUNING, "inflated-text cache, GB"},
  {"ITSX_WRITE_MIN_MB", SW_TUNING, "smallest output written by several threads"},
  {"ITSX_WRITE_UNIT_KB", SW_TUNING, "unit of the streamed writer"},
  {"ITSX_STREAM_RESERVE_MB", SW_TUNING, "streamed loads: first reservation"},
  {"ITSX_STREAM_RESERVE_X", SW_TUNING, "streamed loads: growth factor"},
};
static const int g_nsw = (int)(sizeof(g_sw) / sizeof(g_sw[0]));

const Switch *sw_registry(int *n) { if (n) *n = g_nsw; return g_sw; }

static bool hooks_on() { const char *e = sw_get("ITSX_TEST_HOOKS"); return e && atoi(e) == 1; }

const char *sw_get(const char *name)
{
  const char *v = getenv(name);
  if (!v) return nullptr;
  for (int i = 0; i < g_nsw; i++)
    if (strcmp(g_sw[i].name, name) == 0) return (g_sw[i].kind == SW_HOOK && !hooks_on()) ? nullptr : v;
  return nullptr;
}

std::string sw_report()
{
  std::string out;
  const bool on = hooks_on();
  for (int i = 0; i < g_nsw; i++) {
    const char *v = getenv(g_sw[i].name);
    if (!v) continue;
    out += g_sw[i].name; out += "="; out += v;
    if (g_sw[i].kind == SW_HOOK && !on) out += " (ignored: ITSX_TEST_HOOKS is not 1)";
    out += "\n";
  }
  return out;
}

}
```

Before: 4.895 million.

## Carry two state vectors per pair in bound forward/backward kernels, shrinking saved states

The forward and backward bound kernels now keep two register arrays per column pair (a combined M+D score and the insert state) instead of three (M, I, D). Per-row work is redistributed: the loop runs one extra step and finishes the previous pair's update while starting the next, and the host tables are reindexed to match. This cuts register pressure and the saved prefix/suffix row state from 36 to 25 float4 per profile, so fewer bytes are written and read and more nodes fit in the budget. It also replaces the fixed min-2 launch bound with a waves-per-EU attribute of 3, and adds a tuning switch for the state budget divisor. The risks are changed floating-point summation order and spills if 3 waves per EU is too tight.

Result: faster. 5.121 million, median of 6 (+4.6%).

```diff
diff --git a/itsxpress_amd/csrc/engine.h b/itsxpress_amd/csrc/engine.h
--- a/itsxpress_amd/csrc/engine.h
+++ b/itsxpress_amd/csrc/engine.h
@@ -17,7 +17,7 @@
 constexpr int MSV_TW = 24;
 constexpr int MAXDOM = 8;
 constexpr int BOUND_PAIRS = 23;
-constexpr int BOUND_RTAB = BOUND_PAIRS * 12 + 4;
+constexpr int BOUND_RTAB = (BOUND_PAIRS + 1) * 12;
 constexpr int BOUND_TAB = (BOUND_PAIRS + 1) * 16 + 2 * BOUND_PAIRS + 2;
 
 struct HostProfile {
diff --git a/itsxpress_amd/csrc/engine.hip b/itsxpress_amd/csrc/engine.hip
--- a/itsxpress_amd/csrc/engine.hip
+++ b/itsxpress_amd/csrc/engine.hip
@@ -699,16 +699,16 @@
       auto rk = [&](int k) { return fold && k >= 1 && k <= KK ? RI[(size_t)i][(size_t)k] : 1.0; };
       for (int j = 0; j <= BOUND_PAIRS; j++) {
         float *o = bt.data() + (size_t)i * BOUND_TAB + (size_t)j * 16;
-        if (j < BOUND_PAIRS) {
-          const int k1 = 2 * j + 1, k2 = 2 * j + 2;
+        if (j > 0) {
+          const int k1 = 2 * (j - 1) + 1, k2 = 2 * (j - 1) + 2;
           o[0] = (float)(tn(k1 + 1, 1) / gk(k1)); o[1] = (float)(tn(k2 + 1, 1) / gk(k2));
           o[2] = (float)(tn(k1 + 1, 2) * rk(k1)); o[3] = (float)(tn(k2 + 1, 2) * rk(k2));
           o[4] = (float)(tn(k1 + 1, 3) * sk(k1)); o[5] = (float)(tn(k2 + 1, 3) * sk(k2));
           o[6] = tn(k1, 6); o[7] = tn(k2, 6);
           o[12] = (float)(tn(k1, 5) / gk(k1)); o[13] = (float)(tn(k2, 5) / gk(k2));
         }
-        if (j > 0) {
-          const int k1 = 2 * (j - 1) + 1, k2 = 2 * (j - 1) + 2;
+        if (j < BOUND_PAIRS) {
+          const int k1 = 2 * j + 1, k2 = 2 * j + 2;
           o[8] = tn(k1, 0); o[9] = tn(k2, 0);
           if (fold) { o[10] = k1 > 1 ? (float)AA[(size_t)i][(size_t)k1 - 1] : 0.0f; o[11] = (float)AA[(size_t)i][(size_t)k1]; }
           else { o[10] = tn(k1 - 1, 7); o[11] = tn(k1, 7); }
@@ -724,16 +724,13 @@
       const float *b = bt.data() + (size_t)i * BOUND_TAB;
       for (int j = 0; j <= BOUND_PAIRS; j++) {
         float *o = rt.data() + (size_t)i * BOUND_RTAB + (size_t)j * 12;
-        if (j < BOUND_PAIRS) {
-          for (int q = 0; q < 6; q++) o[q] = b[(size_t)j * 16 + q];
-          o[6] = b[(size_t)(j + 1) * 16 + 8]; o[7] = b[(size_t)(j + 1) * 16 + 9];
-        }
+        if (j < BOUND_PAIRS) { o[6] = b[(size_t)j * 16 + 8]; o[7] = b[(size_t)j * 16 + 9]; }
         if (j >= 1) {
           const int jj = j - 1;
-          float *q = j < BOUND_PAIRS ? o + 8 : o;
-          q[0] = b[(size_t)jj * 16 + 6]; q[1] = b[(size_t)jj * 16 + 7];
-          q[2] = b[(size_t)(jj + 1) * 16 + 11];
-          q[3] = (jj + 2 <= BOUND_PAIRS) ? b[(size_t)(jj + 2) * 16 + 10] : 0.0f;
+          for (int q = 0; q < 6; q++) o[q] = b[(size_t)(jj + 1) * 16 + q];
+          o[8] = b[(size_t)(jj + 1) * 16 + 6]; o[9] = b[(size_t)(jj + 1) * 16 + 7];
+          o[10] = b[(size_t)jj * 16 + 11];
+          o[11] = (jj + 1 < BOUND_PAIRS) ? b[(size_t)(jj + 1) * 16 + 10] : 0.0f;
         }
       }
     }
@@ -2033,7 +2030,9 @@
   if (const char *e = sw_get("ITSX_SHARE_GB")) gb = std::max(0.0001, atof(e));
   const bool two_fwd = sw_get("ITSX_SHARE_FWD_STREAMS") ? atoi(sw_get("ITSX_SHARE_FWD_STREAMS")) >= 2 : (U < 2000000 && !sw_get("ITSX_SHARE_GB"));
   const double state_b = fwd_too ? (two_fwd ? 2.0 : 1.0) * (double)FWD_STATE_Q * sizeof(float4) : 2.0 * (double)MSV_STATE_Q * sizeof(uint4);
-  if (!sw_get("ITSX_SHARE_GB")) gb = std::min(gb, std::max(1.0, (double)((int64_t)NN + NG) * state_b * (double)P / (double)(1ull << 30) / 3.8));
+  double share_div = 3.8, share_floor = 1.0;
+  if (const char *e = sw_get("ITSX_SHARE_DIV")) { share_div = std::min(16.0, std::max(1.0, atof(e))); share_floor = 0.0001; }
+  if (!sw_get("ITSX_SHARE_GB")) gb = std::min(gb, std::max(share_floor, (double)((int64_t)NN + NG) * state_b * (double)P / (double)(1ull << 30) / share_div));
   if (gb > 1.0) gb = floor(gb * 2.0) / 2.0;
   const int64_t nodes_max = std::max<int64_t>(1, (int64_t)(gb * (double)(1ull << 30) / (state_b * (double)P)));
   std::vector<int32_t> bstart; std::vector<itsx_ctx::ShareBatch> &bt = ctx->sh_batches;
diff --git a/itsxpress_amd/csrc/k_api.h b/itsxpress_amd/csrc/k_api.h
--- a/itsxpress_amd/csrc/k_api.h
+++ b/itsxpress_amd/csrc/k_api.h
@@ -379,7 +379,7 @@
 void launch_chain_recs(int32_t n, const ReadsDev &rd, const int32_t *order , const int32_t *seed_read, const int32_t *src, const int32_t *node0,
                        const unsigned long long *mask, const int32_t *endrow, const int32_t *jlev, const int32_t *jsrc, ChainRec *out, hipStream_t st);
 constexpr int MSV_STATE_Q = 8;
-constexpr int FWD_STATE_Q = 36;
+constexpr int FWD_STATE_Q = 25;
 void launch_need_bits(const uint16_t *res, int32_t U, int32_t P, int32_t W, uint32_t *pass, uint32_t *need, hipStream_t st);
 void launch_need_up(int d, const uint8_t *depth, const int32_t *parent, int32_t U, int32_t W, uint32_t *need, hipStream_t st);
 void launch_need_mark(uint16_t *res, int32_t U, int32_t P, int32_t W, const uint32_t *pass, const uint32_t *need, unsigned long long *n_helpers, hipStream_t st);
diff --git a/itsxpress_amd/csrc/k_lazy.hip b/itsxpress_amd/csrc/k_lazy.hip
--- a/itsxpress_amd/csrc/k_lazy.hip
+++ b/itsxpress_amd/csrc/k_lazy.hip
@@ -46,8 +46,12 @@
 #define ITSX_FWD_WPB 1
 #endif
 constexpr int FWD_WPB = ITSX_FWD_WPB;
+#ifndef ITSX_BOUND_WAVES
+#define ITSX_BOUND_WAVES 3
+#endif
+#define BOUND_OCC __attribute__((amdgpu_waves_per_eu(ITSX_BOUND_WAVES, ITSX_BOUND_WAVES)))
 template <bool SHARE, bool FOLD>
-__global__ void __launch_bounds__(64 * FWD_WPB, 2) k_fwd_bound(FloatArgs a, int wave0, int nwaves, const float *__restrict__ btab, float *__restrict__ fb, ShareLaunch sl)
+__global__ void __launch_bounds__(64 * FWD_WPB) BOUND_OCC k_fwd_bound(FloatArgs a, int wave0, int nwaves, const float *__restrict__ btab, float *__restrict__ fb, ShareLaunch sl)
 {
   const int wv = threadIdx.x >> 6, widx = blockIdx.x * FWD_WPB + wv;
   WaveDesc wd = a.waves[wave0 + min(widx, nwaves - 1)];
@@ -83,9 +87,9 @@
   if (recs) { sq.w = a.rd.words + cr.woff; sq.exc = a.rd.exc + cr.excoff; sq.nexc = cr.nexc; sq.L = cr.L; }
   else sq = open_seq(a.rd, a.seed_read[a.sorted_uniq[pr.useq]]);
   int Lw = wd.rows - 1;
-  f2 M[BP], I[BP], D[BP];
-#pragma unroll
-  for (int j = 0; j < BP; j++) { M[j] = (f2){0.f, 0.f}; I[j] = (f2){0.f, 0.f}; D[j] = (f2){0.f, 0.f}; }
+  f2 S[BP], Ip[BP];
+#pragma unroll
+  for (int j = 0; j < BP; j++) { S[j] = (f2){0.f, 0.f}; Ip[j] = (f2){0.f, 0.f}; }
   const float pmove = (2.0f + 1.0f) / ((float)L + 2.0f + 1.0f);
   const float ploop = 1.0f - pmove;
   float xE = 0.f, xN = 1.f, xJ = 0.f, xB = pmove, xC = 0.f;
@@ -111,12 +115,10 @@
       const int64_t node = (int64_t)(recs ? cr.src : sl.src[k]) - sl.node_base;
       const f4 *src = (const f4 *)sl.slots + (node * sl.Pb + (prof - sl.p0)) * FWD_STATE_Q;
 #pragma unroll
-      for (int j = 0; j < BP; j++) { const f4 v = src[j]; M[j] = (f2){v.x, v.y}; I[j] = (f2){v.z, v.w}; }
-#pragma unroll
-      for (int j = 0; j < BP / 2; j++) { const f4 v = src[BP + j]; D[2 * j] = (f2){v.x, v.y}; D[2 * j + 1] = (f2){v.z, v.w}; }
-      const f4 u = src[BP + BP / 2], t = src[BP + BP / 2 + 1];
-      D[BP - 1] = (f2){u.x, u.y}; xN = u.z; xJ = u.w; xC = t.x; xB = t.y;
-      totscale = __builtin_bit_cast(double, (f2){t.z, t.w});
+      for (int j = 0; j < BP; j++) { const f4 v = src[j]; S[j] = (f2){v.x, v.y}; Ip[j] = (f2){v.z, v.w}; }
+      const f4 u = src[BP], t = src[BP + 1];
+      xN = u.x; xJ = u.y; xC = u.z; xB = u.w;
+      totscale = __builtin_bit_cast(double, (f2){t.x, t.y});
     }
   }
   SeqStream ss; ss.open(sq, row0, +1);
@@ -129,26 +131,21 @@
           const int64_t node = snode + __popcll(smask & ((1ull << d) - 1ull));
           f4 *dst = (f4 *)sl.slots + (node * sl.Pb + (prof - sl.p0)) * FWD_STATE_Q;
 #pragma unroll
-          for (int j = 0; j < BP; j++) dst[j] = (f4){M[j].x, M[j].y, I[j].x, I[j].y};
-#pragma unroll
-          for (int j = 0; j < BP / 2; j++) dst[BP + j] = (f4){D[2 * j].x, D[2 * j].y, D[2 * j + 1].x, D[2 * j + 1].y};
+          for (int j = 0; j < BP; j++) dst[j] = (f4){S[j].x, S[j].y, Ip[j].x, Ip[j].y};
           const f2 ts = __builtin_bit_cast(f2, totscale);
-          dst[BP + BP / 2] = (f4){D[BP - 1].x, D[BP - 1].y, xN, xJ};
-          dst[BP + BP / 2 + 1] = (f4){xC, xB, ts.x, ts.y};
+          dst[BP] = (f4){xN, xJ, xC, xB};
+          dst[BP + 1] = (f4){ts.x, ts.y, 0.f, 0.f};
         }
         if (d == jlev) {
           const f4 *g = (const f4 *)sl.gslots + (jnode * sl.Pb + (prof - sl.p0)) * FWD_STATE_Q;
           f2 sa = (f2){0.f, 0.f}, sb = (f2){0.f, 0.f};
 #pragma unroll
-          for (int j = 0; j < BP; j++) { const f4 v = g[j]; sa = pfma(M[j], (f2){v.x, v.y}, sa); sb = pfma(I[j], (f2){v.z, v.w}, sb); }
-#pragma unroll
-          for (int j = 0; j < BP / 2; j++) { const f4 v = g[BP + j]; sa = pfma(D[2 * j], (f2){v.x, v.y}, sa); sb = pfma(D[2 * j + 1], (f2){v.z, v.w}, sb); }
-          const f4 u = g[BP + BP / 2], t = g[BP + BP / 2 + 1];
-          sa = pfma(D[BP - 1], (f2){u.x, u.y}, sa);
-          sb = pfma((f2){xN, xJ}, (f2){u.z, u.w}, sb);
-          sa = pfma((f2){xC, xB}, (f2){t.x, t.y}, sa);
+          for (int j = 0; j < BP; j++) { const f4 v = g[j]; sa = pfma(S[j], (f2){v.x, v.y}, sa); sb = pfma(Ip[j], (f2){v.z, v.w}, sb); }
+          const f4 u = g[BP], t = g[BP + 1];
+          sb = pfma((f2){xN, xJ}, (f2){u.x, u.y}, sb);
+          sa = pfma((f2){xC, xB}, (f2){u.z, u.w}, sa);
           const float dot = (sa.x + sa.y) + (sb.x + sb.y);
-          const double gscale = __builtin_bit_cast(double, (f2){t.z, t.w});
+          const double gscale = __builtin_bit_cast(double, (f2){t.x, t.y});
           const bool jbad = (dot != dot) || (dot <= 0.0f) || (dot == __builtin_inff());
           const float sc = jbad ? __builtin_nanf("") : (float)(totscale + gscale + det_log((double)dot));
           fb[pi] = sc;
@@ -164,52 +161,39 @@
       const float *tb = tab + opaque_zero();
       const f2 xBv = (f2){xB, xB};
       f2 acc = (f2){0.f, 0.f};
-      float sprev = 0.0f;
       BT cur = ldbt(tb, 0);
       f2 ecur = *(const f2 *)(ex);
-      __builtin_amdgcn_s_waitcnt(0xC07F);
-      f2 Scur = pfma(M[0], cur.mm, pfma(I[0], cur.im, D[0] * cur.dm));
-      if constexpr (FOLD) I[0] = pfma(I[0], cur.ii, M[0]); else I[0] = pfma(M[0], cur.mi, I[0] * cur.ii);
       float dprev = 0.0f, mdprev = 0.0f;
-      f2 Sprev = (f2){0.f, 0.f};
-      f2 dlast = (f2){0.f, 0.f};
-      cur = ldbt(tb, 1);
+      float sprev = 0.0f;
+      f2 mnp = (f2){0.f, 0.f}, dnp = mnp;
 #define SB __builtin_amdgcn_sched_barrier(0)
 #pragma unroll
-      for (int j = 0; j < BP; j++) {
+      for (int j = 0; j <= BP; j++) {
         __builtin_amdgcn_s_waitcnt(0xC07F);
-        const bool more = j + 1 < BP;
-        BT nxt = cur; f2 enxt = ecur;
-        if (more) { nxt = ldbt(tb, j + 2); enxt = *(const f2 *)(ex + 2 * (j + 1)); }
+        const bool chain = j < BP, fin = j > 0;
+        const BT c = cur; const f2 e = ecur;
+        if (chain) { cur = ldbt(tb, j + 1); if (j + 1 < BP) ecur = *(const f2 *)(ex + 2 * (j + 1)); }
         SB;
-        const f2 sh = (f2){Sprev.y, Scur.x}; SB;
-        f2 t = (f2){0.f, 0.f}, u = t, Sn = Scur;
-        if (more) { t = D[j + 1] * cur.dm; SB; }
-        f2 dn;
-        asm("v_fma_f32 %0, %1, %2, %3" : "=v"(dn.x) : "v"(dprev), "s"(cur.dd1), "v"(mdprev)); SB;
-        const f2 w = pfma(xBv, cur.bm, sh); SB;
-        if (more) { t = pfma(I[j + 1], cur.im, t); SB; if constexpr (!FOLD) { u = I[j + 1] * cur.ii; SB; } }
-        const f2 mn = w * ecur; SB;
-        if (more) { Sn = pfma(M[j + 1], cur.mm, t); SB; }
+        f2 sh = (f2){0.f, 0.f}, t = sh, u = sh, w = sh, mn = sh, md = sh, dn = sh;
+        if (chain) { sh = (f2){sprev, S[j].x}; sprev = S[j].y; SB; }
+        if (fin) { t = Ip[j - 1] * c.im; SB; if constexpr (!FOLD) { u = Ip[j - 1] * c.ii; SB; } }
+        if (chain) { asm("v_fma_f32 %0, %1, %2, %3" : "=v"(dn.x) : "v"(dprev), "s"(c.dd1), "v"(mdprev)); SB; }
+        if (chain) { w = pfma(xBv, c.bm, sh); SB; }
+        if (fin) { t = pfma(dnp, c.dm, t); SB; }
+        if (chain) { mn = w * e; SB; }
+        if (fin) { S[j - 1] = pfma(mnp, c.mm, t); SB; }
         if constexpr (FOLD) {
-          acc = acc + mn; SB;
-          if (more) { I[j + 1] = pfma(I[j + 1], cur.ii, M[j + 1]); SB; }
-          asm("v_fma_f32 %0, %1, %2, %3" : "=v"(dn.y) : "v"(dn.x), "s"(cur.dd2), "v"(mn.x)); SB;
-          mdprev = mn.y;
+          if (chain) { acc = acc + mn; SB; }
+          if (fin) { Ip[j - 1] = pfma(Ip[j - 1], c.ii, mnp); SB; }
+          if (chain) { asm("v_fma_f32 %0, %1, %2, %3" : "=v"(dn.y) : "v"(dn.x), "s"(c.dd2), "v"(mn.x)); SB; mdprev = mn.y; }
         } else {
-          const f2 md = mn * cur.md; SB;
-          acc = acc + mn; SB;
-          if (more) { I[j + 1] = pfma(M[j + 1], cur.mi, u); SB; }
-          acc = acc + dlast; SB;
-          asm("v_fma_f32 %0, %1, %2, %3" : "=v"(dn.y) : "v"(dn.x), "s"(cur.dd2), "v"(md.x)); SB;
-          mdprev = md.y; dlast = dn;
+          if (chain) { md = mn * c.md; SB; acc = acc + mn; SB; }
+          if (fin) { Ip[j - 1] = pfma(mnp, c.mi, u); SB; acc = acc + dnp; SB; }
+          if (chain) { asm("v_fma_f32 %0, %1, %2, %3" : "=v"(dn.y) : "v"(dn.x), "s"(c.dd2), "v"(md.x)); SB; mdprev = md.y; }
         }
-        M[j] = mn; D[j] = dn;
-        dprev = dn.y;
-        Sprev = Scur; Scur = Sn; cur = nxt; ecur = enxt;
+        mnp = mn; dnp = dn; dprev = dn.y;
       }
 #undef SB
-      if constexpr (!FOLD) acc = acc + dlast;
       xE = acc.x + acc.y;
       xN = xN * ploop;
       xC = __builtin_fmaf(xC, ploop, xE * 0.5f);
@@ -220,7 +204,7 @@
         xN *= r; xC *= r; xJ *= r; xB *= r;
         const f2 rv = (f2){r, r};
 #pragma unroll
-        for (int j = 0; j < BP; j++) { M[j] = M[j] * rv; I[j] = I[j] * rv; D[j] = D[j] * rv; }
+        for (int j = 0; j < BP; j++) { S[j] = S[j] * rv; Ip[j] = Ip[j] * rv; }
         totscale += det_log((double)xE);
         xE = 1.0f;
       }
@@ -242,7 +226,7 @@
   t.mm = (f2){a.x, a.y}; t.im = (f2){a.z, a.w}; t.dm = (f2){b.x, b.y}; t.bm = (f2){b.z, b.w}; t.ii = (f2){c.x, c.y}; t.aa = (f2){c.z, c.w};
   return t;
 }
-__global__ void __launch_bounds__(64 * FWD_WPB, 2) k_bwd_bound(FloatArgs a, int wave0, int nwaves, const float *__restrict__ btab, const float *__restrict__ rtab, ShareLaunch sl)
+__global__ void __launch_bounds__(64 * FWD_WPB) BOUND_OCC k_bwd_bound(FloatArgs a, int wave0, int nwaves, const float *__restrict__ btab, const float *__restrict__ rtab, ShareLaunch sl)
 {
   const int wv = threadIdx.x >> 6, widx = blockIdx.x * FWD_WPB + wv;
   WaveDesc wd = a.waves[wave0 + min(widx, nwaves - 1)];
@@ -267,9 +251,9 @@
   }
   Seq sq; sq.w = a.rd.words + cr.woff; sq.exc = a.rd.exc + cr.excoff; sq.nexc = cr.nexc; sq.L = cr.L;
   const int nsteps = (sl.dbg & 32) ? 0 : wave_max(active ? cr.endrow : 0);
-  f2 M[BP], I[BP], D[BP];
-#pragma unroll
-  for (int j = 0; j < BP; j++) { M[j] = (f2){0.f, 0.f}; I[j] = (f2){0.f, 0.f}; D[j] = (f2){0.f, 0.f}; }
+  f2 W[BP], G[BP];
+#pragma unroll
+  for (int j = 0; j < BP; j++) { W[j] = (f2){0.f, 0.f}; G[j] = (f2){0.f, 0.f}; }
   const float pmove = (2.0f + 1.0f) / ((float)L + 2.0f + 1.0f);
   const float ploop = 1.0f - pmove;
   float xN = 0.f, xJ = 0.f, xB = 0.f, xC = pmove;
@@ -283,14 +267,12 @@
     const int64_t node = (int64_t)cr.src - sl.node_base;
     const f4 *src = (const f4 *)sl.slots + (node * sl.Pb + (prof - sl.p0)) * FWD_STATE_Q;
 #pragma unroll
-    for (int j = 0; j < BP; j++) { const f4 v = src[j]; M[j] = (f2){v.x, v.y}; I[j] = (f2){v.z, v.w}; }
-#pragma unroll
-    for (int j = 0; j < BP / 2; j++) { const f4 v = src[BP + j]; D[2 * j] = (f2){v.x, v.y}; D[2 * j + 1] = (f2){v.z, v.w}; }
-    const f4 u = src[BP + BP / 2], t = src[BP + BP / 2 + 1];
-    D[BP - 1] = (f2){u.x, u.y}; xN = u.z; xJ = u.w; xC = t.x; xB = t.y;
-    totscale = __builtin_bit_cast(double, (f2){t.z, t.w});
-  }
-  const int A = (L + (1 << sl.logB) - 1) >> sl.logB;
+    for (int j = 0; j < BP; j++) { const f4 v = src[j]; W[j] = (f2){v.x, v.y}; G[j] = (f2){v.z, v.w}; }
+    const f4 u = src[BP], t = src[BP + 1];
+    xN = u.x; xJ = u.y; xC = u.z; xB = u.w;
+    totscale = __builtin_bit_cast(double, (f2){t.x, t.y});
+  }
+  const int A =(L + (1 << sl.logB) - 1) >> sl.logB;
   const int top = (A - rd) << sl.logB;
   const int first = top < L ? top : L;
   SeqStream ss; ss.open(sq, first > 0 ? first - 1 : 0, -1);
@@ -302,12 +284,10 @@
         const int64_t node = snode + __popcll(smask & ((1ull << rdl) - 1ull));
         f4 *dst = (f4 *)sl.slots + (node * sl.Pb + (prof - sl.p0)) * FWD_STATE_Q;
 #pragma unroll
-        for (int j = 0; j < BP; j++) dst[j] = (f4){M[j].x, M[j].y, I[j].x, I[j].y};
-#pragma unroll
-        for (int j = 0; j < BP / 2; j++) dst[BP + j] = (f4){D[2 * j].x, D[2 * j].y, D[2 * j + 1].x, D[2 * j + 1].y};
+        for (int j = 0; j < BP; j++) dst[j] = (f4){W[j].x, W[j].y, G[j].x, G[j].y};
         const f2 ts = __builtin_bit_cast(f2, totscale);
-        dst[BP + BP / 2] = (f4){D[BP - 1].x, D[BP - 1].y, xN, xJ};
-        dst[BP + BP / 2 + 1] = (f4){xC, xB, ts.x, ts.y};
+        dst[BP] = (f4){xN, xJ, xC, xB};
+        dst[BP + 1] = (f4){ts.x, ts.y, 0.f, 0.f};
       }
     }
     if (step >= nsteps) break;
@@ -324,38 +304,31 @@
       float aDn = 0.0f, wn = 0.0f;
       f2 accB = (f2){0.f, 0.f};
 #define SB __builtin_amdgcn_sched_barrier(0)
-      const f4 tl = *(cf4q)(uintptr_t)(tb + BP * 12);
-      RT cur = ldrt(tb, BP - 1);
-      f2 ecur = *(const f2 *)(ex + 2 * (BP - 1));
-      __builtin_amdgcn_s_waitcnt(0xC07F);
-      float aD2 = __builtin_fmaf(tl.w, aDn, D[BP - 1].y);
-      f2 pre = M[BP - 1] + aEv;
-      float aD1 = __builtin_fmaf(tl.z, aD2, D[BP - 1].x);
-      f2 iig = (f2){tl.x, tl.y} * I[BP - 1];
-      f2 aM = pre + (f2){aD2, aDn};
-      aDn = aD1;
-#pragma unroll
-      for (int j = BP - 1; j >= 0; j--) {
+      RT cur = ldrt(tb, BP);
+      f2 ecur = (f2){0.f, 0.f};
+      f2 aM = (f2){0.f, 0.f};
+#pragma unroll
+      for (int j = BP; j >= 0; j--) {
         __builtin_amdgcn_s_waitcnt(0xC07F);
         const RT t = cur;
         const f2 e = ecur;
-        const bool more = j > 0;
+        const bool late = j < BP, more = j > 0;
         if (more) { cur = ldrt(tb, j - 1); ecur = *(const f2 *)(ex + 2 * (j - 1)); }
         SB;
-        const f2 w = aM * e; SB;
-        float aD2n = 0.f, aD1n = 0.f; f2 pren = (f2){0.f, 0.f}, iign = pren, aMn = pren;
-        if (more) { aD2n = __builtin_fmaf(t.aa.y, aDn, D[j - 1].y); SB; }
-        accB = pfma(t.bm, w, accB); SB;
-        if (more) { pren = M[j - 1] + aEv; SB; }
-        const f2 wsh = (f2){w.y, wn}; SB;
-        if (more) { aD1n = __builtin_fmaf(t.aa.x, aD2n, D[j - 1].x); SB; }
-        const f2 gi = I[j];
-        M[j] = pfma(t.mm, wsh, gi); SB;
-        if (more) { iign = t.ii * I[j - 1]; SB; }
-        I[j] = pfma(t.im, wsh, iig); SB;
-        if (more) { aMn = pren + (f2){aD2n, aDn}; SB; }
-        D[j] = t.dm * wsh; SB;
-        wn = w.x; aDn = aD1n; aM = aMn; iig = iign;
+        f2 w = (f2){0.f, 0.f}, gD = w, pren = w, gMp = w, iig = w, aMn = w;
+        float aD2n = 0.f, aD1n = 0.f;
+        if (late) { w = aM * e; SB; }
+        if (more) { gD = t.dm * W[j - 1]; SB; }
+        if (late) { accB = pfma(t.bm, w, accB); SB; }
+        if (more) { pren = G[j - 1] + aEv; SB; }
+        if (more) { aD2n = __builtin_fmaf(t.aa.y, aDn, gD.y); SB; }
+        if (late) { W[j] = (f2){w.y, wn}; SB; }
+        if (more) { gMp = pfma(t.mm, W[j - 1], pren); SB; }
+        if (more) { aD1n = __builtin_fmaf(t.aa.x, aD2n, gD.x); SB; }
+        if (more) { iig = t.ii * G[j - 1]; SB; }
+        if (more) { aMn = gMp + (f2){aD2n, aDn}; SB; }
+        if (more) { G[j - 1] = pfma(t.im, W[j - 1], iig); SB; }
+        wn = w.x; aDn = aD1n; aM = aMn;
       }
 #undef SB
       xB = accB.x + accB.y;
@@ -364,13 +337,13 @@
     if ((step & 15) == 15) {
       f2 sm = (f2){0.f, 0.f};
 #pragma unroll
-      for (int j = 0; j < BP; j++) sm = sm + ((M[j] + I[j]) + D[j]);
+      for (int j = 0; j < BP; j++) sm = sm + (W[j] + G[j]);
       const float tot = (sm.x + sm.y) + ((xN + xJ) + (xC + xB));
       if (tot > 1e6f || (tot < 1e-6f && tot > 0.0f)) {
         const float r = 1.0f / tot;
         const f2 rv = (f2){r, r};
 #pragma unroll
-        for (int j = 0; j < BP; j++) { M[j] = M[j] * rv; I[j] = I[j] * rv; D[j] = D[j] * rv; }
+        for (int j = 0; j < BP; j++) { W[j] = W[j] * rv; G[j] = G[j] * rv; }
         xN *= r; xJ *= r; xC *= r; xB *= r;
         totscale += det_log((double)tot);
       }
@@ -386,8 +359,9 @@
 
 static float bound_rescale()
 {
-  static const float v = [] { const char *e = sw_get("ITSX_BOUND_RESCALE_EXP"); const double x = e ? atof(e) : 20.0; return (float)pow(10.0, x < 4.0 ? 4.0 : x > 28.0 ? 28.0 : x); }();
-  return v;
+  const char *e = sw_get("ITSX_BOUND_RESCALE_EXP");
+  const double x = e ? atof(e) : 20.0;
+  return (float)pow(10.0, x < 4.0 ? 4.0 : x > 28.0 ? 28.0 : x);
 }
 void launch_fwd_bound_seq(const FloatArgs &a, const float *btab, bool fold, float *fb, int nwaves, int wave0, hipStream_t st)
 {
diff --git a/itsxpress_amd/csrc/switches.cpp b/itsxpress_amd/csrc/switches.cpp
--- a/itsxpress_amd/csrc/switches.cpp
+++ b/itsxpress_amd/csrc/switches.cpp
@@ -37,6 +37,7 @@
   {"ITSX_MSV_TWO", SW_TUNING, "=0: the MSV filter keeps the one-sided (prefix-only) schedule when pass A shares two-sidedly"},
   {"ITSX_SHARE_B", SW_TUNING, "rows per block of the prefix / suffix trees (default 32)"},
   {"ITSX_SHARE_GB", SW_TUNING, "budget of the saved row states, GB"},
+  {"ITSX_SHARE_DIV", SW_TUNING, "the saved row states' budget is all of a search's states divided by this (default 3.8: four batches; 2.8: three)"},
   {"ITSX_SHARE_MIN", SW_TUNING, "smallest shared-row fraction for which the shared schedule is used (default 0.10)"},
   {"ITSX_SHARE_FWD_STREAMS", SW_TUNING, "1 | 2 streams for pass A's batches"},
   {"ITSX_SHARE_MSV_STREAMS", SW_TUNING, "1 | 2 streams for the MSV filter's batches"},
```
